# swacisko/ALGA

Measured on AMD Instinct MI355X. Metric: overlap_edges_per_sec, higher is better.
Workload: dtype u32; 1 GPU; cfg4_50M_150bp: 50000000 x 150 bp reads, genome 250000000, seed 11, err 0.00 -> 90621096 nodes (both strands, duplicates removed), min_overlap 82, rsoemo 116; generated on the device (alga_amd.workload.device_build) in 0.9 s; nodes=90621096, edges=92350115

## Files before the change

alga_amd/csrc/engine.hip:

```cpp
#include <hip/hip_runtime.h>

#include <algorithm>
#include <chrono>
#include <cstdio>
#include <cstdlib>
#include <cstring>
#include <new>
#include <string>
#include <thread>
#include <vector>

#include "engine_internal.h"

using namespace alga;

namespace {

using Prepared = AlgaPrepared;

int prepare(alga_engine *e, const alga_nodes *nodes, const alga_prefsuf_params *p, hipStream_t s, Prepared &out) {
    if (!nodes || !p) return alga_fail(e, ALGA_ERR_INVALID_ARGUMENT, "nodes/params must not be NULL");
    if (nodes->n < 0) return alga_fail(e, ALGA_ERR_INVALID_ARGUMENT, "negative node count");
    if (nodes->n > 0 && (!nodes->words || !nodes->len)) return alga_fail(e, ALGA_ERR_INVALID_ARGUMENT, "words/len must not be NULL");
    if (nodes->stride_words <= 0 && nodes->n > 0) return alga_fail(e, ALGA_ERR_INVALID_ARGUMENT, "stride_words must be positive");
// ... 2 lines not shown
    if (p->max_len_cap < 1 || p->max_len_cap > 500) return alga_fail(e, ALGA_ERR_INVALID_ARGUMENT, "max_len_cap must be in [1, 500]");
    if (p->rsoe_min_overlap < 0) return alga_fail(e, ALGA_ERR_INVALID_ARGUMENT, "rsoe_min_overlap must be >= 0");
    if (p->keys_shared < 0 || p->keys_shared > 2) return alga_fail(e, ALGA_ERR_INVALID_ARGUMENT, "keys_shared must be 0, 1 or 2");
    int rc;
    if ((rc = alga_ensure(e, e->counters, (CNT_TOTAL + 2) * sizeof(unsigned long long)))) return rc;
    HIP_TRY(e, hipMemsetAsync(e->counters.p, 0, (CNT_TOTAL + 2) * sizeof(unsigned long long), s));
    NodesDev nd;
    nd.words = nodes->words; nd.len = nodes->len; nd.from = nodes->align_from; nd.to = nodes->align_to;
    nd.n = nodes->n; nd.stride = nodes->stride_words;
    unsigned long long *cnt = (unsigned long long *) e->counters.p;
    int *d_maxlen = (int *) (cnt + CNT_TOTAL);
    unsigned long long mask_asym = 0;
    int min_len = 0;
    if (p->keys_shared == 2 && e->store_n == nodes->n && e->store_words == (const void *) nodes->words && e->stat_len == (const void *) nodes->len &&
        e->stat_from == (const void *) nodes->align_from && e->stat_to == (const void *) nodes->align_to) {
        out.max_len = e->stat_max_len; out.live = e->stat_live; mask_asym = e->stat_mask_asym; min_len = e->stat_min_len;
    } else {
        launch_node_stats(nd, cnt, d_maxlen, s);
        if ((rc = alga_check_launch(e, "k_node_stats"))) return rc;
        HIP_TRY(e, hipMemcpyAsync(e->h_counters, e->counters.p, (CNT_TOTAL + 2) * sizeof(unsigned long long), hipMemcpyDeviceToHost, s));
        HIP_TRY(e, hipStreamSynchronize(s));
        out.max_len = (int) (e->h_counters[CNT_TOTAL] & 0xFFFFFFFFull);
        min_len = out.max_len > 0 ? 0x7FFFFFFF - (int) (e->h_counters[CNT_TOTAL] >> 32) : 0;
        out.live = e->h_counters[CNT_LIVE_NODES];
        mask_asym = e->h_counters[CNT_MASK_ASYM];
        e->stat_max_len = out.max_len; e->stat_min_len = min_len; e->stat_live = out.live; e->stat_mask_asym = mask_asym;
        e->stat_len = (const void *) nodes->len; e->stat_from = (const void *) nodes->align_from; e->stat_to = (const void *) nodes->align_to;
    }
    out.nd = nd;
    out.uniform_len = (out.max_len > 0 && min_len == out.max_len && !nodes->align_from) ? out.max_len : 0;
    if ((int64_t) blocks_of(out.max_len) > (int64_t) nodes->stride_words)
        return alga_fail(e, ALGA_ERR_INVALID_ARGUMENT, "stride_words is smaller than the longest read needs");
    if (out.max_len > OL_MAX_NODE_LEN) return alga_fail(e, ALGA_ERR_CAPACITY, "a node is longer than 4 194 303 nt (overlap records keep the offset in 22 bits)");
    PrefSufCfg c;
    c.Lmin = p->min_overlap;
    c.rsoemo = p->rsoe_min_overlap;
    c.Lcap = std::min(out.max_len, p->max_len_cap) + 1;
    c.soes = p->soes;
    const int seed_nt = std::min(c.Lmin, SEED_MAX_NT);
    c.seed_words = (2 * seed_nt + 31) >> 5;
    c.seed_last_mask = (2 * seed_nt & 31) ? ((1u << (2 * seed_nt & 31)) - 1u) : 0xFFFFFFFFu;
    c.reversed = (c.rsoemo > c.Lcap) ? 1 : 0;
    c.stats = p->collect_stats ? 1 : 0;
    out.cfg = c;
    if (p->reduction < ALGA_REDUCTION_AUTO || p->reduction > ALGA_REDUCTION_SOURCE_SIDE)
        return alga_fail(e, ALGA_ERR_INVALID_ARGUMENT, "reduction must be an alga_reduction value");
    out.local_ok = out.max_len <= p->max_len_cap && out.max_len - c.Lmin <= LOCAL_MAX_SPAN && c.Lmin <= c.rsoemo && c.rsoemo <= c.Lcap &&
                   mask_asym == 0;
    out.local_sw = out.max_len - c.Lmin <= 63 ? 1 : 2;
    out.cluster_eq = 0;
    const bool wide = out.local_sw == 2 || blocks_of(out.max_len) > 13;
    if (out.local_ok && e->opt_probe != ALGA_PROBE_TABLE && !(wide && e->opt_probe == ALGA_PROBE_AUTO && out.live < (4ull << 20))) {
        int eq = 0;
        if (cluster_plan(c, out.max_len, out.live, e->opt_cluster_bucket_bias, &out.cluster, &eq)) out.cluster_eq = eq;
    }
    out.keys_shared = p->keys_shared;
    out.reduction = p->reduction;
    if (out.reduction == ALGA_REDUCTION_AUTO && e->opt_force_per_target) out.reduction = ALGA_REDUCTION_PER_TARGET;
    return ALGA_OK;
}

int cluster_alloc(alga_engine *e, const Prepared &pp) {
    int rc;
    const uint64_t n = (uint64_t) pp.nd.n;
    for (int k = 0; k < 2; k++) {
        if ((rc = alga_ensure(e, e->cl_keys[k], (n + ALGA_KEY_ARRAY_SLACK + 1) * sizeof(uint32_t)))) return rc;
        if ((rc = alga_ensure(e, e->cl_vals[k], (n + 1) * sizeof(uint32_t)))) return rc;
    }
    if ((rc = alga_ensure(e, e->cl_meta, (n + ALGA_KEY_ARRAY_SLACK + 1) * sizeof(uint32_t)))) return rc;
    if ((rc = alga_ensure(e, e->cl_runs, (n + 1) * CL_RMAX * 8))) return rc;
    if ((rc = alga_ensure(e, e->cl_nruns, n + 16))) return rc;
    if ((rc = alga_ensure(e, e->cl_store, (n + 2) * 16 * (size_t) pp.cluster_eq))) return rc;
    if ((rc = alga_ensure(e, e->cl_dir, ((size_t) pp.cluster.n_buckets + 2) * 16))) return rc;
    return alga_ensure(e, e->sort_temp, cluster_sort_temp_bytes(n));
}

int pile_alloc(alga_engine *e, uint64_t n, uint32_t n_buckets, hipStream_t s) {
    int rc;
    if ((rc = alga_ensure(e, e->cl_pile_rec, pile_record_bytes(n)))) return rc;
    if ((rc = alga_ensure(e, e->cl_pile_rec2, pile_record_bytes(n)))) return rc;
    if ((rc = alga_ensure(e, e->cl_pile_succ, ((size_t) n + 64) * 16))) return rc;
    if ((rc = alga_ensure(e, e->cl_pile_cnt, PILE_CNT_WORDS * sizeof(unsigned long long)))) return rc;
    if ((rc = alga_ensure(e, e->cl_pile_own, pile_own_mask_bytes(n)))) return rc;
    if ((rc = alga_ensure(e, e->cl_defer, (size_t) (n + 64) * sizeof(int32_t)))) return rc;
    const void *before = e->cl_pile_tab.p;
    const size_t cap_before = e->cl_pile_tab.cap;
    if ((rc = alga_ensure(e, e->cl_pile_tab, pile_table_bytes(n_buckets)))) return rc;
    if (e->cl_pile_tab.p != before || e->cl_pile_tab.cap != cap_before) {
        HIP_TRY(e, hipMemsetAsync(e->cl_pile_tab.p, 0, e->cl_pile_tab.cap, s));
        HIP_TRY(e, hipStreamSynchronize(s));
        e->pile_epoch = 0;
    }
    return ALGA_OK;
}

int discover_impl(alga_engine *e, const Prepared &pp, int32_t src_begin, int32_t src_end, hipStream_t s, uint64_t *n_rec, bool local = false,
                  bool *overflow = nullptr) {
    int rc;
    const NodesDev &nd = pp.nd;
    const PrefSufCfg &cfg = pp.cfg;
    unsigned long long *cnt = (unsigned long long *) e->counters.p;
    *n_rec = 0;
    HIP_TRY(e, hipEventRecord(e->ev[EV_START], s));
    if (pp.live >= (1ull << 31)) return alga_fail(e, ALGA_ERR_CAPACITY, "too many nodes for one seed table; shard the input");
    const bool clustered = local && pp.cluster_eq != 0;
    e->pairs_timed = false;
    e->store_timed = false;
    e->pile_timed = false;
    const bool all_sources = src_begin == 0 && src_end == pp.nd.n;
    const bool pile_index_left = e->opt_pile_range != 0 && e->pile_n == pp.nd.n && e->pile_words == (const void *) pp.nd.words;
    bool pile = clustered && e->opt_pile != 0 && e->opt_cluster_pairs != 0 && e->opt_cluster_order != 0 && pp.local_sw == 1 &&
                      (pp.keys_shared == 0 || (pp.keys_shared == 2 && pile_index_left)) &&
                      (all_sources || (e->opt_pile_range != 0 && src_begin >= 0 && src_end <= pp.nd.n && src_begin < src_end)) && pile_plan(cfg, pp.cluster, pp.cluster_eq, pp.uniform_len, pp.nd.from != nullptr || pp.nd.to != nullptr);
    e->loc_second_used = false;
    bool keys_only = false;
    const bool need_vals = !e->opt_own_sort || e->opt_test_unsorted_index;
    uint32_t n_buckets = 0, filter_bits = 0;
    bool have_table = false;
    auto build_table = [&]() -> int {
        n_buckets = seed_buckets_for(pp.live, e->seed_fill_x10);
        const size_t table_bytes = (size_t) n_buckets * SEED_BUCKET * sizeof(unsigned long long);
        int r;
        if ((r = alga_ensure(e, e->table, table_bytes))) return r;
        HIP_TRY(e, hipMemsetAsync(e->table.p, 0xFF, table_bytes, s));
        filter_bits = seed_filter_bits_for(pp.live);
        if (filter_bits) {
            if ((r = alga_ensure(e, e->filter, filter_bits / 8))) return r;
            HIP_TRY(e, hipMemsetAsync(e->filter.p, 0, filter_bits / 8, s));
        }
        launch_seed_build(nd, cfg, (unsigned long long *) e->table.p, n_buckets, (uint32_t *) e->filter.p, filter_bits, s);
        if ((r = alga_check_launch(e, "k_seed_build"))) return r;
        e->stats.table_slots = (uint64_t) n_buckets * SEED_BUCKET;
        have_table = true;
        return ALGA_OK;
    };
    ClusterCfg cc{};
    if (clustered) {
        cc = pp.cluster;
        if ((rc = cluster_alloc(e, pp))) return rc;
        if (pp.keys_shared == 2) {
            const bool store_left = e->store_n == nd.n && e->store_words == (const void *) nd.words && e->store_eq == pp.cluster_eq && e->store_buckets == cc.n_buckets;
            const bool piles_serve = pile && e->pile_kept_pure && e->store_buckets == cc.n_buckets && e->store_eq == pp.cluster_eq;
            if (!(store_left || piles_serve) || src_begin < e->store_run_begin || src_end > e->store_run_end)
                return alga_fail(e, ALGA_ERR_INVALID_ARGUMENT, "keys_shared = 2: no entry array of this node set that covers the sources is left from the previous build");
            keys_only = pile && e->pile_keys_only;
        } else {
            int32_t run_begin = 0, run_end = nd.n;
            if (pp.keys_shared == 1) {
                if (e->keyed_n != nd.n || e->keyed_words != (const void *) nd.words || src_begin < e->keyed_begin || src_end > e->keyed_end)
                    return alga_fail(e, ALGA_ERR_INVALID_ARGUMENT, "keys_shared: alga_prefsuf_keys_device has not been called on this node set for a range that covers the sources");
                run_begin = e->keyed_begin; run_end = e->keyed_end;
            } else {
                keys_only = pile && e->opt_pile_runs != 0 && !e->expect_pairwise && !e->opt_pile_check;
                launch_cluster_keys(nd, cfg, cc, 0, nd.n, (uint32_t *) e->cl_keys[0].p, need_vals ? (uint32_t *) e->cl_vals[0].p : nullptr, (uint32_t *) e->cl_meta.p, e->cl_runs.p,
                                    (uint8_t *) e->cl_nruns.p, s, !keys_only);
                if ((rc = alga_check_launch(e, "k_node_runs"))) return rc;
            }
            HIP_TRY(e, hipEventRecord(e->ev[EV_KEYS], s));
            e->keyed_n = -1;
            e->store_n = -1;
            HIP_TRY(e, launch_cluster_store(nd, cc, (uint32_t *) e->cl_keys[0].p, (uint32_t *) e->cl_vals[0].p, (uint32_t *) e->cl_keys[1].p,
                                            (uint32_t *) e->cl_vals[1].p, e->sort_temp.p, cluster_sort_temp_bytes((uint64_t) nd.n), e->cl_dir.p, pp.keys_shared == 1 || !need_vals,
                                            e->ev[EV_SORT], cnt + CNT_TOTAL + 1, e->opt_test_unsorted_index != 0, s, e->opt_own_sort != 0));
            HIP_TRY(e, hipEventRecord(e->ev[EV_DIR], s));
            e->pile_n = -1;
            if (pile) {
                rc = e->opt_test_pile_oom ? alga_fail(e, ALGA_ERR_OUT_OF_MEMORY, "pile_alloc (option test_pile_oom)") : pile_alloc(e, (uint64_t) nd.n, cc.n_buckets, s);
                if (rc == ALGA_ERR_OUT_OF_MEMORY) {
                    (void) hipGetLastError();
                    alga_release(e->cl_pile_tab); alga_release(e->cl_pile_rec); alga_release(e->cl_pile_rec2); alga_release(e->cl_pile_succ); alga_release(e->cl_pile_own);
                    e->pile_epoch = 0; e->pile_n = -1;
                    e->err.clear();
                    pile = false;
                    rc = ALGA_OK;
                    if (keys_only) {
                        launch_cluster_keys(nd, cfg, cc, 0, nd.n, (uint32_t *) e->cl_keys[0].p, (uint32_t *) e->cl_vals[0].p, (uint32_t *) e->cl_meta.p, e->cl_runs.p,
                                            (uint8_t *) e->cl_nruns.p, s, true);
                        if ((rc = alga_check_launch(e, "k_node_runs"))) return rc;
                        keys_only = false;
                    }
                } else if (rc) return rc;
            }
            if (pile) {
                launch_pile_sample(nd, cc, pp.uniform_len, (const uint32_t *) e->cl_keys[1].p, (const uint32_t *) e->cl_vals[1].p, e->cl_dir.p,
                                   (unsigned long long *) e->cl_pile_cnt.p, e->opt_pile >= 2 ? e->opt_pile - 1 : 0, s);
                if ((rc = alga_check_launch(e, "k_pile_build<sample>"))) return rc;
            }
            HIP_TRY(e, launch_cluster_gather(nd, cc, pp.cluster_eq, (const uint32_t *) e->cl_keys[1].p, (const uint32_t *) e->cl_vals[1].p, (const uint32_t *) e->cl_meta.p,
                                             pp.uniform_len, e->cl_store.p, (pile && e->opt_pile_skip_gather) ? (const unsigned long long *) e->cl_pile_cnt.p : nullptr, s));
            HIP_TRY(e, hipEventRecord(e->ev[EV_GATHER], s));
            if (pile) {
                if (e->pile_epoch >= 511u) {
                    HIP_TRY(e, hipMemsetAsync(e->cl_pile_tab.p, 0, e->cl_pile_tab.cap, s));
                    e->pile_epoch = 0;
                }
                e->pile_epoch++;
                const bool from_consensus = e->opt_pile_runs != 0;
                launch_pile_build(nd, cfg, cc, pp.uniform_len, (const uint32_t *) e->cl_keys[1].p, (const uint32_t *) e->cl_vals[1].p, e->cl_dir.p, e->cl_pile_rec.p, e->cl_pile_rec2.p, e->cl_pile_tab.p,
                                  e->pile_epoch, e->cl_pile_succ.p, e->cl_runs.p, pp.uniform_len - cfg.Lmin + 1, (const unsigned long long *) e->cl_pile_cnt.p,
                                  from_consensus ? (uint32_t *) e->cl_pile_own.p : nullptr, s);
                if ((rc = alga_check_launch(e, "k_pile_build"))) return rc;
                if (keys_only) {
                    launch_pile_own_ids((const uint32_t *) e->cl_pile_own.p, (const uint32_t *) e->cl_vals[1].p, (uint64_t) nd.n, (int32_t *) e->cl_defer.p, (uint32_t) nd.n,
                                        (unsigned long long *) e->cl_pile_cnt.p, s);
                    launch_cluster_runs_list(nd, cfg, cc, (const int32_t *) e->cl_defer.p, (const unsigned long long *) e->cl_pile_cnt.p + 3, (uint32_t) nd.n, (uint32_t) e->n_cu * 16u,
                                             e->cl_runs.p, (uint8_t *) e->cl_nruns.p, s);
                    launch_cluster_keys(nd, cfg, cc, 0, nd.n, (uint32_t *) e->cl_keys[0].p, (uint32_t *) e->cl_vals[0].p, (uint32_t *) e->cl_meta.p, e->cl_runs.p,
                                        (uint8_t *) e->cl_nruns.p, s, true, (const unsigned long long *) e->cl_pile_cnt.p);
                    if ((rc = alga_check_launch(e, "k_node_runs (own lists)"))) return rc;
                }
                if (e->opt_pile_check && from_consensus)
                    launch_pile_check(e->cl_pile_succ.p, (uint64_t) nd.n, cc.n_buckets, e->cl_pile_tab.p, e->cl_pile_rec2.p, e->pile_epoch, e->cl_runs.p, nd.n, pp.uniform_len - cfg.Lmin + 1,
                                      (unsigned long long *) e->cl_pile_cnt.p, s);
                e->pile_n = nd.n; e->pile_words = (const void *) nd.words;
                e->pile_keys_only = keys_only; e->pile_kept_pure = false;
                e->pile_timed = nd.n > 0;
            }
            e->store_timed = nd.n > 0;
            e->store_n = pile ? -1 : nd.n;
            e->store_words = (const void *) nd.words; e->store_eq = pp.cluster_eq; e->store_buckets = cc.n_buckets;
            e->store_run_begin = run_begin; e->store_run_end = run_end;
        }
        e->stats.table_slots = cc.n_buckets;
    } else if ((rc = build_table())) return rc;
    HIP_TRY(e, hipEventRecord(e->ev[EV_SEED], s));

    const uint64_t n_src = (uint64_t) std::max<int64_t>(0, (int64_t) src_end - src_begin);
    const uint64_t slack = std::max(probe_record_slack(e->n_cu, n_src, local), clustered ? cluster_record_slack(e->n_cu, n_src) : 0);
    uint64_t &hint = local ? e->rec_cap_hint_local : e->rec_cap_hint;
    uint64_t cap = std::max<uint64_t>(hint, (local ? 2 : 16) * n_src + 4096) + slack;
    if (local) {
        if ((rc = alga_ensure(e, e->outdeg, (size_t) (n_src + 1) * sizeof(uint32_t)))) return rc;
        if ((rc = alga_ensure(e, e->loc_first, (size_t) (n_src + 1) * sizeof(unsigned long long)))) return rc;
    }
    const uint32_t big_list_cap = 1u << 20;
    if (local && (rc = alga_ensure(e, e->loc_big_list, big_list_cap * sizeof(int32_t)))) return rc;
    for (int attempt = 0; attempt < 4; attempt++) {
        if (cap >= (1ull << 32) - 16) return alga_fail(e, ALGA_ERR_CAPACITY, "more than 2^32 overlap records; shard the input");
        if (local) HIP_TRY(e, hipMemsetAsync(e->outdeg.p, 0, (size_t) (n_src + 1) * sizeof(uint32_t), s));
        if ((rc = alga_ensure(e, e->rec_dst, cap * sizeof(uint32_t)))) return rc;
        if ((rc = alga_ensure(e, e->rec_val, cap * sizeof(unsigned long long)))) return rc;
        HIP_TRY(e, hipMemsetAsync(cnt, 0, CNT_TOTAL * sizeof(unsigned long long), s));
        ProbeBig big{(int32_t *) e->loc_big_list.p, big_list_cap, 0u, nullptr, 0u};
        e->defer_list_valid = clustered && e->opt_cluster_pairs && pp.local_sw == 1 && pp.cluster_eq <= 4;
        if (clustered) {
            if (e->opt_cluster_pairs && pp.local_sw == 1 && pp.cluster_eq <= 4) {
                if ((rc = alga_ensure(e, e->cl_defer, (size_t) (n_src + 64) * sizeof(int32_t)))) return rc;
                const uint32_t slot_stride = e->opt_stream_slots >= 4 ? (uint32_t) (n_src + 1) : 0u;
                if ((rc = alga_ensure(e, e->loc_second, (size_t) (slot_stride ? LOCAL_SLOTS_MAX - 1 : 1) * (n_src + 1) * sizeof(unsigned long long)))) return rc;
                e->loc_second_used = true;
                e->loc_slot_stride = slot_stride;
                const bool by_key = e->opt_cluster_order != 0 && src_begin == 0 && src_end == nd.n;
                const bool piled = pile && e->pile_n == nd.n && e->pile_words == (const void *) nd.words;
                if (piled) {
                    if (!all_sources) {
                        if ((rc = alga_ensure(e, e->cl_pile_side_r, (size_t) (n_src + 64) * 16))) return rc;
                        if ((rc = alga_ensure(e, e->cl_pile_cursor, 64))) return rc;
                    }
                    launch_pile_probe(nd, cfg, cc, pp.uniform_len, e->cl_pile_tab.p, e->pile_epoch, e->cl_pile_rec.p, e->cl_pile_rec2.p, e->cl_pile_succ.p,
                                      e->cl_runs.p, cnt, (uint32_t *) e->outdeg.p, (unsigned long long *) e->loc_first.p, (unsigned long long *) e->loc_second.p,
                                      (int32_t *) e->cl_defer.p, (uint32_t) n_src, (const unsigned long long *) e->cl_pile_cnt.p, e->n_cu, s, src_begin, src_end,
                                      e->cl_pile_side_r.p, (unsigned long long *) e->cl_pile_cursor.p);
                    if ((rc = alga_check_launch(e, "k_pile_probe"))) return rc;
                    if (keys_only)
                        launch_cluster_runs_list(nd, cfg, cc, (const int32_t *) e->cl_defer.p, cnt + CNT_DEFERRED, (uint32_t) std::min<uint64_t>(n_src + 64, 0xFFFFFFFFull),
                                                 (uint32_t) e->n_cu * 16u, e->cl_runs.p, (uint8_t *) e->cl_nruns.p, s);
                }
                launch_probe_stream(nd, cfg, cc, pp.cluster_eq, e->cl_store.p, e->cl_dir.p, e->cl_runs.p, (const uint8_t *) e->cl_nruns.p,
                                    src_begin, src_end, by_key, cnt, e->n_cu, (uint32_t *) e->outdeg.p, (unsigned long long *) e->loc_first.p,
                                    (unsigned long long *) e->loc_second.p, (int32_t *) e->cl_defer.p, (uint32_t) n_src,
                                    piled ? (const unsigned long long *) e->cl_pile_cnt.p : nullptr, s, slot_stride);
                if ((rc = alga_check_launch(e, "k_probe_stream"))) return rc;
                if (piled) {
                    if ((rc = alga_ensure(e, e->cl_defer2, (size_t) (n_src + 64) * sizeof(int32_t)))) return rc;
                    launch_probe_stream_list(nd, cfg, cc, pp.cluster_eq, e->cl_store.p, e->cl_dir.p, e->cl_runs.p, (const uint8_t *) e->cl_nruns.p, (int32_t *) e->cl_defer.p,
                                             (uint32_t) n_src, cnt, e->n_cu, (uint32_t *) e->outdeg.p, (unsigned long long *) e->loc_first.p,
                                             (unsigned long long *) e->loc_second.p, (int32_t *) e->cl_defer2.p, (const unsigned long long *) e->cl_pile_cnt.p, s, slot_stride, src_begin);
                    if ((rc = alga_check_launch(e, "k_probe_stream (list)"))) return rc;
                }
                HIP_TRY(e, hipEventRecord(e->ev[EV_PAIRS], s));
                e->pairs_timed = true;
                launch_probe_clustered(nd, cfg, cc, pp.cluster_eq, e->cl_store.p, e->cl_dir.p, e->cl_runs.p, (const uint8_t *) e->cl_nruns.p, 0,
                                       (int32_t) n_src, (const int32_t *) e->cl_defer.p, src_begin, (uint32_t *) e->rec_dst.p, (unsigned long long *) e->rec_val.p,
                                       cap, cnt, e->n_cu, (uint32_t *) e->outdeg.p, (unsigned long long *) e->loc_first.p, &big, cnt + CNT_DEFERRED, 1, s,
                                       (const uint32_t *) e->cl_keys[1].p, (const uint32_t *) e->cl_vals[1].p, pp.uniform_len,
                                       (piled && e->opt_pile_skip_gather) ? (const unsigned long long *) e->cl_pile_cnt.p : nullptr);
                if (piled) launch_pile_deg((int32_t) n_src, (unsigned long long *) e->loc_first.p, (uint32_t *) e->outdeg.p, (const unsigned long long *) e->cl_pile_cnt.p, s);
            } else {
                launch_probe_clustered(nd, cfg, cc, pp.cluster_eq, e->cl_store.p, e->cl_dir.p, e->cl_runs.p, (const uint8_t *) e->cl_nruns.p, src_begin,
                                       src_end, nullptr, src_begin, (uint32_t *) e->rec_dst.p, (unsigned long long *) e->rec_val.p, cap, cnt, e->n_cu,
                                       (uint32_t *) e->outdeg.p, (unsigned long long *) e->loc_first.p, &big, nullptr, pp.local_sw, s);
            }
        }
        else
            launch_probe(nd, cfg, (const unsigned long long *) e->table.p, n_buckets, (const uint32_t *) e->filter.p, filter_bits, src_begin, src_end,
                         (uint32_t *) e->rec_dst.p, (unsigned long long *) e->rec_val.p, cap, cnt, e->n_cu, local ? pp.local_sw : 0, (uint32_t *) e->outdeg.p,
                         (unsigned long long *) e->loc_first.p, local ? &big : nullptr, s);
        if ((rc = alga_check_launch(e, "k_probe_sources"))) return rc;
        HIP_TRY(e, hipEventRecord(e->ev[EV_PROBE], s));
        HIP_TRY(e, hipMemcpyAsync(e->h_counters, cnt, (CNT_TOTAL + 2) * sizeof(unsigned long long), hipMemcpyDeviceToHost, s));
        HIP_TRY(e, hipStreamSynchronize(s));
        if (clustered && e->h_counters[CNT_TOTAL + 1] != 0) {
            e->store_n = -1; e->keyed_n = -1;
            return alga_fail(e, ALGA_ERR_HIP, "clustered index: the sorted key array is not in order (entry directory invalid)");
        }
        if (local && e->h_counters[CNT_LOCAL_OVERFLOW] != 0) {
            const uint64_t n_big = e->h_counters[CNT_LOCAL_OVERFLOW], max_items = e->h_counters[CNT_LOCAL_MAXITEMS];
            const uint64_t limit = e->big_limit >= 0 ? (uint64_t) e->big_limit : (uint64_t) local_big_limit();
            if (n_big > big_list_cap || max_items > limit) { if (overflow) *overflow = true; *n_rec = 0; return ALGA_OK; }
            big.count = (uint32_t) n_big;
            big.item_cap = (uint32_t) ((max_items + 63) & ~63ull);
            if ((rc = alga_ensure(e, e->loc_big_items, probe_big_bytes(e->n_cu, big.count, pp.local_sw, big.item_cap)))) return rc;
            big.items = e->loc_big_items.p;
            if (!have_table && (rc = build_table())) return rc;
            HIP_TRY(e, hipMemsetAsync(cnt + CNT_LOCAL_OVERFLOW, 0, sizeof(unsigned long long), s));
            launch_probe(nd, cfg, (const unsigned long long *) e->table.p, n_buckets, (const uint32_t *) e->filter.p, filter_bits, src_begin, src_end,
                         (uint32_t *) e->rec_dst.p, (unsigned long long *) e->rec_val.p, cap, cnt, e->n_cu, pp.local_sw, (uint32_t *) e->outdeg.p,
                         (unsigned long long *) e->loc_first.p, &big, s);
            if ((rc = alga_check_launch(e, "k_probe_sources (second pass)"))) return rc;
            HIP_TRY(e, hipEventRecord(e->ev[EV_PROBE], s));
            HIP_TRY(e, hipMemcpyAsync(e->h_counters, cnt, CNT_TOTAL * sizeof(unsigned long long), hipMemcpyDeviceToHost, s));
            HIP_TRY(e, hipStreamSynchronize(s));
            if (e->h_counters[CNT_LOCAL_OVERFLOW] != 0) { if (overflow) *overflow = true; *n_rec = 0; return ALGA_OK; }
            e->stats.big_sources = n_big;
        }
        const uint64_t need = e->h_counters[CNT_RECORDS];
        if (need <= cap) {
            *n_rec = need;
            hint = std::max<uint64_t>(hint, need + need / 16 + 4096);
            if (overflow) *overflow = false;
            if (local) { e->stats.transitive_compares = e->h_counters[CNT_TR_COMPARES]; e->stats.generic_sources = e->h_counters[CNT_LOCAL_GENERIC]; }
            e->stats.records = e->h_counters[CNT_VALID_RECORDS];
            e->stats.raw_overlaps = e->h_counters[CNT_RAW];
            e->stats.windows_probed = e->h_counters[CNT_WINDOWS];
            e->stats.slots_scanned = e->h_counters[CNT_SLOTS];
            e->stats.probe_rounds = e->h_counters[CNT_ROUNDS];
            e->stats.pile_buckets = e->h_counters[CNT_PILE_BUCKETS]; e->stats.pile_irregular = e->h_counters[CNT_PILE_IRREGULAR];
            e->stats.pile_own_lists = e->h_counters[CNT_PILE_OWN];
            if (pile && pp.keys_shared != 2 && e->pile_n == nd.n) {
                const bool kept = e->opt_pile == 2 || e->stats.pile_irregular * (uint64_t) ALGA_PILE_DECLINE_ONE_IN <= e->stats.pile_buckets;
                e->stats.pile_mixed = kept && e->stats.pile_irregular * (uint64_t) ALGA_PILE_IRREGULAR_ONE_IN > e->stats.pile_buckets;
                e->stats.pile_deferred = e->stats.pile_mixed ? e->h_counters[CNT_DEFERRED_PILE] : (kept ? e->h_counters[CNT_DEFERRED] : 0);
                if (!kept || e->stats.pile_mixed || !e->opt_pile_skip_gather) e->store_n = nd.n;
                e->expect_pairwise = !kept;
                e->pile_kept_pure = kept && !e->stats.pile_mixed && e->opt_pile_skip_gather != 0;
                e->stats.pile_list_checked = 0; e->stats.pile_list_mismatch = 0;
                if (e->opt_pile_check) {
                    unsigned long long chk[2] = {0ull, 0ull};
                    HIP_TRY(e, hipMemcpyAsync(chk, (const unsigned long long *) e->cl_pile_cnt.p + 4, sizeof(chk), hipMemcpyDeviceToHost, s));
                    HIP_TRY(e, hipStreamSynchronize(s));
                    e->stats.pile_list_checked = chk[0]; e->stats.pile_list_mismatch = chk[1];
                }
            }
            if (!pile) e->expect_pairwise = false;
            e->stats.probe_used = clustered ? ALGA_PROBE_CLUSTER : ALGA_PROBE_TABLE;
            if (clustered) e->stats.deferred_sources = e->defer_list_valid ? e->h_counters[CNT_DEFERRED] : n_src;
            return ALGA_OK;
        }
        cap = need + need / 16 + 4096 + slack;
    }
    return alga_fail(e, ALGA_ERR_HIP, "record buffer kept overflowing");
}

int key_bits_for(int64_t n_owned) {
    int b = 1;
    while (b < 31 && (1ll << b) < n_owned) b++;
    return std::min(32, b + 1);
}

int reduce_impl(alga_engine *e, const Prepared &pp, const uint32_t *rec_dst, const unsigned long long *rec_val, uint64_t n_rec,
                uint64_t n_valid_hint, int32_t dst_begin, int32_t dst_end, hipStream_t s, uint64_t *n_edges) {
    int rc;
    const NodesDev &nd = pp.nd;
    const PrefSufCfg &cfg = pp.cfg;
    unsigned long long *cnt = (unsigned long long *) e->counters.p;
    const int32_t n_owned = dst_end - dst_begin;
    *n_edges = 0;
    if (n_rec >= (1ull << 32) - 16) return alga_fail(e, ALGA_ERR_CAPACITY, "more than 2^32 overlap records; shard the input");
    const int bits = key_bits_for(n_owned);
    const size_t temp_bytes = sort_records_temp_bytes(n_rec, bits);
    if ((rc = alga_ensure(e, e->keys, (size_t) (n_rec + 1) * sizeof(uint32_t)))) return rc;
    if ((rc = alga_ensure(e, e->seg_key, (size_t) (n_rec + 1) * sizeof(uint32_t)))) return rc;
    if ((rc = alga_ensure(e, e->seg_val, (size_t) (n_rec + 1) * sizeof(unsigned long long)))) return rc;
    if ((rc = alga_ensure(e, e->sort_temp, temp_bytes))) return rc;
    if ((rc = alga_ensure(e, e->heads, (size_t) (n_rec + 1) * 16))) return rc;
    if ((rc = alga_ensure(e, e->rowptr, (size_t) (n_owned + 2) * sizeof(uint32_t)))) return rc;
    HIP_TRY(e, hipMemsetAsync(cnt + CNT_SORT_VALID, 0, sizeof(unsigned long long), s));
    launch_make_keys(rec_dst, n_rec, dst_begin, dst_end, (uint32_t *) e->keys.p, cnt + CNT_SORT_VALID, s);
    if ((rc = alga_check_launch(e, "k_make_keys"))) return rc;
    HIP_TRY(e, sort_records(e->sort_temp.p, temp_bytes, (const uint32_t *) e->keys.p, (uint32_t *) e->seg_key.p, rec_val,
                            (unsigned long long *) e->seg_val.p, n_rec, bits, s));
    launch_rowptr_from_sorted((const uint32_t *) e->seg_key.p, cnt + CNT_SORT_VALID, n_rec, n_owned, (uint32_t *) e->rowptr.p, s);
    if ((rc = alga_check_launch(e, "k_rowptr_from_sorted"))) return rc;
    launch_gather_heads(nd, (const unsigned long long *) e->seg_val.p, cnt + CNT_SORT_VALID, n_rec, e->heads.p, s);
    if ((rc = alga_check_launch(e, "k_gather_heads"))) return rc;
    HIP_TRY(e, hipEventRecord(e->ev[EV_GROUP], s));

    if ((rc = alga_ensure(e, e->out_cnt, (size_t) (n_owned + 1) * sizeof(uint32_t)))) return rc;
    if ((rc = alga_ensure(e, e->outdeg, (size_t) (nd.n + 1) * sizeof(uint32_t)))) return rc;
    HIP_TRY(e, hipMemsetAsync(e->outdeg.p, 0, (size_t) (nd.n + 1) * sizeof(uint32_t), s));
    const int tpb = reduce_targets_per_block(n_valid_hint, (uint64_t) std::max(1, n_owned));
    launch_reduce_targets(nd, cfg, dst_begin, n_owned, tpb, (const uint32_t *) e->rowptr.p, (unsigned long long *) e->seg_val.p,
                          e->heads.p, (uint32_t *) e->out_cnt.p, (uint32_t *) e->outdeg.p, cnt, s);
    if ((rc = alga_check_launch(e, "k_reduce_targets"))) return rc;
    HIP_TRY(e, hipEventRecord(e->ev[EV_REDUCE], s));

    if ((rc = alga_ensure(e, e->scan_scratch, scan_scratch_bytes((uint64_t) nd.n)))) return rc;
    if ((rc = alga_ensure(e, e->out_rowptr, (size_t) (nd.n + 1) * sizeof(uint32_t)))) return rc;
    launch_exclusive_scan((const uint32_t *) e->outdeg.p, (uint64_t) nd.n, (uint32_t *) e->out_rowptr.p, (uint64_t *) e->scan_scratch.p, s);
    if ((rc = alga_check_launch(e, "scan(outdeg)"))) return rc;
    uint64_t *d_total = (uint64_t *) e->scan_scratch.p + scan_total_index((uint64_t) nd.n);
    HIP_TRY(e, hipMemcpyAsync(&e->h_counters[CNT_TOTAL], d_total, sizeof(uint64_t), hipMemcpyDeviceToHost, s));
    HIP_TRY(e, hipMemcpyAsync(e->h_counters, cnt, CNT_TOTAL * sizeof(unsigned long long), hipMemcpyDeviceToHost, s));
    HIP_TRY(e, hipStreamSynchronize(s));
    const uint64_t E = e->h_counters[CNT_TOTAL];
    if (E >= (1ull << 32) - 16) return alga_fail(e, ALGA_ERR_CAPACITY, "more than 2^32 edges; shard the input");
    if ((rc = alga_ensure(e, e->edges, (size_t) (E + 1) * sizeof(alga_edge_dev)))) return rc;
    launch_scatter_by_source(cfg, dst_begin, n_owned, (const uint32_t *) e->rowptr.p, (const unsigned long long *) e->seg_val.p,
                             (const uint32_t *) e->out_cnt.p, (const uint32_t *) e->out_rowptr.p, (uint32_t *) e->outdeg.p,
                             (alga_edge_dev *) e->edges.p, s);
    if ((rc = alga_check_launch(e, "k_scatter_by_source"))) return rc;
    launch_sort_rows(nd.n, (const uint32_t *) e->out_rowptr.p, (alga_edge_dev *) e->edges.p, s);
    if ((rc = alga_check_launch(e, "k_sort_rows"))) return rc;
    HIP_TRY(e, hipEventRecord(e->ev[EV_EMIT], s));
    HIP_TRY(e, hipStreamSynchronize(s));
    *n_edges = E;
    e->stats.edges = E;
    e->stats.transitive_listed = e->h_counters[CNT_TR_LISTED];
    e->stats.transitive_compares = e->h_counters[CNT_TR_COMPARES];
    e->stats.transitive_removed = e->h_counters[CNT_TR_REMOVED];
    e->stats.max_in_records = e->h_counters[CNT_MAX_IN];
    return ALGA_OK;
}

int finalize_local(alga_engine *e, const Prepared &pp, int32_t src_begin, int32_t src_end, uint64_t n_rec, hipStream_t s, uint64_t *n_edges) {
    int rc;
    *n_edges = 0;
    const uint64_t n_src = (uint64_t) std::max<int64_t>(0, (int64_t) src_end - src_begin);
    if ((rc = alga_ensure(e, e->scan_scratch, scan_scratch_bytes(n_src)))) return rc;
    if ((rc = alga_ensure(e, e->out_rowptr, (size_t) (n_src + 1) * sizeof(uint32_t)))) return rc;
    if ((rc = alga_ensure(e, e->out_cnt, (size_t) (n_src + 1) * sizeof(uint32_t)))) return rc;
    HIP_TRY(e, hipEventRecord(e->ev[EV_GROUP], s));
    HIP_TRY(e, hipEventRecord(e->ev[EV_REDUCE], s));
    launch_exclusive_scan((const uint32_t *) e->outdeg.p, n_src, (uint32_t *) e->out_rowptr.p, (uint64_t *) e->scan_scratch.p, s);
    if ((rc = alga_check_launch(e, "scan(outdeg)"))) return rc;
    const uint64_t E = e->stats.records;
    if (E >= (1ull << 32) - 16) return alga_fail(e, ALGA_ERR_CAPACITY, "more than 2^32 edges; shard the input");
    if ((rc = alga_ensure(e, e->edges, (size_t) (E + 1) * sizeof(alga_edge_dev)))) return rc;
    launch_local_emit(src_begin, (int32_t) n_src, (const uint32_t *) e->outdeg.p, (const unsigned long long *) e->loc_first.p,
                      e->loc_second_used ? (const unsigned long long *) e->loc_second.p : nullptr, (const uint32_t *) e->rec_dst.p, (const unsigned long long *) e->rec_val.p, n_rec, (const uint32_t *) e->out_rowptr.p,
                      (uint32_t *) e->out_cnt.p, (alga_edge_dev *) e->edges.p,
                      e->defer_list_valid ? (const int32_t *) e->cl_defer.p : nullptr, (const unsigned long long *) e->counters.p + CNT_DEFERRED, (uint32_t) n_src, s,
                      e->loc_second_used ? e->loc_slot_stride : 0u);
    if ((rc = alga_check_launch(e, "k_local_emit"))) return rc;
    HIP_TRY(e, hipEventRecord(e->ev[EV_EMIT], s));
    uint64_t *d_total = (uint64_t *) e->scan_scratch.p + scan_total_index(n_src);
    HIP_TRY(e, hipMemcpyAsync(&e->h_counters[CNT_TOTAL], d_total, sizeof(uint64_t), hipMemcpyDeviceToHost, s));
    HIP_TRY(e, hipStreamSynchronize(s));
    if (e->h_counters[CNT_TOTAL] != E) return alga_fail(e, ALGA_ERR_HIP, "source-side emit: out-degrees and edge count disagree");
    *n_edges = E;
    e->stats.edges = E;
    return ALGA_OK;
}

int build_local(alga_engine *e, const Prepared &pp, int32_t src_begin, int32_t src_end, hipStream_t s, uint64_t *n_edges) {
    if (!pp.local_ok) return alga_fail(e, ALGA_ERR_UNSUPPORTED, "source-side reduction is not exact for this input (read lengths / masks / rsoemo)");
    uint64_t n_rec = 0;
    bool overflow = false;
    int rc = discover_impl(e, pp, src_begin, src_end, s, &n_rec, true, &overflow);
    if (rc) return rc;
    if (overflow) return alga_fail(e, ALGA_ERR_UNSUPPORTED, "a source node has more raw overlaps than the source-side reduction holds");
    if ((rc = finalize_local(e, pp, src_begin, src_end, n_rec, s, n_edges))) return rc;
    e->stats.reduction_used = ALGA_REDUCTION_SOURCE_SIDE;
    return ALGA_OK;
}

double now_ms_host() { return std::chrono::duration<double, std::milli>(std::chrono::steady_clock::now().time_since_epoch()).count(); }

float ev_ms(alga_engine *e, int a, int b) {
    float ms = 0.f;
    if (hipEventElapsedTime(&ms, e->ev[a], e->ev[b]) != hipSuccess) return 0.f;
    return ms;
}

void store_phase_stats(alga_engine *e) {
    if (!e->store_timed) return;
    e->stats.ms_keys = ev_ms(e, EV_START, EV_KEYS);
    e->stats.ms_sort = ev_ms(e, EV_KEYS, EV_SORT);
    e->stats.ms_dir = ev_ms(e, EV_SORT, EV_DIR);
    e->stats.ms_gather = ev_ms(e, EV_DIR, EV_GATHER);
    e->stats.ms_pile = e->pile_timed ? ev_ms(e, EV_GATHER, EV_SEED) : 0.0;
}

}

int alga_prepare(alga_engine *e, const alga_nodes *nodes, const alga_prefsuf_params *p, hipStream_t s, AlgaPrepared &out) { return prepare(e, nodes, p, s, out); }
int alga_cluster_alloc(alga_engine *e, const AlgaPrepared &pp) { return cluster_alloc(e, pp); }

extern "C" {

int alga_abi_version(void) { return ALGA_AMD_ABI_VERSION; }

struct DeviceGuard {
    int prev = -1;
    DeviceGuard() { if (hipGetDevice(&prev) != hipSuccess) prev = -1; }
    ~DeviceGuard() { if (prev >= 0) (void) hipSetDevice(prev); }
};

static void engine_free_handles(alga_engine *e) {
    if (e->h_counters) (void) hipHostFree(e->h_counters);
    for (int i = 0; i < EV_COUNT; i++) if (e->ev[i]) (void) hipEventDestroy(e->ev[i]);
    if (e->own_stream) (void) hipStreamDestroy(e->own_stream);
    if (e->side_stream) (void) hipStreamDestroy(e->side_stream);
    if (e->ev_side) (void) hipEventDestroy(e->ev_side);
    e->h_counters = nullptr; e->own_stream = nullptr; e->side_stream = nullptr; e->ev_side = nullptr;
    for (int i = 0; i < EV_COUNT; i++) e->ev[i] = nullptr;
}

int alga_engine_create(int hip_device, alga_engine **out) {
    if (!out) return ALGA_ERR_INVALID_ARGUMENT;
    *out = nullptr;
    int ndev = 0;
    hipError_t err = hipGetDeviceCount(&ndev);
    if (err != hipSuccess || ndev <= 0) return ALGA_ERR_NO_DEVICE;
    if (hip_device < 0 || hip_device >= ndev) return ALGA_ERR_INVALID_ARGUMENT;
    DeviceGuard guard;
    if (hipSetDevice(hip_device) != hipSuccess) return ALGA_ERR_NO_DEVICE;
    alga_engine *e = new (std::nothrow) alga_engine();
    if (!e) return ALGA_ERR_OUT_OF_MEMORY;
    e->device = hip_device;
    memset(&e->stats, 0, sizeof(e->stats));
    hipDeviceProp_t prop;
    if (hipGetDeviceProperties(&prop, hip_device) == hipSuccess) {
        snprintf(e->dev_name, sizeof(e->dev_name), "%s (%s, %d CUs)", prop.name, prop.gcnArchName, prop.multiProcessorCount);
        if (prop.multiProcessorCount > 0) e->n_cu = prop.multiProcessorCount;
    }
    int rc = ALGA_OK;
    if (hipStreamCreateWithFlags(&e->own_stream, hipStreamNonBlocking) != hipSuccess) { e->own_stream = nullptr; rc = ALGA_ERR_HIP; }
    if (rc == ALGA_OK && hipStreamCreateWithFlags(&e->side_stream, hipStreamNonBlocking) != hipSuccess) { e->side_stream = nullptr; rc = ALGA_ERR_HIP; }
    if (rc == ALGA_OK && hipEventCreateWithFlags(&e->ev_side, hipEventDisableTiming) != hipSuccess) { e->ev_side = nullptr; rc = ALGA_ERR_HIP; }
    for (int i = 0; i < EV_COUNT && rc == ALGA_OK; i++)
        if (hipEventCreate(&e->ev[i]) != hipSuccess) { e->ev[i] = nullptr; rc = ALGA_ERR_HIP; }
    if (rc == ALGA_OK && hipHostMalloc((void **) &e->h_counters, (CNT_TOTAL + 2 + alga_engine::H_EXTRA) * sizeof(unsigned long long)) != hipSuccess) { e->h_counters = nullptr; rc = ALGA_ERR_OUT_OF_MEMORY; }
    if (rc == ALGA_OK && hipHostGetDevicePointer((void **) &e->h_counters_dev, e->h_counters, 0) != hipSuccess) rc = ALGA_ERR_HIP;
    if (rc != ALGA_OK) { engine_free_handles(e); delete e; return rc; }
    *out = e;
    return ALGA_OK;
}

void alga_engine_destroy(alga_engine *e) {
    if (!e) return;
    DeviceGuard guard;
    (void) hipSetDevice(e->device);
    if (e->own_stream) (void) hipStreamSynchronize(e->own_stream);
    if (e->side_stream) (void) hipStreamSynchronize(e->side_stream);
    for (DevBuf *b : e->owned) alga_release(*b);
    alga_release(e->up_raw);
    for (DevBuf *b : {&e->in_bytes[0], &e->in_bytes[1], &e->in_nl[0], &e->in_nl[1], &e->in_tiles, &e->in_tile_off}) alga_release(*b);
    for (DevBuf *b : {&e->sp_rowptr, &e->sp_sorted, &e->sp_list, &e->sp_cnt, &e->sp_orow, &e->sp_out, &e->sp_in}) alga_release(*b);
    alga_staging_release(e);
    for (void *&p : e->gfa_pin) { if (p) (void) hipHostFree(p); p = nullptr; }
    for (auto &kv : e->host_lists) free(kv.first);
    e->host_lists.clear();
    engine_free_handles(e);
    delete e;
}

const char *alga_last_error(const alga_engine *e) { return e ? e->err.c_str() : "no engine"; }

int alga_engine_device_name(const alga_engine *e, char *buf, size_t buflen) {
    if (!e || !buf || buflen == 0) return ALGA_ERR_INVALID_ARGUMENT;
    snprintf(buf, buflen, "%s", e->dev_name);
    return ALGA_OK;
}

int alga_engine_set_option(alga_engine *e, const char *name, int64_t value) {
    if (!e || !name) return ALGA_ERR_INVALID_ARGUMENT;
    e->err.clear();
    if (!strcmp(name, "probe")) {
        if (value < ALGA_PROBE_AUTO || value > ALGA_PROBE_CLUSTER) return alga_fail(e, ALGA_ERR_INVALID_ARGUMENT, "option probe: 0 auto, 1 table, 2 cluster");
        e->opt_probe = (int) value;
    } else if (!strcmp(name, "cluster_bucket_bias")) {
        if (value < -8 || value > 8) return alga_fail(e, ALGA_ERR_INVALID_ARGUMENT, "option cluster_bucket_bias: -8 .. 8");
        e->opt_cluster_bucket_bias = (int) value;
    } else if (!strcmp(name, "cluster_pairs")) {
        e->opt_cluster_pairs = value != 0;
    } else if (!strcmp(name, "pile")) {
        e->opt_pile = (value == 2 || value == 3) ? (int) value : (value != 0);
    } else if (!strcmp(name, "pile_runs")) {
        e->opt_pile_runs = value != 0;
    } else if (!strcmp(name, "pile_check")) {
        e->opt_pile_check = value != 0;
    } else if (!strcmp(name, "pile_skip_gather")) {
        e->opt_pile_skip_gather = value != 0;
    } else if (!strcmp(name, "cluster_order")) {
        e->opt_cluster_order = value != 0;
    } else if (!strcmp(name, "local_big_max")) {
        e->big_limit = value < 0 ? -1 : (int) std::min<int64_t>(value, 1 << 20);
    } else if (!strcmp(name, "shard_bucket_max")) {
        e->opt_shard_dmax = (int) std::max<int64_t>(1, std::min<int64_t>(value, 4096));
    } else if (!strcmp(name, "rsort_variant")) {
        rsort_set_variant((int) value);
    } else if (!strcmp(name, "stream_slots")) {
        e->opt_stream_slots = value >= 4 ? 4 : 2;
    } else if (!strcmp(name, "pile_range")) {
        e->opt_pile_range = value != 0;
    } else if (!strcmp(name, "pkb_legacy")) {
        e->opt_pkb_legacy = (int) value;
    } else if (!strcmp(name, "own_sort")) {
        e->opt_own_sort = value != 0;
    } else if (!strcmp(name, "test_presort_oom")) {
        e->opt_test_presort_oom = value != 0;
    } else if (!strcmp(name, "test_pile_oom")) {
        e->opt_test_pile_oom = value != 0;
    } else if (!strcmp(name, "test_unsorted_index")) {
        e->opt_test_unsorted_index = value != 0;
    } else if (!strcmp(name, "gfa_chunk_mb")) {
        if (value < 1 || value > 4096) return alga_fail(e, ALGA_ERR_INVALID_ARGUMENT, "option gfa_chunk_mb: 1 .. 4096");
        e->opt_gfa_chunk_mb = (int) value;
    } else if (!strcmp(name, "auto_reduction_per_target")) {
        e->opt_force_per_target = value != 0;
    } else return alga_fail(e, ALGA_ERR_INVALID_ARGUMENT, "unknown option");
    return ALGA_OK;
}

int alga_engine_reserve(alga_engine *e, int32_t n_nodes, int32_t max_len, int32_t min_overlap, uint64_t n_edges_hint) {
    if (!e) return ALGA_ERR_INVALID_ARGUMENT;
    e->err.clear();
    if (n_nodes < 0 || max_len < 1 || min_overlap < 1) return alga_fail(e, ALGA_ERR_INVALID_ARGUMENT, "alga_engine_reserve: n_nodes >= 0, max_len >= 1, min_overlap >= 1");
    DeviceGuard guard;
    HIP_TRY(e, hipSetDevice(e->device));
    int rc;
    const uint64_t n = (uint64_t) n_nodes;
    const uint64_t E = n_edges_hint ? n_edges_hint : n + n / 16 + 4096;
    if ((rc = alga_ensure(e, e->counters, (CNT_TOTAL + 2) * sizeof(unsigned long long)))) return rc;
    Prepared pp;
    pp.nd.n = n_nodes; pp.max_len = max_len; pp.live = n;
    pp.cfg.Lmin = min_overlap; pp.cfg.Lcap = std::min(max_len, 500) + 1; pp.cfg.rsoemo = min_overlap; pp.cfg.soes = 3;
    int eq = 0;
    const bool local = max_len <= 500 && max_len - min_overlap <= LOCAL_MAX_SPAN;
    const bool clustered = local && e->opt_probe != ALGA_PROBE_TABLE &&
                           cluster_plan(pp.cfg, max_len, n, e->opt_cluster_bucket_bias, &pp.cluster, &eq);
    if (clustered) {
        pp.cluster_eq = eq;
        if ((rc = cluster_alloc(e, pp))) return rc;
        if (max_len - min_overlap <= 63 && eq <= 4) {
            if ((rc = alga_ensure(e, e->cl_defer, (size_t) (n + 64) * sizeof(int32_t)))) return rc;
            if ((rc = alga_ensure(e, e->loc_second, (size_t) (e->opt_stream_slots >= 4 ? LOCAL_SLOTS_MAX - 1 : 1) * (n + 1) * sizeof(unsigned long long)))) return rc;
        }
        if (e->opt_pile != 0 && e->opt_cluster_pairs != 0 && e->opt_cluster_order != 0 && max_len - min_overlap <= 63 && pile_plan(pp.cfg, pp.cluster, eq, max_len, false)) {
            if ((rc = pile_alloc(e, n, pp.cluster.n_buckets, e->own_stream))) return rc;
        }
    } else {
        const uint32_t nb = seed_buckets_for(n, e->seed_fill_x10);
        if ((rc = alga_ensure(e, e->table, (size_t) nb * SEED_BUCKET * sizeof(unsigned long long)))) return rc;
        const uint32_t fb = seed_filter_bits_for(n);
        if (fb && (rc = alga_ensure(e, e->filter, fb / 8))) return rc;
    }
    if (local) {
        const uint64_t slack = std::max(probe_record_slack(e->n_cu, n, true), clustered ? cluster_record_slack(e->n_cu, n) : 0);
        const uint64_t cap = std::max<uint64_t>(e->rec_cap_hint_local, 2 * n + 4096) + slack;
        if ((rc = alga_ensure(e, e->outdeg, (size_t) (n + 1) * sizeof(uint32_t)))) return rc;
        if ((rc = alga_ensure(e, e->loc_first, (size_t) (n + 1) * sizeof(unsigned long long)))) return rc;
        if ((rc = alga_ensure(e, e->loc_big_list, (1u << 20) * sizeof(int32_t)))) return rc;
        if ((rc = alga_ensure(e, e->rec_dst, cap * sizeof(uint32_t)))) return rc;
        if ((rc = alga_ensure(e, e->rec_val, cap * sizeof(unsigned long long)))) return rc;
        if ((rc = alga_ensure(e, e->scan_scratch, scan_scratch_bytes(n)))) return rc;
        if ((rc = alga_ensure(e, e->out_rowptr, (size_t) (n + 1) * sizeof(uint32_t)))) return rc;
        if ((rc = alga_ensure(e, e->out_cnt, (size_t) (n + 1) * sizeof(uint32_t)))) return rc;
    }
    if ((rc = alga_ensure(e, e->edges, (size_t) (E + 1) * sizeof(alga_edge_dev)))) return rc;
    if (!e->warmed && n_nodes > 0) {
        const int W = blocks_of(max_len), stride = hbm_row_stride(W), wn = 4096;
// ... 616 lines not shown
```

alga_amd/csrc/engine_internal.h:

```cpp
#pragma once
#include <hip/hip_runtime.h>

#include <cstdio>
#include <algorithm>
#include <string>
#include <vector>
#include <unordered_map>

#include "../../include/alga_amd.h"
#include "prefsuf_common.h"
#include "prefsuf_kernels.h"
#include "pkb_kernels.h"

struct DevBuf {
    void  *p = nullptr;
    size_t cap = 0;
};

enum { EV_START = 0, EV_SEED, EV_PROBE, EV_GROUP, EV_REDUCE, EV_EMIT, EV_PAIRS, EV_KEYS, EV_SORT, EV_GATHER, EV_DIR, EV_COUNT };
constexpr int ALGA_STAGE_THREADS = 8;

struct alga_engine {
    std::vector<DevBuf *> owned;
    int         device = -1;
    hipStream_t own_stream = nullptr;
    hipStream_t side_stream = nullptr;
    hipEvent_t  ev_side = nullptr;
    std::string err;
    char        dev_name[256] = {0};
    int         n_cu = 256;
    int         seed_fill_x10 = 20;
    int         opt_probe = 0;
    int         opt_cluster_bucket_bias = 0;
    int         opt_force_per_target = 0;
    int         opt_shard_dmax = 4096;
    int         opt_test_unsorted_index = 0;
    hipEvent_t  ev[EV_COUNT] = {};
    DevBuf table, filter, counters, rowptr, rec_dst, rec_val, keys, seg_key, seg_val, heads, sort_temp, out_cnt, outdeg, out_rowptr, edges, scan_scratch;
    DevBuf cl_defer;
    uint32_t h_first_hkey = 255;
    int32_t keyed_n = -1, keyed_begin = 0, keyed_end = 0;
    bool defer_list_valid = false;
    const void *keyed_words = nullptr;
    int32_t store_n = -1, store_run_begin = 0, store_run_end = 0, store_eq = 0;
    uint32_t store_buckets = 0;
    const void *store_words = nullptr;
    int stat_max_len = 0, stat_min_len = 0; uint64_t stat_live = 0; unsigned long long stat_mask_asym = 0;
    const void *stat_len = nullptr, *stat_from = nullptr, *stat_to = nullptr;
    bool   warmed = false;
    bool   pairs_timed = false;
    bool   store_timed = false;
    bool   pile_keys_only = false, pile_kept_pure = false;
    int    opt_pile_range = 1;
    int    opt_pile_skip_gather = 1;
    int    opt_pile = 1;
    int    opt_pile_runs = 1;
    int    opt_pile_check = 0;
    bool   expect_pairwise = false;
    DevBuf cl_pile_side_r, cl_pile_cursor;
    DevBuf cl_pile_own;
    int    opt_pkb_legacy = 0;
    int    opt_own_sort = 1;
    int    opt_test_presort_oom = 0;
    int    opt_test_pile_oom = 0;
    bool   pile_timed = false;
    DevBuf cl_pile_succ;
    DevBuf cl_pile_rec2;
    DevBuf cl_pile_rec, cl_pile_cnt, cl_pile_tab;
    uint32_t pile_epoch = 0;
    int32_t pile_n = -1; const void *pile_words = nullptr;
    int    opt_cluster_order = 1;
    int    opt_cluster_pairs = 1;
    DevBuf cl_keys[2], cl_vals[2], cl_meta, cl_runs, cl_nruns, cl_store, cl_dir;
    DevBuf loc_second;
    bool   loc_second_used = false;
    uint32_t loc_slot_stride = 0;
    int    opt_stream_slots = 4;
    DevBuf loc_first, loc_big_list, loc_big_items;
    int    big_limit = -1;
    DevBuf edge_keys, edge_keys2, edge_vals, edge_vals2, edges_sorted, xs_dst, xs_val;
    DevBuf up_words, up_len, up_from, up_to;
    DevBuf up_len_narrow;
    DevBuf cp_deg, cp_dst, cp_off;
    DevBuf cl_defer2;
    DevBuf pk_keys, pk_keys2, pk_vals, pk_vals2, pk_marks, pk_big, pk_add, pk_ekeys, pk_ekeys2, pk_flag, pk_pos, pk_edges[2], pk_rowptr, pk_deg,
           pk_mask, pk_cnt, pk_io, pk_io2, pk_tips, pk_heads, pk_g[2], pk_addk, pk_addk2, pk_merged, pk_hsz, pk_hsz2, pk_heads2, pk_nadd, pk_koff,
           pk_gsz, pk_fixlist, pk_bounds, pk_tiprec, pk_tipidx, pk_keys_all, pk_vals_all;
    DevBuf pk_keys2b, pk_vals2b, pk_headsb, pk_hszb, sort_temp2, pk_fixlist2, pk_cnt2;
    DevBuf pp_rows, pp_len, pp_perm[2], pp_keys[2], pp_mark, pp_keep, pp_pos, pp_out_rows, pp_out_len, pp_out_pair, pp_tally;
    bool        stage_ready = false;
    void       *stage_pin[ALGA_STAGE_THREADS][2] = {};
    hipEvent_t  stage_ev[ALGA_STAGE_THREADS][2] = {};
    hipStream_t stage_stream[ALGA_STAGE_THREADS] = {};
    DevBuf      up_raw;
    std::unordered_map<void *, size_t> host_lists;
    void       *host_spare = nullptr;
    size_t      host_spare_cap = 0;
    DevBuf      in_bytes[2], in_nl[2], in_tiles, in_tile_off;
    DevBuf      sp_rowptr, sp_sorted, sp_list, sp_cnt, sp_orow, sp_out, sp_in;
    DevBuf      gfa_sizes, gfa_off, gfa_rowptr, gfa_tiles, gfa_bounds, gfa_buf;
    void       *gfa_pin[2] = {nullptr, nullptr};
    size_t      gfa_pin_cap = 0;
    int         opt_gfa_chunk_mb = 256;
    DevBuf      sh_keys[2], sh_vals[2], sh_store, sh_dir, sh_desc_out, sh_dkey[2], sh_dval[2], sh_small_top, sh_pending, sh_bitmap, sh_small_out,
                sh_ssrc[2], sh_skey[2], sh_edges_out, sh_deg, sh_rowptr, sh_cursor, sh_edges, sh_flagged, sh_cnt, sh_gflag, sh_gpos, sh_gstart;
    struct {
        int      phase = 0;
        int      rank = 0, n_ranks = 1, eq = 0, uniform_len = 0;
        int32_t  n = 0;
        const void *words = nullptr;
        alga::PrefSufCfg cfg{};
        alga::ClusterCfg cc{};
        uint32_t bucket_base = 0, bpr = 0;
        uint64_t n_targets = 0, n_desc = 0, n_rec = 0;
        uint32_t *d_keys_sorted = nullptr;
        unsigned long long *d_vals_sorted = nullptr;
    } sh;
    alga_shard_stats shard_stats{};
    struct {
        int      phase = 0;
        int      rounds = 0, round = 0, rank = 0, n_ranks = 1, cur = 0, key_bits = 0;
        int32_t  prio[4] = {0, 1, 2, 3};
        uint64_t E = 0, nk = 0;
        uint32_t n_tips = 0;
        int      pre_set = 0, cur_set = 0;
        bool     no_look_ahead = false;
        int      pre_round = -1;
        bool     kmers_all = false;
        size_t   kmers_stride = 0;
        int      kmers_sort_bits = 0;
        alga_nodes dn{};
        alga::PkbCfg cfg{};
    } pkb;
    unsigned long long *h_counters = nullptr;
    static constexpr int H_EXTRA = 132 + 16, H_PRE = alga::CNT_TOTAL + 2 + 132;
    uint32_t *h_counters_dev = nullptr;
    uint64_t    rec_cap_hint = 0, rec_cap_hint_local = 0;
    alga_prefsuf_stats stats;
    double      stats_host[2] = {0.0, 0.0};
// ... 71 lines not shown
```

alga_amd/csrc/prefsuf_cluster_device.h:

```cpp
#pragma once
#include <hip/hip_runtime.h>
#include "prefsuf_common.h"
#include "../../include/alga_amd.h"
#include "prefsuf_device.h"

namespace alga {

__device__ __forceinline__ uint32_t kmer_hash(uint32_t lo, uint32_t hi) {
    return (lo ^ __funnelshift_l(hi, hi, 13) ^ (hi >> 7)) * 0x9E3779B1u;
}

__device__ __forceinline__ bool kmer_class0(uint32_t lo) { return (lo & 3u) == 0u && ((((lo >> 2) ^ (lo >> 3)) & 1u) != 0u); }
__device__ __forceinline__ uint32_t order_key0(uint32_t h, int pos) { return ((h >> 1) & 0x7FFFFF00u) | (uint32_t) pos; }
__device__ __forceinline__ uint32_t order_key(uint32_t h, uint32_t lo, int pos) { return order_key0(h, pos) | (kmer_class0(lo) ? 0u : 0x80000000u); }
__device__ __forceinline__ uint32_t class0_mask16(uint32_t cur, uint32_t nxt) {
    const uint32_t nx = __funnelshift_r(cur, nxt, 2);
    return ~(cur | (cur >> 1)) & (nx ^ (nx >> 1)) & 0x55555555u;
}
__device__ __forceinline__ uint32_t compress_even(uint32_t x) {
    x = (x | (x >> 1)) & 0x33333333u;
    x = (x | (x >> 2)) & 0x0F0F0F0Fu;
    x = (x | (x >> 4)) & 0x00FF00FFu;
    return (x | (x >> 8)) & 0x0000FFFFu;
}

__device__ __forceinline__ uint32_t cluster_key(uint32_t h, int fs) {
    uint32_t k = h * 0x9E3779B1u;
    k ^= k >> 15;
    k *= 0x85EBCA77u;
    k ^= k >> 13;
    k *= 0xC2B2AE3Du;
    return (k >> (fs + CL_MBITS)) == (0xFFFFFFFFu >> (fs + CL_MBITS)) ? k ^ 0x80000000u : k;
}

__device__ __forceinline__ uint32_t tgt_sort_key(uint32_t ckey, uint32_t m_c, int fs) {
    const uint32_t fm = ((1u << CL_MBITS) - 1u) << fs;
    return (ckey & ~fm) | ((m_c << fs) & fm);
}
__device__ __forceinline__ bool same_cluster(uint32_t entry_key, uint32_t ckey, int fs) {
    return ((entry_key ^ ckey) & ~(((1u << CL_MBITS) - 1u) << fs)) == 0u;
}

constexpr unsigned long long PILE_IRREGULAR_ONE_IN = ALGA_PILE_IRREGULAR_ONE_IN;
constexpr unsigned long long PILE_DECLINE_ONE_IN = ALGA_PILE_DECLINE_ONE_IN;
__device__ __forceinline__ bool pile_cnt_declines(const unsigned long long *c) { return c[1] * PILE_DECLINE_ONE_IN > c[0]; }
__device__ __forceinline__ bool pile_cnt_mixed(const unsigned long long *c) { return !pile_cnt_declines(c) && c[1] * PILE_IRREGULAR_ONE_IN > c[0]; }
__device__ __forceinline__ void run_slice(const uint4 &rec, uint32_t run_y, uint32_t &e0, uint32_t &cnt) {
    const int q = (int) (run_y & 255u), p0 = (int) ((run_y >> 8) & 255u), p1 = (int) ((run_y >> 16) & 255u);
    int mlo = q - p1 + 1, mhi = q - p0;
    mlo = mlo < 0 ? 0 : mlo; mhi = mhi > 63 ? 63 : mhi;
    e0 = rec.x; cnt = rec.y;
    if (mhi < mlo) { cnt = 0u; return; }
    if (rec.y > 255u) return;
    const int s0 = mlo >> 3, s1 = (mhi >> 3) + 1;
    const uint32_t b0 = ((s0 < 4 ? rec.z : rec.w) >> (8 * (s0 & 3))) & 255u;
    const uint32_t b1 = s1 >= 8 ? rec.y : (((s1 < 4 ? rec.z : rec.w) >> (8 * (s1 & 3))) & 255u);
    e0 = rec.x + b0; cnt = b1 - b0;
}

__device__ __forceinline__ void kmer_key(const uint32_t *row, int i, bool valid, const ClusterCfg &cc, uint32_t &h, uint32_t &pk) {
    const int bit = 2 * i, q = bit >> 5, r = bit & 31;
    const uint32_t x0 = row[q], x1 = row[q + 1], x2 = row[q + 2];
    const uint32_t lo = funnel(x0, x1, r) & cc.lo_mask;
    h = kmer_hash(lo, funnel(x1, x2, r) & cc.hi_mask);
    pk = valid ? order_key(h, lo, i) : 0xFFFFFFFFu;
}

constexpr int TK_ROWS = 128;
constexpr int NR_STACK = 8;

template <bool WIDE, int RCAP = CL_RMAX>
__device__ __forceinline__ void node_runs_core(const uint32_t *row, int nwin, bool act, const ClusterCfg &cc, uint32_t (*stk)[TK_ROWS], uint16_t (*rbuf)[TK_ROWS], int t,
                                               int &nr, bool &uncovered, bool &stack_ovf, uint32_t &cur0, int step = 64) {
    constexpr int S0 = NR_STACK + 1;
    const int w = cc.w;
    nr = 0; uncovered = false; stack_ovf = false; cur0 = 0xFFFFFFFFu;
    for (int hb = (WIDE && nwin > step) ? ((nwin - 1) / step) * step : 0; hb >= 0; hb -= step) {
        const uint32_t *rowh = row + (hb >> 4);
        const int nwh = !WIDE ? nwin : (nwin - hb < step ? nwin - hb : step);
        const int nk = act ? nwh - 1 + w : 0;
        uint64_t m_lo, m_hi;
        {
            uint32_t dm[4];
#pragma unroll
            for (int d = 0; d < 4; d++) {
                const uint32_t x0 = rowh[2 * d], x1 = rowh[2 * d + 1], x2 = rowh[2 * d + 2];
                dm[d] = compress_even(class0_mask16(x0, x1)) | (compress_even(class0_mask16(x1, x2)) << 16);
            }
            m_lo = (uint64_t) dm[0] | ((uint64_t) dm[1] << 32);
            m_hi = (uint64_t) dm[2] | ((uint64_t) dm[3] << 32);
            m_lo &= nk >= 64 ? ~0ull : (nk <= 0 ? 0ull : ((1ull << nk) - 1ull));
            m_hi &= nk <= 64 ? 0ull : ((1ull << (nk - 64)) - 1ull);
        }
        uint64_t b0 = w >= 64 ? m_lo : (m_lo & ((1ull << w) - 1ull));
        uint64_t b1 = w >= 64 ? m_hi : ((m_lo >> w) | (m_hi << (64 - w)));
        auto key_at = [&](int pos) -> uint32_t {
            const int bit = 2 * pos, q = bit >> 5, r = bit & 31;
            const uint32_t x0 = rowh[q], x1 = rowh[q + 1], x2 = rowh[q + 2];
            return order_key0(kmer_hash(funnel(x0, x1, r) & cc.lo_mask, funnel(x1, x2, r) & cc.hi_mask), pos);
        };
        uint32_t cur1 = 0xFFFFFFFFu;
        int sp1 = 0;
        while (b1 != 0ull) {
            const int e = __builtin_ctzll(b1);
            b1 &= b1 - 1ull;
            const uint32_t pk = key_at(w + e);
            const bool push = pk < cur1;
            stk[(push && sp1 < NR_STACK) ? sp1 : NR_STACK][t] = pk;
            cur1 = push ? pk : cur1;
            sp1 += push ? 1 : 0;
        }
        uint32_t cur0h = 0xFFFFFFFFu;
        int sp0 = 0;
        while (b0 != 0ull) {
            const int e = 63 - __builtin_clzll(b0);
            b0 ^= 1ull << e;
            const uint32_t pk = key_at(e);
            const bool push = pk < cur0h;
            stk[S0 + ((push && sp0 < NR_STACK) ? sp0 : NR_STACK)][t] = pk;
            cur0h = push ? pk : cur0h;
            sp0 += push ? 1 : 0;
        }
        if (hb == 0) cur0 = cur0h;
        stack_ovf = stack_ovf || sp1 > NR_STACK || sp0 > NR_STACK;
        sp1 = sp1 > NR_STACK ? NR_STACK : sp1;
        sp0 = sp0 > NR_STACK ? NR_STACK : sp0;
        {
            const uint32_t hq = (uint32_t) hb | ((uint32_t) hb << 8);
            uint32_t top = sp1 > 0 ? stk[sp1 - 1][t] : 0xFFFFFFFFu;
            uint32_t nxt0 = stk[S0][t];
            uint32_t c0 = 0xFFFFFFFFu, win = top;
            int i0 = 0, p_hi = nwh - 1;
            int e0 = sp0 > 0 ? (int) (nxt0 & 255u) : -1;
            int e1 = sp1 > 0 ? (int) (top & 255u) - w : -1;
            while ((e0 > e1 ? e0 : e1) >= 0) {
                const int pe = e0 > e1 ? e0 : e1;
                const bool take0 = e0 >= e1;
                const int row_i = take0 ? S0 + i0 + 1 : (sp1 >= 2 ? sp1 - 2 : NR_STACK);
                const uint32_t v = stk[row_i][t];
                i0 += take0 ? 1 : 0;
                sp1 -= take0 ? 0 : 1;
                c0 = take0 ? nxt0 : c0;
                nxt0 = take0 ? v : nxt0;
                top = take0 ? top : (sp1 >= 1 ? v : 0xFFFFFFFFu);
                e0 = take0 ? (i0 < sp0 ? (int) (v & 255u) : -1) : e0;
                e1 = take0 ? e1 : (sp1 >= 1 ? (int) (v & 255u) - w : -1);
                const uint32_t wn = c0 < top ? c0 : top;
                const int pc = pe < p_hi ? pe : p_hi;
                const bool em = wn != win && pc < p_hi;
                rbuf[(em && nr < RCAP) ? nr : RCAP][t] = (uint16_t) (((win & 255u) | ((uint32_t) (pc + 1) << 8)) + hq);
                uncovered = uncovered || (em && win == 0xFFFFFFFFu);
                nr += em ? 1 : 0;
                p_hi = em ? pc : p_hi;
                win = wn;
            }
            if (act) {
                if (nr < RCAP) rbuf[nr][t] = (uint16_t) ((win & 255u) + hq);
                uncovered = uncovered || win == 0xFFFFFFFFu;
                nr++;
            }
        }
    }
}

__device__ __forceinline__ uint32_t bperm(uint32_t v, int src_lane) { return (uint32_t) __builtin_amdgcn_ds_bpermute(src_lane << 2, (int) v); }

}
```

alga_amd/csrc/prefsuf_kernels.h:

```cpp
#pragma once
#include <hip/hip_runtime.h>
#include <stddef.h>
#include <stdint.h>
#include "prefsuf_common.h"

namespace alga {

struct alga_edge_dev { int32_t src, dst, offset; };

void launch_restride(const uint32_t *in, int stride_in, uint32_t *out, int stride_out, uint64_t n, hipStream_t s);
void launch_widen_len(const void *in, int elem_bytes , int32_t *out, uint64_t n, hipStream_t s);
void launch_compact_edges(const alga_edge_dev *edges, int32_t n, uint64_t n_edges, uint8_t *deg, uint32_t *dst, uint8_t *off, unsigned long long *bad, hipStream_t s);
void launch_expand_twins(const uint32_t *in, int stride_in, const int32_t *len , uint32_t *out, int stride_out, uint64_t n_pairs, hipStream_t s);
void launch_node_stats(const NodesDev &nd, unsigned long long *counters, int *max_len , hipStream_t s);

uint32_t seed_buckets_for(uint64_t live_nodes, int fill_x10);
uint32_t seed_filter_bits_for(uint64_t live_nodes);
void launch_seed_build(const NodesDev &nd, const PrefSufCfg &cfg, unsigned long long *table, uint32_t n_buckets, uint32_t *filter,
                       uint32_t filter_bits, hipStream_t s);

struct ProbeBig { int32_t *list; uint32_t list_cap; uint32_t count; void *items; uint32_t item_cap; };
int    local_item_capacity();
int    local_big_limit();
size_t probe_big_bytes(int n_cu, uint32_t count, int local, uint32_t item_cap);

void launch_probe(const NodesDev &nd, const PrefSufCfg &cfg, const unsigned long long *table, uint32_t n_buckets,
                  const uint32_t *filter, uint32_t filter_bits, int32_t src_begin, int32_t src_end, uint32_t *rec_dst, unsigned long long *rec_val, uint64_t rec_cap,
                  unsigned long long *counters, int n_cu, int local , uint32_t *deg , unsigned long long *first ,
                  const ProbeBig *big , hipStream_t s);
uint64_t probe_record_slack(int n_cu, uint64_t n_src, bool local);
void launch_local_emit(int32_t src_base, int32_t n_src, const uint32_t *deg, const unsigned long long *first, const unsigned long long *second,
                       const uint32_t *rec_dst, const unsigned long long *rec_val, uint64_t n_rec, const uint32_t *rowptr, uint32_t *cursor,
                       alga_edge_dev *edges, const int32_t *record_sources, const unsigned long long *record_sources_count, uint32_t record_sources_cap, hipStream_t s, uint32_t slot_stride = 0);

bool       cluster_plan(const PrefSufCfg &cfg, int max_len, uint64_t live, int bucket_log2_bias, ClusterCfg *c, int *eq);
size_t     cluster_sort_temp_bytes(uint64_t n);
void       launch_cluster_keys(const NodesDev &nd, const PrefSufCfg &cfg, const ClusterCfg &cc, int32_t node_begin, int32_t node_end, uint32_t *keys,
                               uint32_t *vals, uint32_t *meta, void *runs, uint8_t *nruns, hipStream_t s, bool with_runs = true ,
                               const unsigned long long *only_if_declined = nullptr );
void       launch_cluster_runs_list(const NodesDev &nd, const PrefSufCfg &cfg, const ClusterCfg &cc, const int32_t *ids, const unsigned long long *count, uint32_t cap,
                                    uint32_t grid_blocks, void *runs, uint8_t *nruns, hipStream_t s);
hipError_t launch_cluster_store(const NodesDev &nd, const ClusterCfg &cc, uint32_t *keys, uint32_t *vals, uint32_t *keys2 , uint32_t *vals2, void *sort_temp,
                                size_t sort_temp_bytes, void *dir, bool fill_vals, hipEvent_t ev_sorted ,
                                unsigned long long *bad_flag ,
                                bool test_skip_sort , hipStream_t s, bool own_sort = true);
hipError_t launch_cluster_gather(const NodesDev &nd, const ClusterCfg &cc, int eq, const uint32_t *keys2, const uint32_t *vals2, const uint32_t *meta,
                                 int uniform_len , void *store,
                                 const unsigned long long *pile_cnt , hipStream_t s);
uint64_t   cluster_record_slack(int n_cu, uint64_t n_src);
void       launch_probe_clustered(const NodesDev &nd, const PrefSufCfg &cfg, const ClusterCfg &cc, int eq, const void *store, const void *dir,
                                  const void *runs, const uint8_t *nruns, int32_t src_begin, int32_t src_end, const int32_t *src_list, int32_t src_base, uint32_t *rec_dst, unsigned long long *rec_val, uint64_t rec_cap,
                                  unsigned long long *counters, int n_cu, uint32_t *deg, unsigned long long *first, const ProbeBig *big,
                                  const unsigned long long *list_count ,
                                  int sw , hipStream_t s,
                                  const uint32_t *skeys = nullptr, const uint32_t *sids = nullptr, int uniform_len = 0,
                                  const unsigned long long *pile_cnt = nullptr );
void       launch_probe_stream(const NodesDev &nd, const PrefSufCfg &cfg, const ClusterCfg &cc, int eq, const void *store, const void *dir,
                               const void *runs, const uint8_t *nruns, int32_t src_begin, int32_t src_end, bool by_key ,
                               unsigned long long *counters, int n_cu, uint32_t *deg, unsigned long long *first, unsigned long long *second, int32_t *defer_list,
                               uint32_t defer_cap, const unsigned long long *pile_cnt ,
                               hipStream_t s, uint32_t slot_stride = 0 );
void       launch_pile_deg(int32_t n, unsigned long long *first, uint32_t *deg, const unsigned long long *pile_cnt, hipStream_t s);
bool       pile_plan(const PrefSufCfg &cfg, const ClusterCfg &cc, int eq, int uniform_len, bool masks);
size_t     pile_record_bytes(uint64_t n);
size_t     pile_table_bytes(uint32_t n_buckets);
void       launch_pile_sample(const NodesDev &nd, const ClusterCfg &cc, int uniform_len, const uint32_t *skeys , const uint32_t *sids , const void *dir,
                              unsigned long long *pile_cnt , int no_sample, hipStream_t s);
constexpr int PILE_CNT_WORDS = 6;
size_t     pile_own_mask_bytes(uint64_t n);
void       launch_pile_build(const NodesDev &nd, const PrefSufCfg &cfg, const ClusterCfg &cc, int uniform_len, const uint32_t *skeys, const uint32_t *sids, const void *dir, void *rec,
                             void *rec2 , void *tab, uint32_t epoch, void *side, const void *runs, int nwin, const unsigned long long *pile_cnt,
                             uint32_t *own_mask , hipStream_t s);
void       launch_pile_own_ids(const uint32_t *own_mask, const uint32_t *sids, uint64_t n_entries, int32_t *list, uint32_t cap, unsigned long long *pile_cnt, hipStream_t s);
void       launch_pile_check(const void *side, uint64_t n_entries, uint32_t n_buckets, const void *tab, const void *rec2, uint32_t epoch, const void *runs, int n_nodes, int nwin,
                             unsigned long long *pile_cnt, hipStream_t s);
void       launch_probe_stream_list(const NodesDev &nd, const PrefSufCfg &cfg, const ClusterCfg &cc, int eq, const void *store, const void *dir, const void *runs, const uint8_t *nruns,
                                    int32_t *src_list, uint32_t list_cap, unsigned long long *counters, int n_cu, uint32_t *deg, unsigned long long *first,
                                    unsigned long long *second, int32_t *defer2, const unsigned long long *pile_cnt, hipStream_t s, uint32_t slot_stride = 0,
                                    int32_t src_base = 0 );
void       launch_pile_probe(const NodesDev &nd, const PrefSufCfg &cfg, const ClusterCfg &cc, int uniform_len, const void *tab, uint32_t epoch, const void *rec, const void *rec2, const void *side,
                             const void *runs, unsigned long long *counters, uint32_t *deg, unsigned long long *first, unsigned long long *second, int32_t *defer_list,
                             uint32_t defer_cap, const unsigned long long *pile_cnt, int n_cu, hipStream_t s, int32_t src_begin, int32_t src_end,
                             void *side_range , unsigned long long *cursor );

size_t     rsort_u32_pairs_temp_bytes(uint64_t n);
void       rsort_set_variant(int v);
hipError_t rsort_u32_pairs(void *temp, size_t temp_bytes, const uint32_t *keys_in, uint32_t *keys_out, const uint32_t *vals_in, uint32_t *vals_out, uint64_t n,
                           int begin_bit, hipStream_t s);
size_t     sort_u32_pairs_temp_bytes(uint64_t n);
hipError_t sort_u32_pairs(void *temp, size_t temp_bytes, const uint32_t *keys_in, uint32_t *keys_out, const uint32_t *vals_in, uint32_t *vals_out,
                          uint64_t n, int begin_bit , hipStream_t s, bool own_sort = true );
size_t     rsort_u64_pairs_temp_bytes(uint64_t n);
hipError_t rsort_u64_pairs(void *temp, size_t temp_bytes, const unsigned long long *keys_in, unsigned long long *keys_out, const unsigned long long *vals_in,
                           unsigned long long *vals_out, uint64_t n, int bits, hipStream_t s);
hipError_t rsort_u32_u64(void *temp, size_t temp_bytes, const uint32_t *keys_in, uint32_t *keys_out, const unsigned long long *vals_in, unsigned long long *vals_out,
                         uint64_t n, int begin_bit, int end_bit, hipStream_t s);
size_t     sort_u64_pairs_temp_bytes(uint64_t n, int bits);
hipError_t sort_u64_pairs(void *temp, size_t temp_bytes, const unsigned long long *keys_in, unsigned long long *keys_out,
                          const unsigned long long *vals_in, unsigned long long *vals_out, uint64_t n, int bits, hipStream_t s);

void launch_make_keys(const uint32_t *rec_dst, uint64_t n_rec, int32_t dst_begin, int32_t dst_end, uint32_t *keys,
                      unsigned long long *n_valid, hipStream_t s);
size_t     sort_records_temp_bytes(uint64_t n, int bits);
hipError_t sort_records(void *temp, size_t temp_bytes, const uint32_t *keys_in, uint32_t *keys_out, const unsigned long long *vals_in,
                        unsigned long long *vals_out, uint64_t n, int bits, hipStream_t s);
void launch_rowptr_from_sorted(const uint32_t *keys, const unsigned long long *n_valid_ptr, uint64_t n_rec_max, int32_t n_owned,
                               uint32_t *rowptr, hipStream_t s);

size_t   scan_scratch_bytes(uint64_t n);
uint64_t scan_total_index(uint64_t n);
void launch_exclusive_scan(const uint32_t *in, uint64_t n, uint32_t *out, uint64_t *scratch, hipStream_t s);
constexpr int MAIL_SEGS = 6;
struct MailSeg { const uint32_t *src; uint32_t words, dst; };
struct MailArgs {
    MailSeg seg[MAIL_SEGS];
    int n = 0;
    void add(const void *src, uint32_t words, uint32_t dst_word) { seg[n].src = (const uint32_t *) src; seg[n].words = words; seg[n].dst = dst_word; n++; }
};
void launch_mail(const MailArgs &a, uint32_t *host_block_dev, hipStream_t s);

int  reduce_targets_per_block(uint64_t n_records, uint64_t n_targets);
void launch_gather_heads(const NodesDev &nd, const unsigned long long *seg_val, const unsigned long long *n_valid_ptr, uint64_t n_rec_max,
                         void *heads , hipStream_t s);
void launch_reduce_targets(const NodesDev &nd, const PrefSufCfg &cfg, int32_t dst_begin, int32_t n_owned, int32_t targets_per_block,
                           const uint32_t *rowptr, unsigned long long *seg_val, const void *heads, uint32_t *out_cnt, uint32_t *outdeg,
                           unsigned long long *counters, hipStream_t s);
void launch_scatter_by_source(const PrefSufCfg &cfg, int32_t dst_begin, int32_t n_owned, const uint32_t *rowptr,
                              const unsigned long long *seg_val, const uint32_t *out_cnt, const uint32_t *out_rowptr, uint32_t *out_cursor,
                              alga_edge_dev *edges, hipStream_t s);
void launch_sort_rows(int32_t n, const uint32_t *out_rowptr, alga_edge_dev *edges, hipStream_t s);

void launch_edges_to_keys(const alga_edge_dev *e, uint64_t n, unsigned long long *keys, uint32_t *vals, hipStream_t s);
void launch_keys_to_edges(const unsigned long long *keys, const uint32_t *vals, uint64_t n, alga_edge_dev *e, hipStream_t s);
size_t     sort_edges_temp_bytes(uint64_t n);
hipError_t sort_edges(void *temp, size_t temp_bytes, const unsigned long long *keys_in, unsigned long long *keys_out, const uint32_t *vals_in,
                      uint32_t *vals_out, uint64_t n, int src_bits, hipStream_t s);

}
```

alga_amd/csrc/prefsuf_kernels.hip:

```cpp
#include <hip/hip_runtime.h>
#include <algorithm>
#include "prefsuf_common.h"
#include "prefsuf_kernels.h"
#include "prefsuf_device.h"

namespace alga {

__global__ void __launch_bounds__(256) k_node_stats(NodesDev nd, unsigned long long *counters, int *max_len) {
    __shared__ int s_max[4], s_min[4];
    __shared__ unsigned long long s_live[4];
    int m = 0, mn = 0x7FFFFFFF;
    unsigned long long live = 0, asym = 0;
    auto one = [&](int l, int64_t i) {
        m = l > m ? l : m;
        mn = (l > 0 && l < mn) ? l : mn;
        live += l > 0;
        if (nd.to && l > 0 && !nd.to[i] && (nd.from == nullptr || nd.from[i])) asym++;
    };
    const int64_t gid = (int64_t) blockIdx.x * blockDim.x + threadIdx.x, gsz = (int64_t) gridDim.x * blockDim.x;
    int64_t done = 0;
    if ((reinterpret_cast<uintptr_t>(nd.len) & 15u) == 0) {
        const int64_t nq = (int64_t) nd.n >> 2;
        const int4 *len4 = reinterpret_cast<const int4 *>(nd.len);
        for (int64_t q = gid; q < nq; q += gsz) { const int4 l = len4[q]; one(l.x, 4 * q); one(l.y, 4 * q + 1); one(l.z, 4 * q + 2); one(l.w, 4 * q + 3); }
        done = 4 * nq;
    }
    for (int64_t i = done + gid; i < nd.n; i += gsz) one(nd.len[i], i);
#pragma unroll
    for (int o = 32; o > 0; o >>= 1) { int t = __shfl_xor(m, o); m = t > m ? t : m; t = __shfl_xor(mn, o); mn = t < mn ? t : mn; }
    live = wave_sum_u64(live);
    asym = wave_sum_u64(asym);
    const int wave = (int) (threadIdx.x >> 6);
    if (lane_id() == 0) { s_max[wave] = m; s_min[wave] = mn; s_live[wave] = live; if (asym) atomicAdd(&counters[CNT_MASK_ASYM], asym); }
    __syncthreads();
    if (threadIdx.x == 0) {
        for (int w = 1; w < 4; w++) { m = s_max[w] > m ? s_max[w] : m; mn = s_min[w] < mn ? s_min[w] : mn; live += s_live[w]; }
        if (m > 0) { atomicMax(max_len, m); atomicMax(max_len + 1, 0x7FFFFFFF - mn); }
        if (live) atomicAdd(&counters[CNT_LIVE_NODES], live);
    }
}

__device__ __forceinline__ uint32_t seed_bucket(uint64_t h, uint32_t n_buckets) { return __umulhi((uint32_t) h, n_buckets); }
__device__ __forceinline__ uint32_t seed_taglen(uint64_t h, int len) {
    return ((uint32_t) (h >> 41) << 9) | (uint32_t) (len > 511 ? 511 : len);
}

__device__ __forceinline__ uint32_t seed_filter_index(uint64_t h, uint32_t filter_mask) { return (uint32_t) (h >> 32) & filter_mask; }

__global__ void __launch_bounds__(256) k_seed_build(NodesDev nd, PrefSufCfg cfg, unsigned long long *table, uint32_t n_buckets,
                                                     uint32_t *filter, uint32_t filter_mask) {
    int i = blockIdx.x * blockDim.x + threadIdx.x;
    if (i >= nd.n) return;
    int len = nd.len[i];
    if (len <= 0 || len < cfg.Lmin) return;
    if (nd.to && !nd.to[i]) return;
    const uint32_t *row = nd.words + (size_t) i * nd.stride;
    uint64_t h = fp_init();
    for (int k = 0; k < cfg.seed_words; k++) {
        uint32_t w = row[k];
        if (k == cfg.seed_words - 1) w &= cfg.seed_last_mask;
        h = fp_step(h, w);
    }
    h = fp_final(h);
    uint32_t b = seed_bucket(h, n_buckets);
    if (filter) { const uint32_t fi = seed_filter_index(h, filter_mask); atomicOr(&filter[fi >> 5], 1u << (fi & 31)); }
    const unsigned long long entry = ((unsigned long long) seed_taglen(h, len) << 32) | (uint32_t) i;
    for (;;) {
        unsigned long long *bp = table + (size_t) b * SEED_BUCKET;
        for (int j = 0; j < SEED_BUCKET; j++) {
            if (bp[j] != SEED_EMPTY) continue;
            if (atomicCAS(&bp[j], (unsigned long long) SEED_EMPTY, entry) == SEED_EMPTY) return;
        }
        b = (b + 1 == n_buckets) ? 0u : b + 1;
    }
}

#ifndef PROBE_OCC
#define PROBE_OCC 4
#endif
template <bool STATS, int NQ, int LOCAL, bool BIG = false>
__global__ void __launch_bounds__(PROBE_WAVES * 64, PROBE_OCC)
k_probe_sources(NodesDev nd, PrefSufCfg cfg, const unsigned long long *__restrict__ table, uint32_t n_buckets,
                const uint32_t *__restrict__ filter, uint32_t filter_mask, int32_t src_begin, int32_t src_end, ProbeOut o) {
    __shared__ uint32_t sB[PROBE_WAVES][STAGE_WORDS];
    __shared__ uint32_t sCandC[PROBE_WAVES][CANDMAX];
    __shared__ uint32_t sCandW[PROBE_WAVES][CANDMAX];
    constexpr int WB = LOCAL ? WBUF_LOCAL : WBUF;
// ... 397 lines not shown
    flush_records<CHUNK, WB>(o, w, chunk_base, chunk_fill);
    close_chunk<CHUNK>(o, chunk_base, chunk_fill);
    st_rec = wave_sum_u64(st_rec);
    if (lane == 0 && st_rec) atomicAdd(&o.counters[CNT_VALID_RECORDS], (unsigned long long) st_rec);
    if (STATS) {
        st_raw = wave_sum_u64(st_raw); st_slots = wave_sum_u64(st_slots); st_win = wave_sum_u64(st_win);
        st_cmp = wave_sum_u64(st_cmp); st_generic = wave_sum_u64(st_generic);
        if (lane == 0) {
            atomicAdd(&o.counters[CNT_RAW], (unsigned long long) st_raw);
            atomicAdd(&o.counters[CNT_SLOTS], (unsigned long long) st_slots);
            atomicAdd(&o.counters[CNT_WINDOWS], (unsigned long long) st_win);
            if (LOCAL) {
                atomicAdd(&o.counters[CNT_TR_COMPARES], (unsigned long long) st_cmp);
                atomicAdd(&o.counters[CNT_LOCAL_GENERIC], (unsigned long long) st_generic);
            }
        }
    }
}

__global__ void __launch_bounds__(256) k_make_keys(const uint32_t *__restrict__ rec_dst, uint64_t n_rec, int32_t dst_begin, int32_t dst_end,
                                                    uint32_t *__restrict__ keys, unsigned long long *__restrict__ n_valid) {
    __shared__ unsigned long long s_cnt[4];
    unsigned long long cnt = 0;
    for (uint64_t i = (uint64_t) blockIdx.x * blockDim.x + threadIdx.x; i < n_rec; i += (uint64_t) gridDim.x * blockDim.x) {
        const uint32_t c = rec_dst[i];
        const bool ok = c != REC_INVALID && (int) c >= dst_begin && (int) c < dst_end;
        keys[i] = ok ? c - (uint32_t) dst_begin : 0xFFFFFFFFu;
        cnt += ok;
    }
    cnt = wave_sum_u64(cnt);
    if (lane_id() == 0) s_cnt[threadIdx.x >> 6] = cnt;
    __syncthreads();
    if (threadIdx.x == 0) { cnt = s_cnt[0] + s_cnt[1] + s_cnt[2] + s_cnt[3]; if (cnt) atomicAdd(n_valid, cnt); }
}

__global__ void __launch_bounds__(256) k_rowptr_from_sorted(const uint32_t *__restrict__ keys, const unsigned long long *__restrict__ n_valid_ptr,
                                                             int32_t n_owned, uint32_t *__restrict__ rowptr) {
    const uint64_t nv = (uint64_t) *n_valid_ptr;
    for (uint64_t i = (uint64_t) blockIdx.x * blockDim.x + threadIdx.x; i <= nv; i += (uint64_t) gridDim.x * blockDim.x) {
        const int64_t lo = i == 0 ? 0 : (int64_t) keys[i - 1] + 1;
        const int64_t hi = i == nv ? (int64_t) n_owned : (int64_t) keys[i];
        for (int64_t t = lo; t <= hi; t++) rowptr[t] = (uint32_t) i;
    }
}

constexpr int SCAN_BLOCK = 256;
constexpr int SCAN_ITEMS = 16;
constexpr int SCAN_TILE = SCAN_BLOCK * SCAN_ITEMS;

__device__ __forceinline__ uint32_t block_exclusive_scan(uint32_t v, uint32_t *total, uint32_t *lds ) {
    const int lane = lane_id(), wave = (int) (threadIdx.x >> 6);
    uint32_t inc = v;
#pragma unroll
    for (int o = 1; o < 64; o <<= 1) { uint32_t t = (uint32_t) __shfl_up((int) inc, o); if (lane >= o) inc += t; }
    if (lane == 63) lds[wave] = inc;
    __syncthreads();
    uint32_t wave_off = 0, tot = 0;
    const int nw = (int) (blockDim.x >> 6);
    for (int w = 0; w < nw; w++) { uint32_t s = lds[w]; if (w < wave) wave_off += s; tot += s; }
    __syncthreads();
    *total = tot;
    return wave_off + inc - v;
}

__global__ void __launch_bounds__(SCAN_BLOCK) k_scan_tile_sums(const uint32_t *__restrict__ in, uint64_t n, uint64_t *__restrict__ tile_sums) {
    __shared__ uint32_t lds[8];
    const uint64_t base = (uint64_t) blockIdx.x * SCAN_TILE;
    uint32_t s = 0;
    if (base + SCAN_TILE <= n && (reinterpret_cast<uintptr_t>(in) & 15u) == 0) {
        const uint4 *in4 = reinterpret_cast<const uint4 *>(in + base);
#pragma unroll
        for (int k = 0; k < SCAN_ITEMS / 4; k++) { const uint4 v = in4[k * SCAN_BLOCK + threadIdx.x]; s += v.x + v.y + v.z + v.w; }
    } else {
        for (int k = 0; k < SCAN_ITEMS; k++) {
            uint64_t i = base + (uint64_t) k * SCAN_BLOCK + threadIdx.x;
            if (i < n) s += in[i];
        }
    }
    uint32_t tot;
    block_exclusive_scan(s, &tot, lds);
    if (threadIdx.x == 0) tile_sums[blockIdx.x] = tot;
}

__global__ void __launch_bounds__(1024) k_scan_spine(uint64_t *tile_sums, uint32_t n_tiles) {
    __shared__ uint64_t lds[1024];
    __shared__ uint64_t carry;
    if (threadIdx.x == 0) carry = 0;
    __syncthreads();
    for (uint32_t base = 0; base < n_tiles; base += 1024) {
        uint32_t i = base + threadIdx.x;
        uint64_t v = i < n_tiles ? tile_sums[i] : 0;
        lds[threadIdx.x] = v;
        __syncthreads();
        for (int o = 1; o < 1024; o <<= 1) {
            uint64_t t = threadIdx.x >= (unsigned) o ? lds[threadIdx.x - o] : 0;
            __syncthreads();
            lds[threadIdx.x] += t;
            __syncthreads();
        }
        uint64_t inc = lds[threadIdx.x];
        uint64_t c = carry;
        if (i < n_tiles) tile_sums[i] = c + inc - v;
        __syncthreads();
        if (threadIdx.x == 1023) carry = c + inc;
        __syncthreads();
    }
    if (threadIdx.x == 0) tile_sums[n_tiles] = carry;
}

__global__ void __launch_bounds__(SCAN_BLOCK) k_scan_tiles(const uint32_t *__restrict__ in, uint64_t n,
                                                            const uint64_t *__restrict__ tile_sums, uint32_t *__restrict__ out) {
    __shared__ uint32_t lds[8];
    const bool full = (uint64_t) (blockIdx.x + 1) * SCAN_TILE <= n && (reinterpret_cast<uintptr_t>(in) & 15u) == 0 && (reinterpret_cast<uintptr_t>(out) & 15u) == 0;
    if (full) {
        constexpr int G = SCAN_ITEMS / 4;
        const int lane = lane_id(), wave = (int) (threadIdx.x >> 6);
        const uint64_t wbase = (uint64_t) blockIdx.x * SCAN_TILE + (uint64_t) wave * (64 * SCAN_ITEMS);
        const uint4 *in4 = reinterpret_cast<const uint4 *>(in + wbase);
        uint4 q[G];
        uint32_t ex[G];
#pragma unroll
        for (int k = 0; k < G; k++) q[k] = in4[k * 64 + lane];
        uint32_t run = 0;
#pragma unroll
        for (int k = 0; k < G; k++) {
            const uint32_t sk = q[k].x + q[k].y + q[k].z + q[k].w;
            uint32_t inc = sk;
#pragma unroll
            for (int o = 1; o < 64; o <<= 1) { const uint32_t t = (uint32_t) __shfl_up((int) inc, o); if (lane >= o) inc += t; }
            ex[k] = run + inc - sk;
            run += (uint32_t) __shfl((int) inc, 63);
        }
        if (lane == 0) lds[wave] = run;
        __syncthreads();
        uint32_t woff = (uint32_t) tile_sums[blockIdx.x];
        for (int w = 0; w < wave; w++) woff += lds[w];
        uint4 *out4 = reinterpret_cast<uint4 *>(out + wbase);
#pragma unroll
        for (int k = 0; k < G; k++) {
            uint32_t e = woff + ex[k];
            uint4 r;
            r.x = e; e += q[k].x; r.y = e; e += q[k].y; r.z = e; e += q[k].z; r.w = e;
            out4[k * 64 + lane] = r;
        }
    } else {
        const uint64_t base = (uint64_t) blockIdx.x * SCAN_TILE + (uint64_t) threadIdx.x * SCAN_ITEMS;
        uint32_t v[SCAN_ITEMS];
        uint32_t s = 0;
#pragma unroll
        for (int k = 0; k < SCAN_ITEMS; k++) { uint64_t i = base + k; v[k] = i < n ? in[i] : 0u; s += v[k]; }
        uint32_t tot;
        uint32_t ex = block_exclusive_scan(s, &tot, lds) + (uint32_t) tile_sums[blockIdx.x];
#pragma unroll
        for (int k = 0; k < SCAN_ITEMS; k++) { uint64_t i = base + k; if (i < n) out[i] = ex; ex += v[k]; }
    }
    if (blockIdx.x == gridDim.x - 1 && threadIdx.x == 0) out[n] = (uint32_t) tile_sums[gridDim.x];
}

__device__ __forceinline__ uint64_t seg_key(unsigned long long val) {
    const uint32_t ol = (uint32_t) (val >> 32);
    return ((uint64_t) (ol_small(ol) ? 0u : 1u) << 63) | ((uint64_t) (uint32_t) ol_len(ol) << 32) | (uint32_t) val;
}

__device__ __forceinline__ bool eq_shifted(const uint32_t *rowA, const uint32_t *rowB, int d, int nnt, int wordsA) {
    const int bit = 2 * d, q = bit >> 5, r = bit & 31;
    const int nbits = 2 * nnt;
// ... 438 lines not shown
template <int NQ>
static void launch_probe_nq(const NodesDev &nd, const PrefSufCfg &cfg, const ProbeTable &t, int local,
                            int32_t src_begin, int32_t src_end, const ProbeOut &o, dim3 grid, dim3 block, hipStream_t s) {
    if (local == 1)      launch_probe_nql<NQ, 1>(nd, cfg, t, src_begin, src_end, o, grid, block, s);
    else if (local == 2) launch_probe_nql<NQ, 2>(nd, cfg, t, src_begin, src_end, o, grid, block, s);
    else                 launch_probe_nql<NQ, 0>(nd, cfg, t, src_begin, src_end, o, grid, block, s);
}

void launch_probe(const NodesDev &nd, const PrefSufCfg &cfg, const unsigned long long *table, uint32_t n_buckets,
                  const uint32_t *filter, uint32_t filter_bits,
                  int32_t src_begin, int32_t src_end, uint32_t *rec_dst, unsigned long long *rec_val, uint64_t rec_cap,
                  unsigned long long *counters, int n_cu, int local, uint32_t *deg, unsigned long long *first, const ProbeBig *big, hipStream_t s) {
    const int64_t ns = (int64_t) src_end - src_begin;
    if (ns <= 0) return;
    const bool second = local && big && big->count > 0;
    dim3 grid((unsigned) probe_blocks(n_cu, second ? (uint64_t) big->count : (uint64_t) ns)), block(PROBE_WAVES * 64);
    ProbeOut o{rec_dst, rec_val, rec_cap, counters, deg, first, src_begin};
    if (local && big) {
        o.big_list = big->list; o.big_list_cap = big->list_cap;
        if (second) {
            const size_t items = (size_t) grid.x * PROBE_WAVES * (size_t) big->item_cap;
            o.big_count = big->count;
            o.bigO = (uint4 *) big->items;
            o.bigC = (uint32_t *) (o.bigO + items * (size_t) local);
            o.bigM = o.bigC + items;
            o.big_cap = big->item_cap;
        }
    }
    ProbeTable t{table, n_buckets, filter_bits ? filter : nullptr, filter_bits ? filter_bits - 1 : 0u};
    const int need_q = (((2 * cfg.Lcap + 31) >> 5) + 3) >> 2;
    const bool aligned = (nd.stride & 3) == 0 && ((uintptr_t) nd.words & 15u) == 0;
    const int row_q = nd.stride >> 2;
    if (aligned && need_q <= 2 && row_q >= 2)      launch_probe_nq<2>(nd, cfg, t, local, src_begin, src_end, o, grid, block, s);
    else if (aligned && need_q <= 3 && row_q >= 3) launch_probe_nq<3>(nd, cfg, t, local, src_begin, src_end, o, grid, block, s);
    else if (aligned && need_q <= 4 && row_q >= 4) launch_probe_nq<4>(nd, cfg, t, local, src_begin, src_end, o, grid, block, s);
    else                                           launch_probe_nq<0>(nd, cfg, t, local, src_begin, src_end, o, grid, block, s);
}

void launch_local_emit(int32_t src_base, int32_t n_src, const uint32_t *deg, const unsigned long long *first, const unsigned long long *second,
                       const uint32_t *rec_dst, const unsigned long long *rec_val, uint64_t n_rec, const uint32_t *rowptr, uint32_t *cursor,
                       alga_edge_dev *edges, const int32_t *record_sources, const unsigned long long *record_sources_count, uint32_t record_sources_cap, hipStream_t s,
                       uint32_t slot_stride) {
    if (n_src <= 0) return;
    if (record_sources) hipLaunchKernelGGL(k_zero_cursors_list, dim3(std::min<unsigned>(grid_for((uint64_t) record_sources_cap, 256), 2048u)), dim3(256), 0, s, record_sources, record_sources_count,
                                           record_sources_cap, src_base, cursor);
    else (void) hipMemsetAsync(cursor, 0, (size_t) (n_src + 1) * sizeof(uint32_t), s);
    hipLaunchKernelGGL(k_local_emit_first, dim3(grid_for((uint64_t) n_src, 256)), dim3(256), 0, s, src_base, n_src, deg, first, second, rowptr, edges, slot_stride);
    if (n_rec) {
        unsigned g = std::min<unsigned>(grid_for(n_rec, 256), 4096u);
        hipLaunchKernelGGL(k_local_emit_records, dim3(std::max(1u, g)), dim3(256), 0, s, src_base, rec_dst, rec_val, n_rec, rowptr, cursor, edges);
    }
    if (record_sources) {
        if (n_rec) hipLaunchKernelGGL(k_sort_rows_list, dim3(std::min<unsigned>(grid_for((uint64_t) record_sources_cap, 256), 2048u)), dim3(256), 0, s, record_sources, record_sources_count,
                                      record_sources_cap, src_base, rowptr, edges);
    } else hipLaunchKernelGGL(k_sort_rows, dim3(grid_for((uint64_t) n_src, 256)), dim3(256), 0, s, n_src, rowptr, edges);
}

void launch_make_keys(const uint32_t *rec_dst, uint64_t n_rec, int32_t dst_begin, int32_t dst_end, uint32_t *keys,
                      unsigned long long *n_valid, hipStream_t s) {
    if (n_rec == 0) return;
    unsigned g = std::min<unsigned>(grid_for(n_rec, 256 * 4), 4096u);
    hipLaunchKernelGGL(k_make_keys, dim3(std::max(1u, g)), dim3(256), 0, s, rec_dst, n_rec, dst_begin, dst_end, keys, n_valid);
}

void launch_rowptr_from_sorted(const uint32_t *keys, const unsigned long long *n_valid_ptr, uint64_t n_rec_max, int32_t n_owned,
                               uint32_t *rowptr, hipStream_t s) {
    unsigned g = std::min<unsigned>(grid_for(n_rec_max + 1, 256), 8192u);
    hipLaunchKernelGGL(k_rowptr_from_sorted, dim3(std::max(1u, g)), dim3(256), 0, s, keys, n_valid_ptr, n_owned, rowptr);
}

size_t scan_scratch_bytes(uint64_t n) {
    uint64_t tiles = (n + SCAN_TILE - 1) / SCAN_TILE;
    return (size_t) (tiles + 2) * sizeof(uint64_t);
}

void launch_exclusive_scan(const uint32_t *in, uint64_t n, uint32_t *out, uint64_t *scratch, hipStream_t s) {
    if (n == 0) { (void) hipMemsetAsync(out, 0, sizeof(uint32_t), s); (void) hipMemsetAsync(scratch, 0, 2 * sizeof(uint64_t), s); return; }
    const uint32_t tiles = (uint32_t) ((n + SCAN_TILE - 1) / SCAN_TILE);
    hipLaunchKernelGGL(k_scan_tile_sums, dim3(tiles), dim3(SCAN_BLOCK), 0, s, in, n, scratch);
    hipLaunchKernelGGL(k_scan_spine, dim3(1), dim3(1024), 0, s, scratch, tiles);
    hipLaunchKernelGGL(k_scan_tiles, dim3(tiles), dim3(SCAN_BLOCK), 0, s, in, n, scratch, out);
}

uint64_t scan_total_index(uint64_t n) { return (n + SCAN_TILE - 1) / SCAN_TILE; }

__global__ void __launch_bounds__(256) k_mail(MailArgs a, uint32_t *__restrict__ dst) {
    for (int i = 0; i < a.n; i++)
        for (uint32_t w = threadIdx.x; w < a.seg[i].words; w += 256) dst[a.seg[i].dst + w] = a.seg[i].src[w];
}

void launch_mail(const MailArgs &a, uint32_t *host_block_dev, hipStream_t s) {
    if (a.n > 0) hipLaunchKernelGGL(k_mail, dim3(1), dim3(256), 0, s, a, host_block_dev);
}

int reduce_targets_per_block(uint64_t n_records, uint64_t n_targets) {
    const double avg = n_targets ? (double) n_records / (double) n_targets : 0.0;
    int tpb = avg > 0 ? (int) (0.6 * RED_CAP / avg) : RED_BLOCK;
    return std::max(16, std::min(RED_BLOCK, tpb));
}

void launch_gather_heads(const NodesDev &nd, const unsigned long long *seg_val, const unsigned long long *n_valid_ptr, uint64_t n_rec_max,
                         void *heads, hipStream_t s) {
    if (n_rec_max == 0) return;
    unsigned g = std::min<unsigned>(grid_for(n_rec_max, 256), 16384u);
    hipLaunchKernelGGL(k_gather_heads, dim3(std::max(1u, g)), dim3(256), 0, s, nd, seg_val, n_valid_ptr, (uint4 *) heads);
}

void launch_reduce_targets(const NodesDev &nd, const PrefSufCfg &cfg, int32_t dst_begin, int32_t n_owned, int32_t targets_per_block,
                           const uint32_t *rowptr, unsigned long long *seg_val, const void *heads, uint32_t *out_cnt, uint32_t *outdeg,
                           unsigned long long *counters, hipStream_t s) {
    if (n_owned <= 0) return;
    dim3 grid(grid_for((uint64_t) n_owned, targets_per_block)), block(RED_BLOCK);
    if (cfg.stats)
        hipLaunchKernelGGL(k_reduce_targets<true>, grid, block, 0, s, nd, cfg, dst_begin, n_owned, targets_per_block, rowptr, seg_val,
                           (const uint4 *) heads, out_cnt, outdeg, counters);
    else
        hipLaunchKernelGGL(k_reduce_targets<false>, grid, block, 0, s, nd, cfg, dst_begin, n_owned, targets_per_block, rowptr, seg_val,
                           (const uint4 *) heads, out_cnt, outdeg, counters);
}

void launch_scatter_by_source(const PrefSufCfg &cfg, int32_t dst_begin, int32_t n_owned, const uint32_t *rowptr,
                              const unsigned long long *seg_val, const uint32_t *out_cnt, const uint32_t *out_rowptr, uint32_t *out_cursor,
                              alga_edge_dev *edges, hipStream_t s) {
    if (n_owned <= 0) return;
    hipLaunchKernelGGL(k_scatter_by_source, dim3(grid_for((uint64_t) n_owned, 256)), dim3(256), 0, s, cfg, dst_begin, n_owned, rowptr, seg_val,
                       out_cnt, out_rowptr, out_cursor, edges);
}

void launch_edges_to_keys(const alga_edge_dev *e, uint64_t n, unsigned long long *keys, uint32_t *vals, hipStream_t s) {
    if (n == 0) return;
    hipLaunchKernelGGL(k_edges_to_keys, dim3(std::min<unsigned>(grid_for(n, 256), 8192u)), dim3(256), 0, s, e, n, keys, vals);
}

void launch_keys_to_edges(const unsigned long long *keys, const uint32_t *vals, uint64_t n, alga_edge_dev *e, hipStream_t s) {
    if (n == 0) return;
    hipLaunchKernelGGL(k_keys_to_edges, dim3(std::min<unsigned>(grid_for(n, 256), 8192u)), dim3(256), 0, s, keys, vals, n, e);
}

void launch_sort_rows(int32_t n, const uint32_t *out_rowptr, alga_edge_dev *edges, hipStream_t s) {
    if (n <= 0) return;
    hipLaunchKernelGGL(k_sort_rows, dim3(grid_for((uint64_t) n, 256)), dim3(256), 0, s, n, out_rowptr, edges);
}

}
```

alga_amd/csrc/prefsuf_pile.hip:

```cpp
#include <hip/hip_runtime.h>
#include <algorithm>
#include "prefsuf_common.h"
#include "prefsuf_kernels.h"
#include "prefsuf_device.h"
#include "prefsuf_cluster_device.h"

namespace alga {

constexpr int PB_TILE = 192, PB_HALO = 64, PB_THREADS = PB_TILE + PB_HALO;
constexpr int PILE_SW = 13;
constexpr int PILE_MAXSUB = 4;
constexpr int PILE_EQ = 3;

__device__ __forceinline__ bool pile_declines(const unsigned long long *pile_cnt) { return pile_cnt_declines(pile_cnt); }

__device__ __forceinline__ void load_row9(const NodesDev &nd, uint32_t id, uint32_t (&row)[9]) {
    const uint32_t *rp = nd.words + (size_t) id * nd.stride;
    if ((nd.stride & 3) == 0 && nd.stride >= 12 && ((uintptr_t) nd.words & 15u) == 0) {
        const uint4 v0 = reinterpret_cast<const uint4 *>(rp)[0], v1 = reinterpret_cast<const uint4 *>(rp)[1];
        row[0] = v0.x; row[1] = v0.y; row[2] = v0.z; row[3] = v0.w; row[4] = v1.x; row[5] = v1.y; row[6] = v1.z; row[7] = v1.w;
        row[8] = rp[8];
    } else {
#pragma unroll
        for (int k = 0; k < 9; k++) row[k] = k < nd.stride ? rp[k] : 0u;
    }
}

template <bool SAMPLE>
__global__ void __launch_bounds__(PB_THREADS, 6) k_pile_build(NodesDev nd, const uint32_t *__restrict__ skeys, const uint32_t *__restrict__ sids, uint64_t n_entries, const uint4 *__restrict__ dir, ClusterCfg cc, int U,
                                                           uint4 *__restrict__ rec, uint4 *__restrict__ tab, uint32_t epoch,
                                                           uint4 *__restrict__ side, unsigned long long *__restrict__ pile_cnt, uint32_t *__restrict__ own_mask) {
    if (!SAMPLE && pile_declines(pile_cnt)) return;
    const int idx_shift = cc.idx_shift, kk = cc.kk;
    __shared__ uint32_t sRow[PB_THREADS][PILE_SW];
    __shared__ unsigned long long sKm[PB_THREADS];
    __shared__ unsigned long long sLead[PB_THREADS];
    __shared__ unsigned long long sRm[PB_THREADS];
    __shared__ uint32_t sMin[PB_THREADS], sMax[PB_THREADS];
    __shared__ uint32_t sBad[PB_THREADS];
    __shared__ uint8_t sTag[PB_THREADS];
    __shared__ uint32_t sCount[3];
    const int t = (int) threadIdx.x;
    const uint64_t base = (uint64_t) blockIdx.x * PB_TILE;
    const uint64_t j = base + (uint64_t) t;
    const bool have = j < n_entries;
    const uint64_t jc = have ? j : (n_entries ? n_entries - 1 : 0);
    const uint32_t key = skeys[jc], node_id = min(sids[jc], (uint32_t) nd.n - 1u);
    const uint32_t meta = key >> (cc.idx_shift - CL_MBITS);
    const bool tgt = have && key != 0xFFFFFFFFu;
    uint4 drec = make_uint4(0u, 0u, 0u, 0u);
    if (tgt) drec = dir[key >> idx_shift];
    const uint64_t e0 = drec.x;
    const uint32_t cnt = drec.y;
    const bool owned = tgt && e0 >= base && e0 < base + PB_TILE && e0 <= j && j - e0 < (uint64_t) cnt;
    const int s = owned ? (int) (e0 - base) : 0;
    const int i = owned ? (int) (j - e0) : 0;
    const bool part = owned && cnt <= 64u;
    uint32_t row[9] = {0u, 0u, 0u, 0u, 0u, 0u, 0u, 0u, 0u};
    if (part) load_row9(nd, node_id, row);
    sLead[t] = 0ull; sRm[t] = 0ull; sMin[t] = 0xFFFFFFFFu; sMax[t] = 0u; sBad[t] = 0u;
    if (t < 3) sCount[t] = 0u;
    __syncthreads();
    const int m = (int) (meta & 63u);
    uint32_t A[PILE_SW];
    {
        const int w0 = (2 * m) >> 5, sh = (2 * m) & 31;
        const int lo = 2 * (64 - m), hi = lo + 2 * U;
        uint32_t Rp[18];
#pragma unroll
        for (int k = 0; k < 18; k++) Rp[k] = 0u;
#pragma unroll
        for (int k = 0; k < 9; k++) Rp[4 + k] = row[k];
        uint32_t m1 = 0u - (uint32_t) (w0 & 1), m2 = 0u - (uint32_t) ((w0 >> 1) & 1);
        asm volatile("" : "+v"(m1), "+v"(m2));
        uint32_t y1[PILE_SW + 3], y[PILE_SW + 1];
#pragma unroll
        for (int k = 0; k < PILE_SW + 3; k++) y1[k] = (Rp[k + 1] & m1) | (Rp[k] & ~m1);
#pragma unroll
        for (int k = 0; k <= PILE_SW; k++) y[k] = (y1[k + 2] & m2) | (y1[k] & ~m2);
#pragma unroll
        for (int k = 0; k < PILE_SW; k++) A[k] = funnel(y[k], y[k + 1], sh) & low_bits32(hi - 32 * k) & ~low_bits32(lo - 32 * k);
    }
    const unsigned long long kmask = kk >= 32 ? ~0ull : ((1ull << (2 * kk)) - 1ull);
    const unsigned long long kmer = (((unsigned long long) A[5] << 32) | A[4]) & kmask;
    sKm[t] = kmer;
#pragma unroll
    for (int k = 0; k < PILE_SW; k++) sRow[t][k] = A[k];
    __syncthreads();
    int L = t;
    if (part) {
        for (int u = 0; u < i; u++) if (sKm[s + u] == kmer) { L = s + u; break; }
        if (L == t) {
            atomicOr(&sLead[s], 1ull << i);
            sTag[t] = (uint8_t) (cluster_key(kmer_hash((uint32_t) kmer & cc.lo_mask, (uint32_t) (kmer >> 32) & cc.hi_mask), idx_shift - CL_MBITS) & 31u);
        }
        atomicMin(&sMin[L], ((uint32_t) m << 16) | (uint32_t) t);
        atomicMax(&sMax[L], ((uint32_t) m << 16) | (uint32_t) t);
        const unsigned long long bit = 1ull << (63 - m);
        if (atomicOr(&sRm[L], bit) & bit) atomicOr(&sBad[s], 1u);
    }
    __syncthreads();
    uint32_t *sSlot = reinterpret_cast<uint32_t *>(sKm);
    int my_slot = -1, my_rank = 0;
    if (part) {
        const unsigned long long lm = sLead[s];
        const int kgrp = __popcll(lm & ((1ull << (L - s)) - 1ull));
        if (kgrp < PILE_MAXSUB) {
            int before = 0;
            unsigned long long rest = lm;
#pragma unroll
            for (int g = 0; g < PILE_MAXSUB - 1; g++) {
                if (g < kgrp) { before += __popcll(sRm[s + __builtin_ctzll(rest)]); rest &= rest - 1ull; }
            }
            my_rank = m == 0 ? 0 : __popcll(sRm[L] >> (64 - m));
            my_slot = s + before + my_rank;
            if (my_slot < s + (int) cnt) sSlot[my_slot] = node_id; else my_slot = -1;
        }
    }
    uint32_t S[PILE_SW];
#pragma unroll
    for (int k = 0; k < PILE_SW; k++) S[k] = 0u;
    if (part) {
        const int t0 = (int) (sMax[L] & 0xFFFFu), t1 = (int) (sMin[L] & 0xFFFFu);
        const int lo = 2 * (64 - m), hi = lo + 2 * U;
        uint32_t diff = 0u;
#pragma unroll
        for (int k = 0; k < PILE_SW; k++) {
            S[k] = sRow[t0][k] | sRow[t1][k];
            diff |= (A[k] ^ S[k]) & low_bits32(hi - 32 * k) & ~low_bits32(lo - 32 * k);
        }
        if (diff != 0u) atomicOr(&sBad[s], 1u);
    }
    __syncthreads();
    if (owned) {
        uint4 *line = tab + (size_t) (key >> idx_shift) * 8;
        if (!part) {
            if (i == 0) {
                if (!SAMPLE) { line[3] = make_uint4(0u, 0u, 0u, (1u << 22) | (epoch << 23)); line[4] = make_uint4(127u, drec.x, drec.z, drec.w); }
                atomicAdd(&sCount[0], 1u); atomicAdd(&sCount[1], 1u);
            }
        } else {
            const unsigned long long lm = sLead[s];
            const int nsub = __popcll(lm);
            const int iL = L - s;
            const int k = __popcll(lm & ((1ull << iL) - 1ull));
            if (!SAMPLE) {
                const unsigned long long right = m == 0 ? 0ull : (sRm[L] >> (64 - m));
                uint32_t succ_id = 0xFFFFFFFFu, delta = 0u;
                if (right != 0ull && my_slot > s && my_rank >= 1) { succ_id = sSlot[my_slot - 1]; delta = 1u + (uint32_t) __builtin_ctzll(right); }
                const bool first_group = (k == 0 || own_mask != nullptr) && k < PILE_MAXSUB && sBad[s] == 0u && nsub <= PILE_MAXSUB;
                const bool leftmost = first_group && t == (int) (sMax[L] & 0xFFFFu);
                side[j] = make_uint4(node_id, succ_id, delta | ((uint32_t) m << 8) | ((uint32_t) k << 16) | (leftmost ? 0x40000000u : 0u) | (first_group ? 0x80000000u : 0u),
                                     k == 0 ? key >> idx_shift : (uint32_t) (e0 + (uint64_t) k));
                if (!first_group && own_mask) atomicOr(&own_mask[j >> 5], 1u << (j & 31u));
            }
            if (!SAMPLE && L == t && k >= 1 && k < PILE_MAXSUB) {
                const unsigned long long rm = sRm[t];
                const uint64_t slot = e0 + (uint64_t) k;
                rec[slot * 4 + 0] = make_uint4(S[0], S[1], S[2], S[3]);
                rec[slot * 4 + 1] = make_uint4(S[4], S[5], S[6], S[7]);
                rec[slot * 4 + 2] = make_uint4(S[8], S[9], S[10], S[11]);
                rec[slot * 4 + 3] = make_uint4(S[12], 0u, (uint32_t) rm, (uint32_t) (rm >> 32));
            }
            if (i == 0) {
                uint32_t tg[PILE_MAXSUB] = {0u, 0u, 0u, 0u};
                unsigned long long rest = lm;
#pragma unroll
                for (int g = 0; g < PILE_MAXSUB; g++) {
                    if (rest) { tg[g] = sTag[s + __builtin_ctzll(rest)]; rest &= rest - 1ull; }
                }
                const bool irregular = sBad[s] != 0u || nsub > PILE_MAXSUB;
                const uint32_t ns1 = (uint32_t) (nsub < PILE_MAXSUB ? nsub : PILE_MAXSUB) - 1u;
                if (!SAMPLE) {
                    const unsigned long long rm = sRm[t];
                    line[0] = make_uint4(S[0], S[1], S[2], S[3]);
                    line[1] = make_uint4(S[4], S[5], S[6], S[7]);
                    line[2] = make_uint4(S[8], S[9], S[10], S[11]);
                    line[3] = make_uint4(S[12], (uint32_t) rm, (uint32_t) (rm >> 32), tg[0] | (tg[1] << 5) | (tg[2] << 10) | (tg[3] << 15) | (ns1 << 20) | (irregular ? 1u << 22 : 0u) | (epoch << 23));
                }
                atomicAdd(&sCount[0], 1u);
                if (irregular) atomicAdd(&sCount[1], 1u);
            }
            if (!SAMPLE && L == s && t == (int) (sMax[s] & 0xFFFFu)) {
                line[4] = make_uint4(cnt, drec.x, drec.z, drec.w);
                line[5] = make_uint4(sSlot[s], sMin[s] >> 16, 0u, 0u);
            }
        }
    }
    if (!SAMPLE && have && t < PB_TILE && !(tgt && cnt <= 64u)) {
        side[j] = make_uint4(node_id, 0xFFFFFFFFu, 0u, 0u);
        if (own_mask) atomicOr(&own_mask[j >> 5], 1u << (j & 31u));
    }
    if (SAMPLE && owned) atomicAdd(&sCount[2], 1u);
    __syncthreads();
    if (SAMPLE && t < 3 && sCount[t]) atomicAdd(&pile_cnt[t], (unsigned long long) sCount[t]);
}

constexpr int PILE_RUNS = 8;
__device__ __forceinline__ void pile_list_store(uint4 *line, uint32_t entries, bool ok, int n, const uint32_t (&key)[PILE_RUNS], const uint32_t (&kc)[PILE_RUNS], uint32_t c1_last) {
    uint32_t *lw = reinterpret_cast<uint32_t *>(line);
    if (ok) {
        line[5] = make_uint4(key[0], key[1], key[2], key[3]);
        line[6] = make_uint4(key[4], key[5], key[6], key[7]);
        line[7] = make_uint4(kc[0] | (kc[1] << 16), kc[2] | (kc[3] << 16), kc[4] | (kc[5] << 16), kc[6] | (kc[7] << 16));
        bool dup = false;
#pragma unroll
        for (int a = 0; a < PILE_RUNS; a++)
#pragma unroll
            for (int b = a + 1; b < PILE_RUNS; b++) dup = dup || (b < n && key[a] == key[b]);
        lw[16] = (entries & 255u) | ((uint32_t) n << 8) | ((c1_last & 255u) << 16) | (dup ? 0x80000000u : 0u);
    } else lw[16] = entries & 255u;
}

__global__ void __launch_bounds__(256) k_pile_runs(const uint4 *__restrict__ side, uint64_t n_entries, uint32_t n_buckets, uint4 *__restrict__ tab, const uint2 *__restrict__ runs,
                                                   int n_nodes, int nwin, const unsigned long long *__restrict__ pile_cnt) {
    if (pile_declines(pile_cnt)) return;
    const uint64_t j = (uint64_t) blockIdx.x * 256 + threadIdx.x;
    if (j >= n_entries) return;
    const uint4 sd = side[j];
    if (((sd.z >> 30) & 1u) == 0u) return;
    uint4 *line = tab + (size_t) min(sd.w, n_buckets) * 8;
    const uint4 l4 = line[4], l5 = line[5];
    const uint4 *r0 = reinterpret_cast<const uint4 *>(runs + (size_t) min(sd.x, (uint32_t) n_nodes - 1u) * CL_RMAX);
    const uint4 *r1 = reinterpret_cast<const uint4 *>(runs + (size_t) min(l5.x, (uint32_t) n_nodes - 1u) * CL_RMAX);
    const uint4 a0 = r0[0], a1 = r0[1], a2 = r0[2], a3 = r0[3], b0 = r1[0], b1 = r1[1], b2 = r1[2];
    const int s0 = -(int) ((sd.z >> 8) & 63u), s1 = -(int) (l5.y & 63u), seam = s0 + nwin;
    const uint32_t k0[CL_RMAX] = {a0.x, a0.z, a1.x, a1.z, a2.x, a2.z, a3.x, a3.z}, y0[CL_RMAX] = {a0.y, a0.w, a1.y, a1.w, a2.y, a2.w, a3.y, a3.w};
    const uint32_t k1[6] = {b0.x, b0.z, b1.x, b1.z, b2.x, b2.z}, y1[6] = {b0.y, b0.w, b1.y, b1.w, b2.y, b2.w};
    const int nr0 = (int) (y0[0] >> 24), nr1 = (int) (y1[0] >> 24);
    bool ok = nr0 >= 1 && nr0 <= CL_RMAX && nr1 >= 1 && nr1 <= 6 && s1 <= seam;
    uint32_t ok_[PILE_RUNS], kc_[PILE_RUNS];
#pragma unroll
    for (int k = 0; k < PILE_RUNS; k++) { ok_[k] = 0u; kc_[k] = 0u; }
    int n = 0;
    uint32_t last_key = 0u, last_pos = 0xFFFFFFFFu, c1_last = 0u;
#pragma unroll
    for (int r = CL_RMAX - 1; r >= 0; r--) {
        if (ok && r < nr0) {
            const uint32_t kpos = (uint32_t) (s0 + (int) (y0[r] & 255u) + 64), c0 = (uint32_t) (s0 + (int) ((y0[r] >> 8) & 255u) + 64), c1 = (uint32_t) (s0 + (int) ((y0[r] >> 16) & 255u) + 64);
#pragma unroll
            for (int k = 0; k < PILE_RUNS; k++) if (k == n) { ok_[k] = k0[r]; kc_[k] = kpos | (c0 << 8); }
            last_key = k0[r]; last_pos = kpos; c1_last = c1;
            n++;
        }
    }
#pragma unroll
    for (int r = 5; r >= 0; r--) {
        if (ok && r < nr1) {
            const int c1i = s1 + (int) ((y1[r] >> 16) & 255u);
            if (c1i > seam) {
                const int c0i = max(s1 + (int) ((y1[r] >> 8) & 255u), seam);
                const uint32_t kpos = (uint32_t) (s1 + (int) (y1[r] & 255u) + 64), c1 = (uint32_t) (c1i + 64);
                if (n >= 1 && k1[r] == last_key && kpos == last_pos) c1_last = c1;
                else {
#pragma unroll
                    for (int k = 0; k < PILE_RUNS; k++) if (k == n) { ok_[k] = k1[r]; kc_[k] = kpos | ((uint32_t) (c0i + 64) << 8); }
                    last_key = k1[r]; last_pos = kpos; c1_last = c1;
                    n++;
                }
            }
        }
    }
    ok = ok && n >= 1 && n <= PILE_RUNS;
    pile_list_store(line, l4.x, ok, n, ok_, kc_, c1_last);
}

constexpr int PR_TILE = 3072;
constexpr int PR_TKW = 21;
constexpr int PR_RCAP = 14;
__global__ void __launch_bounds__(TK_ROWS) k_pile_runs_consensus(const uint4 *__restrict__ side, uint64_t n_entries, uint32_t n_buckets, uint4 *__restrict__ tab, const uint4 *__restrict__ rec,
                                                                 uint4 *__restrict__ rec2, ClusterCfg cc, int U, int Lmin,
                                                                 const unsigned long long *__restrict__ pile_cnt, uint32_t *__restrict__ own_mask) {
    if (pile_declines(pile_cnt)) return;
    __shared__ uint32_t s[TK_ROWS][PR_TKW];
    __shared__ uint32_t stk[2 * (NR_STACK + 1)][TK_ROWS];
    __shared__ uint16_t rbuf[PR_RCAP + 1][TK_ROWS];
    __shared__ uint32_t sList[PR_TILE];
    __shared__ uint32_t sN;
    const int t = (int) threadIdx.x;
    if (t == 0) sN = 0u;
    __syncthreads();
    const uint64_t base = (uint64_t) blockIdx.x * PR_TILE;
#pragma unroll
    for (int q = 0; q < PR_TILE / TK_ROWS; q++) {
        const uint64_t j = base + (uint64_t) q * TK_ROWS + (uint64_t) t;
        if (j < n_entries) {
            const uint4 sd = side[j];
            if ((sd.z >> 30) & 1u) sList[atomicAdd(&sN, 1u)] = ((sd.z >> 16) & 3u) == 0u ? min(sd.w, n_buckets) : (uint32_t) min((uint64_t) sd.w, n_entries) | 0x80000000u;
        }
    }
    __syncthreads();
    const int np = (int) sN;
    const int fs = cc.idx_shift - CL_MBITS;
    const int step = max(16, min(64, cc.w) & ~15);
    for (int c0 = 0; c0 < np; c0 += TK_ROWS) {
        const bool in = c0 + t < np;
        const uint32_t who = sList[in ? c0 + t : 0];
        const bool further = (who >> 31) != 0u;
        const uint32_t slot = who & 0x7FFFFFFFu;
        uint4 *line = tab + (size_t) (further ? 0u : who) * 8;
        const uint4 *src = further ? rec + (size_t) slot * 4 : (const uint4 *) line;
        uint32_t S[PILE_SW + 1];
        unsigned long long rm = 0ull;
        {
            const uint4 l0 = src[0], l1 = src[1], l2 = src[2], l3 = src[3];
            S[0] = l0.x; S[1] = l0.y; S[2] = l0.z; S[3] = l0.w; S[4] = l1.x; S[5] = l1.y; S[6] = l1.z; S[7] = l1.w;
            S[8] = l2.x; S[9] = l2.y; S[10] = l2.z; S[11] = l2.w; S[12] = l3.x; S[13] = 0u;
            rm = !in ? 0ull : (further ? (((unsigned long long) l3.w << 32) | l3.z) : (((unsigned long long) l3.z << 32) | l3.y));
        }
        const bool act = in && rm != 0ull;
        const int m_min = act ? __clzll((long long) rm) : 0, m_max = act ? 63 - __builtin_ctzll(rm) : 0;
        const int len_v = U + m_max - m_min;
        const int nwin = len_v - Lmin + 1;
        {
            const int ob = 2 * (64 - m_max), w0 = ob >> 5, sh = ob & 31;
            uint32_t m1 = 0u - (uint32_t) (w0 & 1), m2 = 0u - (uint32_t) ((w0 >> 1) & 1), m4 = 0u - (uint32_t) ((w0 >> 2) & 1);
            asm volatile("" : "+v"(m1), "+v"(m2), "+v"(m4));
            uint32_t y1[PILE_SW + 1], y2[PILE_SW + 1], y[PILE_SW + 1];
#pragma unroll
            for (int k = 0; k <= PILE_SW; k++) y1[k] = ((k + 1 <= PILE_SW ? S[k + 1] : 0u) & m1) | (S[k] & ~m1);
#pragma unroll
            for (int k = 0; k <= PILE_SW; k++) y2[k] = ((k + 2 <= PILE_SW ? y1[k + 2] : 0u) & m2) | (y1[k] & ~m2);
#pragma unroll
            for (int k = 0; k <= PILE_SW; k++) y[k] = ((k + 4 <= PILE_SW ? y2[k + 4] : 0u) & m4) | (y2[k] & ~m4);
#pragma unroll
            for (int k = 0; k < PR_TKW; k++) s[t][k] = k < PILE_SW ? funnel(y[k], y[k + 1], sh) : 0u;
        }
        int nr = 0;
        bool uncovered = false, stack_ovf = false;
        uint32_t cur0 = 0u;
        node_runs_core<true, PR_RCAP>(s[t], nwin, act, cc, stk, rbuf, t, nr, uncovered, stack_ovf, cur0, step);
        bool ok = act && nr >= 1 && nr <= PR_RCAP && !uncovered && !stack_ovf;
        uint32_t key_[PILE_RUNS], kc_[PILE_RUNS];
#pragma unroll
        for (int k = 0; k < PILE_RUNS; k++) { key_[k] = 0u; kc_[k] = 0u; }
        int n = 0;
        uint32_t last_q = 0xFFFFFFFFu;
        const int nrs = nr < PR_RCAP ? nr : PR_RCAP;
        for (int r = PR_RCAP - 1; r >= 0; r--) {
            if (ok && r < nrs) {
                const uint32_t d = rbuf[r][t];
                const int q = (int) (d & 255u), p0 = (int) (d >> 8);
                if ((uint32_t) q != last_q) {
                    uint32_t h, pk;
                    kmer_key(s[t], q < 192 ? q : 0, true, cc, h, pk);
                    const uint32_t kv = cluster_key(h, fs), cv = (uint32_t) (q - m_max + 64) | ((uint32_t) (p0 - m_max + 64) << 8);
#pragma unroll
                    for (int k = 0; k < PILE_RUNS; k++) if (k == n) { key_[k] = kv; kc_[k] = cv; }
                    n++;
                    last_q = (uint32_t) q;
                }
            }
        }
        ok = ok && n >= 1 && n <= PILE_RUNS;
        if (in && further) {
            uint4 *l2 = rec2 + (size_t) slot * 4 - 4;
            pile_list_store(l2, 0u, ok, n, key_, kc_, (uint32_t) (nwin - m_max + 64));
            if (!ok) {
                const uint64_t jb = slot >= 3u ? (uint64_t) slot - 3u : 0ull;
                for (uint64_t j2 = jb; j2 < jb + 64u + 3u && j2 < n_entries; j2++) {
                    const uint4 s2 = side[j2];
                    if ((s2.z >> 31) && ((s2.z >> 16) & 3u) != 0u && s2.w == slot) atomicOr(&own_mask[j2 >> 5], 1u << (j2 & 31u));
                }
            }
        } else if (in) {
            uint32_t *lw = reinterpret_cast<uint32_t *>(line);
            pile_list_store(line, lw[16], ok, n, key_, kc_, (uint32_t) (nwin - m_max + 64));
            if (!ok) {
                lw[16] = lw[16] & 255u;
                const uint32_t cntb = min(lw[16] & 255u, 64u), e0b = lw[17];
                for (uint32_t i2 = 0; i2 < cntb; i2++) {
                    const uint64_t j2 = (uint64_t) e0b + i2;
                    if (j2 < n_entries) { const uint4 s2 = side[j2]; if ((s2.z >> 31) && ((s2.z >> 16) & 3u) == 0u) atomicOr(&own_mask[j2 >> 5], 1u << (j2 & 31u)); }
                }
            }
        }
    }
}

__global__ void __launch_bounds__(256) k_pile_own_ids(const uint32_t *__restrict__ own_mask, const uint32_t *__restrict__ sids, uint64_t n_entries, int32_t *__restrict__ out, uint32_t cap,
                                                      unsigned long long *__restrict__ count, const unsigned long long *__restrict__ pile_cnt) {
    if (pile_declines(pile_cnt)) return;
    __shared__ uint32_t sTot, sBase;
    const uint64_t words = (n_entries + 31) / 32;
    const uint64_t w0 = (uint64_t) blockIdx.x * 1024 + threadIdx.x;
    uint32_t mw[4];
    uint32_t mine = 0u;
#pragma unroll
    for (int q = 0; q < 4; q++) { const uint64_t w = w0 + (uint64_t) q * 256; mw[q] = w < words ? own_mask[w] : 0u; mine += (uint32_t) __popc(mw[q]); }
    if (threadIdx.x == 0) sTot = 0u;
    __syncthreads();
    const uint32_t at = atomicAdd(&sTot, mine);
    __syncthreads();
    if (threadIdx.x == 0) sBase = (uint32_t) atomicAdd(count, (unsigned long long) sTot);
    __syncthreads();
    uint32_t o = sBase + at;
#pragma unroll
    for (int q = 0; q < 4; q++) {
        const uint64_t w = w0 + (uint64_t) q * 256;
        uint32_t m = mw[q];
        while (m) {
            const int b = __builtin_ctz(m);
            m &= m - 1u;
            const uint64_t j = w * 32 + (uint64_t) b;
            if (j < n_entries && o < cap) out[o] = (int32_t) sids[j];
            o++;
        }
    }
}

__global__ void __launch_bounds__(256) k_pile_list_check(const uint4 *__restrict__ side, uint64_t n_entries, uint32_t n_buckets, const uint4 *__restrict__ tab, const uint4 *__restrict__ rec2,
                                                         uint32_t epoch, const uint2 *__restrict__ runs, int n_nodes, int nwin, unsigned long long *__restrict__ out ,
                                                         const unsigned long long *__restrict__ pile_cnt) {
    if (pile_declines(pile_cnt)) return;
    const uint64_t j = (uint64_t) blockIdx.x * 256 + threadIdx.x;
    if (j >= n_entries) return;
    const uint4 sd = side[j];
    if ((sd.z >> 31) == 0u) return;
    const bool further = ((sd.z >> 16) & 3u) != 0u;
    const uint4 *line = further ? rec2 + (size_t) min((uint64_t) sd.w, n_entries - 1) * 4 - 4 : tab + (size_t) min(sd.w, n_buckets) * 8;
    const uint4 l4 = line[4];
    if (!further) { const uint4 l3 = line[3]; if ((l3.w >> 23) != epoch || ((l3.w >> 22) & 1u)) return; }
    const int npr = (int) ((l4.x >> 8) & 15u);
    if (npr == 0) return;
    const uint32_t *lw = reinterpret_cast<const uint32_t *>(line);
    const uint2 *own = runs + (size_t) min(sd.x, (uint32_t) n_nodes - 1u) * CL_RMAX;
    const int code = (int) (own[0].y >> 24);
    if (code == 0 || code == CL_RUNS_FLAGGED) return;
    const int nown = code < CL_RMAX ? code : CL_RMAX;
    const int sB = 64 - (int) ((sd.z >> 8) & 63u);
    bool bad = false;
    int r = nown - 1;
    for (int a = 0; a < npr && a < PILE_RUNS; a++) {
        const uint32_t vx = lw[20 + a], pq = (lw[28 + (a >> 1)] >> (16 * (a & 1))) & 0xFFFFu;
        const uint32_t pqn = a + 1 < npr ? (lw[28 + ((a + 1) >> 1)] >> (16 * ((a + 1) & 1))) & 0xFFFFu : 0u;
        const int kpos = (int) (pq & 255u), c0 = (int) (pq >> 8), c1 = a + 1 < npr ? (int) (pqn >> 8) : (int) ((l4.x >> 16) & 255u);
        const int p0 = max(c0, sB) - sB, p1 = min(c1, sB + nwin) - sB;
        if (p0 >= p1) continue;
        if (r < 0) { bad = true; break; }
        const uint2 o = own[r];
        const int oq = (int) (o.y & 255u), op0 = (int) ((o.y >> 8) & 255u), op1 = (int) ((o.y >> 16) & 255u);
        bad = bad || o.x != vx || oq != kpos - sB || op0 != p0 || op1 != p1;
        r--;
    }
    bad = bad || r >= 0;
    atomicAdd(&out[0], 1ull);
    if (bad) atomicAdd(&out[1], 1ull);
}

__device__ __forceinline__ unsigned long long smear_up(unsigned long long x, int g ) {
    unsigned long long acc = 0ull, pw = x;
    int done = 0;
#pragma unroll
    for (int b = 0; b < 6; b++) {
        if ((g >> b) & 1) { acc |= pw << (done + 1); done += 1 << b; }
        pw |= pw << (1 << b);
    }
    return acc;
}
// ... 308 lines not shown
        for (int k = 0; k < CL_RMAX; k++) p1_home = (((vmask >> k) & 1u) != 0u && ((ry[k] >> 8) & 255u) == 0u) ? (int) ((ry[k] >> 16) & 255u) : p1_home;
        const bool by_succ = d1 < p1_home && (int) (my.z & 255u) == d1 && my.y != 0xFFFFFFFFu;
#ifdef PP_LK
        const int d2 = nkept == 2 ? 63 - __clzll((long long) kept) : -1;
        const int dA = by_succ ? d2 : d1, dB = by_succ ? -1 : d2;
        uint32_t idA = 0xFFFFFFFFu, idB = 0xFFFFFFFFu;
        if (dA >= 0) idA = lookup(dA);
        if (dB >= 0) idB = lookup(dB);
        const uint32_t id1 = by_succ ? my.y : idA;
        const uint32_t id2 = by_succ ? idA : idB;
        bool two = false;
        if (nkept == 2) {
#else
        const uint32_t id1 = by_succ ? my.y : lookup(d1);
        uint32_t id2 = 0u;
        int d2 = 0;
        bool two = false;
        if (nkept == 2) {
            d2 = 63 - __clzll((long long) kept);
            id2 = lookup(d2);
#endif
            const int ds0 = U - cfg.rsoemo + 1;
            const unsigned long long lowm = ds0 <= 0 ? 0ull : (ds0 >= 64 ? ~0ull : ((1ull << ds0) - 1ull));
            two = d2 < ds0 || __popcll(occ & ((1ull << d2) - 1ull) & ~lowm) < 3;
        }
        if (id1 == 0xFFFFFFFFu || (nkept == 2 && id2 == 0xFFFFFFFFu)) dfr = true;
        else {
            slot_val = ((unsigned long long) id1 << 32) | (uint32_t) d1 | (two ? 0x100u : 0u);
            if (two) o.second[Bs - o.src_base] = ((unsigned long long) id2 << 32) | (uint32_t) d2;
            st_rec += two ? 2 : 1;
        }
    }
    if (have) o.first[Bs - o.src_base] = slot_val;
    dfr = dfr && nr_code != 0;
    const uint64_t dm = __ballot(dfr);
    if (dm != 0ull) {
        if (dfr) sDefer[wave][n_defer + (int) __builtin_amdgcn_mbcnt_hi((uint32_t) (dm >> 32), __builtin_amdgcn_mbcnt_lo((uint32_t) dm, 0u))] = Bs;
        n_defer += __popcll(dm);
        wave_lds_fence();
        if (n_defer >= 64) flush_defer();
    }
    }
    flush_defer();
    st_rec = wave_sum_u64(st_rec);
    if (lane == 0 && st_rec) atomicAdd(&o.counters[CNT_VALID_RECORDS], (unsigned long long) st_rec);
}

__global__ void __launch_bounds__(256) k_pile_deg(int32_t n, unsigned long long *__restrict__ first, uint32_t *__restrict__ deg, const unsigned long long *__restrict__ pile_cnt) {
    if (pile_declines(pile_cnt)) return;
    const int64_t i = (int64_t) blockIdx.x * 256 + threadIdx.x;
    if (i >= n) return;
    const unsigned long long f = first[i];
    if (f == LOCAL_FIRST_NONE || deg[i] != 0u) return;
    deg[i] = 1u + (uint32_t) ((f >> 8) & 1ull);
    if (f & 0x100ull) first[i] = f & ~0x100ull;
}

bool pile_plan(const PrefSufCfg &cfg, const ClusterCfg &cc, int eq, int uniform_len, bool masks) {
    if (eq != PILE_EQ || uniform_len <= 0 || masks || cfg.stats) return false;
    if (uniform_len > 144 || blocks_of(uniform_len) > 9) return false;
    if (uniform_len - cfg.Lmin + 1 > 64 || cc.w > 64 || cc.w < 16 || cc.kk > 32 || cc.kk < 1) return false;
    return true;
}
size_t pile_record_bytes(uint64_t n) { return (size_t) (n + 2) * 64; }

size_t pile_table_bytes(uint32_t n_buckets) { return ((size_t) n_buckets + 2) * 128; }

__global__ void k_pile_sample_close(unsigned long long *__restrict__ pile_cnt) {
    const unsigned long long by_entries = pile_cnt[2] / 8ull;
    if (by_entries > pile_cnt[0]) pile_cnt[0] = by_entries;
}

__global__ void k_pile_sample_force(unsigned long long *__restrict__ pile_cnt, unsigned long long buckets, unsigned long long irregular) { pile_cnt[0] = buckets; pile_cnt[1] = irregular; }

void launch_pile_sample(const NodesDev &nd, const ClusterCfg &cc, int uniform_len, const uint32_t *skeys, const uint32_t *sids, const void *dir, unsigned long long *pile_cnt,
                        int no_sample, hipStream_t s) {
    (void) hipMemsetAsync(pile_cnt, 0, PILE_CNT_WORDS * sizeof(unsigned long long), s);
    const uint64_t n_entries = nd.n > 0 ? (uint64_t) nd.n : 0;
    if (no_sample == 2) hipLaunchKernelGGL(k_pile_sample_force, dim3(1), dim3(1), 0, s, pile_cnt, 100ull, 1ull);
    if (n_entries == 0 || no_sample) return;
    const uint64_t tiles = (n_entries + PB_TILE - 1) / PB_TILE;
    const dim3 sample((unsigned) std::max<uint64_t>(1, std::min<uint64_t>(tiles, std::max<uint64_t>(64, tiles / 32)))), block(PB_THREADS);
    hipLaunchKernelGGL((k_pile_build<true>), sample, block, 0, s, nd, skeys, sids, n_entries, (const uint4 *) dir, cc, uniform_len, (uint4 *) nullptr, (uint4 *) nullptr, 0u, (uint4 *) nullptr, pile_cnt,
                       (uint32_t *) nullptr);
    hipLaunchKernelGGL(k_pile_sample_close, dim3(1), dim3(1), 0, s, pile_cnt);
}

void launch_pile_build(const NodesDev &nd, const PrefSufCfg &cfg, const ClusterCfg &cc, int uniform_len, const uint32_t *skeys, const uint32_t *sids, const void *dir, void *rec, void *rec2,
                       void *tab, uint32_t epoch, void *side, const void *runs, int nwin, const unsigned long long *pile_cnt, uint32_t *own_mask, hipStream_t s) {
    const uint64_t n_entries = nd.n > 0 ? (uint64_t) nd.n : 0;
    if (n_entries == 0) return;
    const uint64_t tiles = (n_entries + PB_TILE - 1) / PB_TILE;
    if (own_mask) (void) hipMemsetAsync(own_mask, 0, pile_own_mask_bytes(n_entries), s);
    hipLaunchKernelGGL((k_pile_build<false>), dim3((unsigned) tiles), dim3(PB_THREADS), 0, s, nd, skeys, sids, n_entries, (const uint4 *) dir, cc, uniform_len, (uint4 *) rec, (uint4 *) tab, epoch,
                       (uint4 *) side, const_cast<unsigned long long *>(pile_cnt), own_mask);
    if (own_mask)
        hipLaunchKernelGGL(k_pile_runs_consensus, dim3((unsigned) ((n_entries + PR_TILE - 1) / PR_TILE)), dim3(TK_ROWS), 0, s, (const uint4 *) side, n_entries, cc.n_buckets, (uint4 *) tab,
                           (const uint4 *) rec, (uint4 *) rec2, cc, uniform_len, cfg.Lmin, pile_cnt, own_mask);
    else
        hipLaunchKernelGGL(k_pile_runs, dim3((unsigned) ((n_entries + 255) / 256)), dim3(256), 0, s, (const uint4 *) side, n_entries, cc.n_buckets, (uint4 *) tab, (const uint2 *) runs, nd.n, nwin, pile_cnt);
}

size_t pile_own_mask_bytes(uint64_t n) { return (size_t) ((n + 31) / 32 + 1024) * 4; }

void launch_pile_own_ids(const uint32_t *own_mask, const uint32_t *sids, uint64_t n_entries, int32_t *list, uint32_t cap, unsigned long long *pile_cnt, hipStream_t s) {
    if (n_entries == 0) return;
    const uint64_t words = (n_entries + 31) / 32;
    hipLaunchKernelGGL(k_pile_own_ids, dim3((unsigned) ((words + 1023) / 1024)), dim3(256), 0, s, own_mask, sids, n_entries, list, cap, pile_cnt + 3, (const unsigned long long *) pile_cnt);
}

void launch_pile_check(const void *side, uint64_t n_entries, uint32_t n_buckets, const void *tab, const void *rec2, uint32_t epoch, const void *runs, int n_nodes, int nwin,
                       unsigned long long *pile_cnt, hipStream_t s) {
    if (n_entries == 0) return;
    hipLaunchKernelGGL(k_pile_list_check, dim3((unsigned) ((n_entries + 255) / 256)), dim3(256), 0, s, (const uint4 *) side, n_entries, n_buckets, (const uint4 *) tab, (const uint4 *) rec2, epoch,
                       (const uint2 *) runs,
                       n_nodes, nwin, pile_cnt + 4, (const unsigned long long *) pile_cnt);
}

constexpr int PSR_IPT = 4;
__global__ void __launch_bounds__(256) k_pile_side_range(const uint4 *__restrict__ side, uint64_t n_entries, uint32_t src_begin, uint32_t src_end, uint4 *__restrict__ out,
                                                         uint64_t out_cap, unsigned long long *__restrict__ cursor, const unsigned long long *__restrict__ pile_cnt) {
    if (pile_declines(pile_cnt)) return;
    __shared__ uint32_t cnt[PSR_IPT * 4];
    __shared__ unsigned long long base;
    const int wave = (int) (threadIdx.x >> 6);
    const uint64_t b0 = (uint64_t) blockIdx.x * (256 * PSR_IPT);
    uint4 v[PSR_IPT];
    uint32_t before[PSR_IPT];
    bool in[PSR_IPT];
#pragma unroll
    for (int k = 0; k < PSR_IPT; k++) {
        const uint64_t j = b0 + (uint64_t) k * 256 + threadIdx.x;
        v[k] = j < n_entries ? side[j] : make_uint4(0xFFFFFFFFu, 0u, 0u, 0u);
        in[k] = j < n_entries && v[k].x >= src_begin && v[k].x < src_end;
        const uint64_t m = __ballot(in[k]);
        before[k] = (uint32_t) __builtin_amdgcn_mbcnt_hi((uint32_t) (m >> 32), __builtin_amdgcn_mbcnt_lo((uint32_t) m, 0u));
        if ((threadIdx.x & 63u) == 0u) cnt[k * 4 + wave] = (uint32_t) __popcll(m);
    }
    __syncthreads();
    if (threadIdx.x == 0) {
        uint32_t tot = 0;
        for (int i = 0; i < PSR_IPT * 4; i++) tot += cnt[i];
        base = tot ? atomicAdd(cursor, (unsigned long long) tot) : 0ull;
    }
    __syncthreads();
    uint32_t run = 0;
#pragma unroll
    for (int k = 0; k < PSR_IPT; k++) {
        uint32_t mine = run;
        for (int w = 0; w < 4; w++) { if (w < wave) mine += cnt[k * 4 + w]; run += cnt[k * 4 + w]; }
        const unsigned long long at = base + mine + before[k];
        if (in[k] && at < out_cap) out[at] = v[k];
    }
}

void launch_pile_probe(const NodesDev &nd, const PrefSufCfg &cfg, const ClusterCfg &cc, int uniform_len, const void *tab, uint32_t epoch, const void *rec, const void *rec2,
                       const void *side, const void *runs, unsigned long long *counters, uint32_t *deg, unsigned long long *first, unsigned long long *second,
                       int32_t *defer_list, uint32_t defer_cap, const unsigned long long *pile_cnt, int n_cu, hipStream_t s, int32_t src_begin, int32_t src_end,
                       void *side_range, unsigned long long *cursor) {
    const uint64_t n_entries = nd.n > 0 ? (uint64_t) nd.n : 0;
    if (n_entries == 0 || src_end <= src_begin) return;
    ProbeOut o{};
    o.counters = counters; o.deg = deg; o.first = first; o.second = second; o.src_base = src_begin;
    uint64_t n_mine = n_entries;
    const void *side_src = side;
    if (src_begin != 0 || src_end != nd.n) {
        n_mine = (uint64_t) (src_end - src_begin);
        (void) hipMemsetAsync(cursor, 0, sizeof(unsigned long long), s);
        hipLaunchKernelGGL(k_pile_side_range, dim3((unsigned) ((n_entries + 256 * PSR_IPT - 1) / (256 * PSR_IPT))), dim3(256), 0, s, (const uint4 *) side, n_entries,
                           (uint32_t) src_begin, (uint32_t) src_end, (uint4 *) side_range, n_mine, cursor, pile_cnt);
        side_src = side_range;
    }
    const uint64_t tiles = (n_mine + PP_WAVES * 64 - 1) / (PP_WAVES * 64);
    const dim3 grid((unsigned) std::max<uint64_t>(1, std::min<uint64_t>(tiles, (uint64_t) std::max(1, n_cu) * (PP_OCC * 4 / PP_WAVES)))), block(PP_WAVES * 64);
    hipLaunchKernelGGL(k_pile_probe, grid, block, 0, s, cfg, cc, uniform_len, nd, n_entries, n_mine, nd.n, (const uint4 *) tab, epoch, (const uint4 *) rec, (const uint4 *) rec2,
                       (const uint4 *) side, (const uint4 *) side_src, (const uint2 *) runs, o, defer_list, defer_cap, pile_cnt);
}

void launch_pile_deg(int32_t n, unsigned long long *first, uint32_t *deg, const unsigned long long *pile_cnt, hipStream_t s) {
    if (n <= 0) return;
    hipLaunchKernelGGL(k_pile_deg, dim3((unsigned) (((int64_t) n + 255) / 256)), dim3(256), 0, s, n, first, deg, pile_cnt);
}

}
```

Before: 4.716 billion edges/s.

## Compact pile consensus work via per-tile lists and fold pile degree into scan

The pile build kernel now records which piles each tile owns into a compact per-tile list with counts. A new list-driven consensus kernel processes only those entries instead of scanning every side entry, using a strided shared-memory row layout that the templated row_word/kmer_key helpers support. Separately, the pile degree fix-up is deferred and folded into the first pass of the outdegree exclusive scan, which removes one kernel pass over outdeg and loc_first. This costs an extra list buffer and more complex indexing, and the deferred degree update has to run before any fallback probe that reads it.

```diff
diff --git a/alga_amd/csrc/engine.hip b/alga_amd/csrc/engine.hip
--- a/alga_amd/csrc/engine.hip
+++ b/alga_amd/csrc/engine.hip
@@ -108,6 +108,7 @@
     if ((rc = alga_ensure(e, e->cl_pile_succ, ((size_t) n + 64) * 16))) return rc;
     if ((rc = alga_ensure(e, e->cl_pile_cnt, PILE_CNT_WORDS * sizeof(unsigned long long)))) return rc;
     if ((rc = alga_ensure(e, e->cl_pile_own, pile_own_mask_bytes(n)))) return rc;
+    if (e->opt_pile_runs_list && (rc = alga_ensure(e, e->cl_pile_list, pile_list_bytes(n)))) return rc;
     if ((rc = alga_ensure(e, e->cl_defer, (size_t) (n + 64) * sizeof(int32_t)))) return rc;
     const void *before = e->cl_pile_tab.p;
     const size_t cap_before = e->cl_pile_tab.cap;
@@ -133,6 +134,7 @@
     e->pairs_timed = false;
     e->store_timed = false;
     e->pile_timed = false;
+    e->pile_deg_pending = false;
     const bool all_sources = src_begin == 0 && src_end == pp.nd.n;
     const bool pile_index_left = e->opt_pile_range != 0 && e->pile_n == pp.nd.n && e->pile_words == (const void *) pp.nd.words;
     bool pile = clustered && e->opt_pile != 0 && e->opt_cluster_pairs != 0 && e->opt_cluster_order != 0 && pp.local_sw == 1 &&
@@ -195,6 +197,7 @@
                 if (rc == ALGA_ERR_OUT_OF_MEMORY) {
                     (void) hipGetLastError();
                     alga_release(e->cl_pile_tab); alga_release(e->cl_pile_rec); alga_release(e->cl_pile_rec2); alga_release(e->cl_pile_succ); alga_release(e->cl_pile_own);
+                    alga_release(e->cl_pile_list);
                     e->pile_epoch = 0; e->pile_n = -1;
                     e->err.clear();
                     pile = false;
@@ -224,7 +227,7 @@
                 const bool from_consensus = e->opt_pile_runs != 0;
                 launch_pile_build(nd, cfg, cc, pp.uniform_len, (const uint32_t *) e->cl_keys[1].p, (const uint32_t *) e->cl_vals[1].p, e->cl_dir.p, e->cl_pile_rec.p, e->cl_pile_rec2.p, e->cl_pile_tab.p,
                                   e->pile_epoch, e->cl_pile_succ.p, e->cl_runs.p, pp.uniform_len - cfg.Lmin + 1, (const unsigned long long *) e->cl_pile_cnt.p,
-                                  from_consensus ? (uint32_t *) e->cl_pile_own.p : nullptr, s);
+                                  from_consensus ? (uint32_t *) e->cl_pile_own.p : nullptr, (from_consensus && e->opt_pile_runs_list) ? e->cl_pile_list.p : nullptr, s);
                 if ((rc = alga_check_launch(e, "k_pile_build"))) return rc;
                 if (keys_only) {
                     launch_pile_own_ids((const uint32_t *) e->cl_pile_own.p, (const uint32_t *) e->cl_vals[1].p, (uint64_t) nd.n, (int32_t *) e->cl_defer.p, (uint32_t) nd.n,
@@ -311,7 +314,8 @@
                                        cap, cnt, e->n_cu, (uint32_t *) e->outdeg.p, (unsigned long long *) e->loc_first.p, &big, cnt + CNT_DEFERRED, 1, s,
                                        (const uint32_t *) e->cl_keys[1].p, (const uint32_t *) e->cl_vals[1].p, pp.uniform_len,
                                        (piled && e->opt_pile_skip_gather) ? (const unsigned long long *) e->cl_pile_cnt.p : nullptr);
-                if (piled) launch_pile_deg((int32_t) n_src, (unsigned long long *) e->loc_first.p, (uint32_t *) e->outdeg.p, (const unsigned long long *) e->cl_pile_cnt.p, s);
+                e->pile_deg_pending = piled && e->opt_pile_deg_fold != 0;
+                if (piled && !e->pile_deg_pending) launch_pile_deg((int32_t) n_src, (unsigned long long *) e->loc_first.p, (uint32_t *) e->outdeg.p, (const unsigned long long *) e->cl_pile_cnt.p, s);
             } else {
                 launch_probe_clustered(nd, cfg, cc, pp.cluster_eq, e->cl_store.p, e->cl_dir.p, e->cl_runs.p, (const uint8_t *) e->cl_nruns.p, src_begin,
                                        src_end, nullptr, src_begin, (uint32_t *) e->rec_dst.p, (unsigned long long *) e->rec_val.p, cap, cnt, e->n_cu,
@@ -339,6 +343,10 @@
             if ((rc = alga_ensure(e, e->loc_big_items, probe_big_bytes(e->n_cu, big.count, pp.local_sw, big.item_cap)))) return rc;
             big.items = e->loc_big_items.p;
             if (!have_table && (rc = build_table())) return rc;
+            if (e->pile_deg_pending) {
+                launch_pile_deg((int32_t) n_src, (unsigned long long *) e->loc_first.p, (uint32_t *) e->outdeg.p, (const unsigned long long *) e->cl_pile_cnt.p, s);
+                e->pile_deg_pending = false;
+            }
             HIP_TRY(e, hipMemsetAsync(cnt + CNT_LOCAL_OVERFLOW, 0, sizeof(unsigned long long), s));
             launch_probe(nd, cfg, (const unsigned long long *) e->table.p, n_buckets, (const uint32_t *) e->filter.p, filter_bits, src_begin, src_end,
                          (uint32_t *) e->rec_dst.p, (unsigned long long *) e->rec_val.p, cap, cnt, e->n_cu, pp.local_sw, (uint32_t *) e->outdeg.p,
@@ -468,7 +476,12 @@
     if ((rc = alga_ensure(e, e->out_cnt, (size_t) (n_src + 1) * sizeof(uint32_t)))) return rc;
     HIP_TRY(e, hipEventRecord(e->ev[EV_GROUP], s));
     HIP_TRY(e, hipEventRecord(e->ev[EV_REDUCE], s));
-    launch_exclusive_scan((const uint32_t *) e->outdeg.p, n_src, (uint32_t *) e->out_rowptr.p, (uint64_t *) e->scan_scratch.p, s);
+    if (e->pile_deg_pending)
+        launch_exclusive_scan_pile_deg((uint32_t *) e->outdeg.p, n_src, (uint32_t *) e->out_rowptr.p, (uint64_t *) e->scan_scratch.p, (unsigned long long *) e->loc_first.p,
+                                       (const unsigned long long *) e->cl_pile_cnt.p, s);
+    else
+        launch_exclusive_scan((const uint32_t *) e->outdeg.p, n_src, (uint32_t *) e->out_rowptr.p, (uint64_t *) e->scan_scratch.p, s);
+    e->pile_deg_pending = false;
     if ((rc = alga_check_launch(e, "scan(outdeg)"))) return rc;
     const uint64_t E = e->stats.records;
     if (E >= (1ull << 32) - 16) return alga_fail(e, ALGA_ERR_CAPACITY, "more than 2^32 edges; shard the input");
@@ -615,6 +628,10 @@
         e->opt_pile = (value == 2 || value == 3) ? (int) value : (value != 0);
     } else if (!strcmp(name, "pile_runs")) {
         e->opt_pile_runs = value != 0;
+    } else if (!strcmp(name, "pile_runs_list")) {
+        e->opt_pile_runs_list = value != 0;
+    } else if (!strcmp(name, "pile_deg_fold")) {
+        e->opt_pile_deg_fold = value != 0;
     } else if (!strcmp(name, "pile_check")) {
         e->opt_pile_check = value != 0;
     } else if (!strcmp(name, "pile_skip_gather")) {
diff --git a/alga_amd/csrc/engine_internal.h b/alga_amd/csrc/engine_internal.h
--- a/alga_amd/csrc/engine_internal.h
+++ b/alga_amd/csrc/engine_internal.h
@@ -55,6 +55,10 @@
     int    opt_pile_skip_gather = 1;
     int    opt_pile = 1;
     int    opt_pile_runs = 1;
+    int    opt_pile_runs_list = 1;
+    DevBuf cl_pile_list;
+    int    opt_pile_deg_fold = 1;
+    bool   pile_deg_pending = false;
     int    opt_pile_check = 0;
     bool   expect_pairwise = false;
     DevBuf cl_pile_side_r, cl_pile_cursor;
diff --git a/alga_amd/csrc/prefsuf_cluster_device.h b/alga_amd/csrc/prefsuf_cluster_device.h
--- a/alga_amd/csrc/prefsuf_cluster_device.h
+++ b/alga_amd/csrc/prefsuf_cluster_device.h
@@ -58,9 +58,16 @@
     e0 = rec.x + b0; cnt = b1 - b0;
 }
 
+template <int RS = 1, int RW = 0>
+__device__ __forceinline__ uint32_t row_word(const uint32_t *row, int k) {
+    if (RW > 0) { const uint32_t v = row[(k < RW ? k : RW - 1) * RS]; return k < RW ? v : 0u; }
+    return row[k * RS];
+}
+
+template <int RS = 1, int RW = 0>
 __device__ __forceinline__ void kmer_key(const uint32_t *row, int i, bool valid, const ClusterCfg &cc, uint32_t &h, uint32_t &pk) {
     const int bit = 2 * i, q = bit >> 5, r = bit & 31;
-    const uint32_t x0 = row[q], x1 = row[q + 1], x2 = row[q + 2];
+    const uint32_t x0 = row_word<RS, RW>(row, q), x1 = row_word<RS, RW>(row, q + 1), x2 = row_word<RS, RW>(row, q + 2);
     const uint32_t lo = funnel(x0, x1, r) & cc.lo_mask;
     h = kmer_hash(lo, funnel(x1, x2, r) & cc.hi_mask);
     pk = valid ? order_key(h, lo, i) : 0xFFFFFFFFu;
@@ -69,14 +76,15 @@
 constexpr int TK_ROWS = 128;
 constexpr int NR_STACK = 8;
 
-template <bool WIDE, int RCAP = CL_RMAX>
+template <bool WIDE, int RCAP = CL_RMAX, int RS = 1, int RW = 0>
 __device__ __forceinline__ void node_runs_core(const uint32_t *row, int nwin, bool act, const ClusterCfg &cc, uint32_t (*stk)[TK_ROWS], uint16_t (*rbuf)[TK_ROWS], int t,
                                                int &nr, bool &uncovered, bool &stack_ovf, uint32_t &cur0, int step = 64) {
     constexpr int S0 = NR_STACK + 1;
     const int w = cc.w;
     nr = 0; uncovered = false; stack_ovf = false; cur0 = 0xFFFFFFFFu;
     for (int hb = (WIDE && nwin > step) ? ((nwin - 1) / step) * step : 0; hb >= 0; hb -= step) {
-        const uint32_t *rowh = row + (hb >> 4);
+        const int h0 = hb >> 4;
+        auto rowh = [&](int k) -> uint32_t { return row_word<RS, RW>(row, h0 + k); };
         const int nwh = !WIDE ? nwin : (nwin - hb < step ? nwin - hb : step);
         const int nk = act ? nwh - 1 + w : 0;
         uint64_t m_lo, m_hi;
@@ -84,7 +92,7 @@
             uint32_t dm[4];
 #pragma unroll
             for (int d = 0; d < 4; d++) {
-                const uint32_t x0 = rowh[2 * d], x1 = rowh[2 * d + 1], x2 = rowh[2 * d + 2];
+                const uint32_t x0 = rowh(2 * d), x1 = rowh(2 * d + 1), x2 = rowh(2 * d + 2);
                 dm[d] = compress_even(class0_mask16(x0, x1)) | (compress_even(class0_mask16(x1, x2)) << 16);
             }
             m_lo = (uint64_t) dm[0] | ((uint64_t) dm[1] << 32);
@@ -96,7 +104,7 @@
         uint64_t b1 = w >= 64 ? m_hi : ((m_lo >> w) | (m_hi << (64 - w)));
         auto key_at = [&](int pos) -> uint32_t {
             const int bit = 2 * pos, q = bit >> 5, r = bit & 31;
-            const uint32_t x0 = rowh[q], x1 = rowh[q + 1], x2 = rowh[q + 2];
+            const uint32_t x0 = rowh(q), x1 = rowh(q + 1), x2 = rowh(q + 2);
             return order_key0(kmer_hash(funnel(x0, x1, r) & cc.lo_mask, funnel(x1, x2, r) & cc.hi_mask), pos);
         };
         uint32_t cur1 = 0xFFFFFFFFu;
diff --git a/alga_amd/csrc/prefsuf_kernels.h b/alga_amd/csrc/prefsuf_kernels.h
--- a/alga_amd/csrc/prefsuf_kernels.h
+++ b/alga_amd/csrc/prefsuf_kernels.h
@@ -68,9 +68,11 @@
                               unsigned long long *pile_cnt , int no_sample, hipStream_t s);
 constexpr int PILE_CNT_WORDS = 6;
 size_t     pile_own_mask_bytes(uint64_t n);
+size_t     pile_list_bytes(uint64_t n);
 void       launch_pile_build(const NodesDev &nd, const PrefSufCfg &cfg, const ClusterCfg &cc, int uniform_len, const uint32_t *skeys, const uint32_t *sids, const void *dir, void *rec,
                              void *rec2 , void *tab, uint32_t epoch, void *side, const void *runs, int nwin, const unsigned long long *pile_cnt,
-                             uint32_t *own_mask , hipStream_t s);
+                             uint32_t *own_mask ,
+                             void *plist , hipStream_t s);
 void       launch_pile_own_ids(const uint32_t *own_mask, const uint32_t *sids, uint64_t n_entries, int32_t *list, uint32_t cap, unsigned long long *pile_cnt, hipStream_t s);
 void       launch_pile_check(const void *side, uint64_t n_entries, uint32_t n_buckets, const void *tab, const void *rec2, uint32_t epoch, const void *runs, int n_nodes, int nwin,
                              unsigned long long *pile_cnt, hipStream_t s);
@@ -110,6 +112,7 @@
 size_t   scan_scratch_bytes(uint64_t n);
 uint64_t scan_total_index(uint64_t n);
 void launch_exclusive_scan(const uint32_t *in, uint64_t n, uint32_t *out, uint64_t *scratch, hipStream_t s);
+void launch_exclusive_scan_pile_deg(uint32_t *deg, uint64_t n, uint32_t *out, uint64_t *scratch, unsigned long long *first, const unsigned long long *pile_cnt, hipStream_t s);
 constexpr int MAIL_SEGS = 6;
 struct MailSeg { const uint32_t *src; uint32_t words, dst; };
 struct MailArgs {
diff --git a/alga_amd/csrc/prefsuf_kernels.hip b/alga_amd/csrc/prefsuf_kernels.hip
--- a/alga_amd/csrc/prefsuf_kernels.hip
+++ b/alga_amd/csrc/prefsuf_kernels.hip
@@ -3,6 +3,7 @@
 #include "prefsuf_common.h"
 #include "prefsuf_kernels.h"
 #include "prefsuf_device.h"
+#include "prefsuf_cluster_device.h"
 
 namespace alga {
 
@@ -566,6 +567,45 @@
     if (threadIdx.x == 0) tile_sums[blockIdx.x] = tot;
 }
 
+__device__ __forceinline__ uint32_t pile_deg_one(unsigned long long *first, uint64_t i, uint32_t d) {
+    const unsigned long long f = first[i];
+    if (f == LOCAL_FIRST_NONE || d != 0u) return d;
+    if (f & 0x100ull) first[i] = f & ~0x100ull;
+    return 1u + (uint32_t) ((f >> 8) & 1ull);
+}
+__global__ void __launch_bounds__(SCAN_BLOCK) k_scan_tile_sums_pile_deg(uint32_t *__restrict__ deg, uint64_t n, uint64_t *__restrict__ tile_sums, unsigned long long *__restrict__ first,
+                                                                         const unsigned long long *__restrict__ pile_cnt) {
+    __shared__ uint32_t lds[8];
+    const bool move = !pile_cnt_declines(pile_cnt);
+    const uint64_t base = (uint64_t) blockIdx.x * SCAN_TILE;
+    uint32_t s = 0;
+    if (base + SCAN_TILE <= n && (reinterpret_cast<uintptr_t>(deg) & 15u) == 0) {
+        uint4 *d4 = reinterpret_cast<uint4 *>(deg + base);
+#pragma unroll
+        for (int k = 0; k < SCAN_ITEMS / 4; k++) {
+            uint4 v = d4[k * SCAN_BLOCK + threadIdx.x];
+            if (move) {
+                const uint64_t i = base + 4 * ((uint64_t) k * SCAN_BLOCK + threadIdx.x);
+                const uint4 w = make_uint4(pile_deg_one(first, i, v.x), pile_deg_one(first, i + 1, v.y), pile_deg_one(first, i + 2, v.z), pile_deg_one(first, i + 3, v.w));
+                if (w.x != v.x || w.y != v.y || w.z != v.z || w.w != v.w) { d4[k * SCAN_BLOCK + threadIdx.x] = w; v = w; }
+            }
+            s += v.x + v.y + v.z + v.w;
+        }
+    } else {
+        for (int k = 0; k < SCAN_ITEMS; k++) {
+            const uint64_t i = base + (uint64_t) k * SCAN_BLOCK + threadIdx.x;
+            if (i < n) {
+                uint32_t v = deg[i];
+                if (move) { const uint32_t w = pile_deg_one(first, i, v); if (w != v) { deg[i] = w; v = w; } }
+                s += v;
+            }
+        }
+    }
+    uint32_t tot;
+    block_exclusive_scan(s, &tot, lds);
+    if (threadIdx.x == 0) tile_sums[blockIdx.x] = tot;
+}
+
 __global__ void __launch_bounds__(1024) k_scan_spine(uint64_t *tile_sums, uint32_t n_tiles) {
     __shared__ uint64_t lds[1024];
     __shared__ uint64_t carry;
@@ -1170,6 +1210,14 @@
     hipLaunchKernelGGL(k_scan_tiles, dim3(tiles), dim3(SCAN_BLOCK), 0, s, in, n, scratch, out);
 }
 
+void launch_exclusive_scan_pile_deg(uint32_t *deg, uint64_t n, uint32_t *out, uint64_t *scratch, unsigned long long *first, const unsigned long long *pile_cnt, hipStream_t s) {
+    if (n == 0) { launch_exclusive_scan(deg, n, out, scratch, s); return; }
+    const uint32_t tiles = (uint32_t) ((n + SCAN_TILE - 1) / SCAN_TILE);
+    hipLaunchKernelGGL(k_scan_tile_sums_pile_deg, dim3(tiles), dim3(SCAN_BLOCK), 0, s, deg, n, scratch, first, pile_cnt);
+    hipLaunchKernelGGL(k_scan_spine, dim3(1), dim3(1024), 0, s, scratch, tiles);
+    hipLaunchKernelGGL(k_scan_tiles, dim3(tiles), dim3(SCAN_BLOCK), 0, s, (const uint32_t *) deg, n, scratch, out);
+}
+
 uint64_t scan_total_index(uint64_t n) { return (n + SCAN_TILE - 1) / SCAN_TILE; }
 
 __global__ void __launch_bounds__(256) k_mail(MailArgs a, uint32_t *__restrict__ dst) {
diff --git a/alga_amd/csrc/prefsuf_pile.hip b/alga_amd/csrc/prefsuf_pile.hip
--- a/alga_amd/csrc/prefsuf_pile.hip
+++ b/alga_amd/csrc/prefsuf_pile.hip
@@ -13,6 +13,10 @@
 constexpr int PILE_EQ = 3;
 
 __device__ __forceinline__ bool pile_declines(const unsigned long long *pile_cnt) { return pile_cnt_declines(pile_cnt); }
+
+__device__ __forceinline__ uint32_t pile_who(uint32_t group, uint32_t w, uint32_t n_buckets, uint64_t n_entries) {
+    return group == 0u ? min(w, n_buckets) : (uint32_t) min((uint64_t) w, n_entries) | 0x80000000u;
+}
 
 __device__ __forceinline__ void load_row9(const NodesDev &nd, uint32_t id, uint32_t (&row)[9]) {
     const uint32_t *rp = nd.words + (size_t) id * nd.stride;
@@ -29,7 +33,8 @@
 template <bool SAMPLE>
 __global__ void __launch_bounds__(PB_THREADS, 6) k_pile_build(NodesDev nd, const uint32_t *__restrict__ skeys, const uint32_t *__restrict__ sids, uint64_t n_entries, const uint4 *__restrict__ dir, ClusterCfg cc, int U,
                                                            uint4 *__restrict__ rec, uint4 *__restrict__ tab, uint32_t epoch,
-                                                           uint4 *__restrict__ side, unsigned long long *__restrict__ pile_cnt, uint32_t *__restrict__ own_mask) {
+                                                           uint4 *__restrict__ side, unsigned long long *__restrict__ pile_cnt, uint32_t *__restrict__ own_mask,
+                                                           uint32_t *__restrict__ plist, uint32_t *__restrict__ pcount) {
     if (!SAMPLE && pile_declines(pile_cnt)) return;
     const int idx_shift = cc.idx_shift, kk = cc.kk;
     __shared__ uint32_t sRow[PB_THREADS][PILE_SW];
@@ -40,6 +45,7 @@
     __shared__ uint32_t sBad[PB_THREADS];
     __shared__ uint8_t sTag[PB_THREADS];
     __shared__ uint32_t sCount[3];
+    __shared__ uint32_t sPiles;
     const int t = (int) threadIdx.x;
     const uint64_t base = (uint64_t) blockIdx.x * PB_TILE;
     const uint64_t j = base + (uint64_t) t;
@@ -60,6 +66,7 @@
     if (part) load_row9(nd, node_id, row);
     sLead[t] = 0ull; sRm[t] = 0ull; sMin[t] = 0xFFFFFFFFu; sMax[t] = 0u; sBad[t] = 0u;
     if (t < 3) sCount[t] = 0u;
+    if (t == 0) sPiles = 0u;
     __syncthreads();
     const int m = (int) (meta & 63u);
     uint32_t A[PILE_SW];
@@ -152,6 +159,7 @@
                 const bool leftmost = first_group && t == (int) (sMax[L] & 0xFFFFu);
                 side[j] = make_uint4(node_id, succ_id, delta | ((uint32_t) m << 8) | ((uint32_t) k << 16) | (leftmost ? 0x40000000u : 0u) | (first_group ? 0x80000000u : 0u),
                                      k == 0 ? key >> idx_shift : (uint32_t) (e0 + (uint64_t) k));
+                if (leftmost && plist) plist[(size_t) blockIdx.x * PB_THREADS + atomicAdd(&sPiles, 1u)] = pile_who((uint32_t) k, k == 0 ? key >> idx_shift : (uint32_t) (e0 + (uint64_t) k), cc.n_buckets, n_entries);
                 if (!first_group && own_mask) atomicOr(&own_mask[j >> 5], 1u << (j & 31u));
             }
             if (!SAMPLE && L == t && k >= 1 && k < PILE_MAXSUB) {
@@ -193,6 +201,7 @@
     }
     if (SAMPLE && owned) atomicAdd(&sCount[2], 1u);
     __syncthreads();
+    if (!SAMPLE && plist && t == 0) pcount[blockIdx.x] = sPiles;
     if (SAMPLE && t < 3 && sCount[t]) atomicAdd(&pile_cnt[t], (unsigned long long) sCount[t]);
 }
 
@@ -268,6 +277,95 @@
 constexpr int PR_TILE = 3072;
 constexpr int PR_TKW = 21;
 constexpr int PR_RCAP = 14;
+constexpr int PR_SEGS = 32;
+
+template <int RS, int RW>
+__device__ __forceinline__ void pile_consensus_one(uint32_t who, bool in, uint32_t *row, uint32_t (*stk)[TK_ROWS], uint16_t (*rbuf)[TK_ROWS], int t, const uint4 *__restrict__ side,
+                                                   uint64_t n_entries, uint4 *__restrict__ tab, const uint4 *__restrict__ rec, uint4 *__restrict__ rec2, const ClusterCfg &cc, int U,
+                                                   int Lmin, uint32_t *__restrict__ own_mask) {
+    const int fs = cc.idx_shift - CL_MBITS;
+    const int step = max(16, min(64, cc.w) & ~15);
+    const bool further = (who >> 31) != 0u;
+    const uint32_t slot = who & 0x7FFFFFFFu;
+    uint4 *line = tab + (size_t) (further ? 0u : who) * 8;
+    const uint4 *src = further ? rec + (size_t) slot * 4 : (const uint4 *) line;
+    uint32_t S[PILE_SW + 1];
+    unsigned long long rm = 0ull;
+    {
+        const uint4 l0 = src[0], l1 = src[1], l2 = src[2], l3 = src[3];
+        S[0] = l0.x; S[1] = l0.y; S[2] = l0.z; S[3] = l0.w; S[4] = l1.x; S[5] = l1.y; S[6] = l1.z; S[7] = l1.w;
+        S[8] = l2.x; S[9] = l2.y; S[10] = l2.z; S[11] = l2.w; S[12] = l3.x; S[13] = 0u;
+        rm = !in ? 0ull : (further ? (((unsigned long long) l3.w << 32) | l3.z) : (((unsigned long long) l3.z << 32) | l3.y));
+    }
+    const bool act = in && rm != 0ull;
+    const int m_min = act ? __clzll((long long) rm) : 0, m_max = act ? 63 - __builtin_ctzll(rm) : 0;
+    const int len_v = U + m_max - m_min;
+    const int nwin = len_v - Lmin + 1;
+    {
+        const int ob = 2 * (64 - m_max), w0 = ob >> 5, sh = ob & 31;
+        uint32_t m1 = 0u - (uint32_t) (w0 & 1), m2 = 0u - (uint32_t) ((w0 >> 1) & 1), m4 = 0u - (uint32_t) ((w0 >> 2) & 1);
+        asm volatile("" : "+v"(m1), "+v"(m2), "+v"(m4));
+        uint32_t y1[PILE_SW + 1], y2[PILE_SW + 1], y[PILE_SW + 1];
+#pragma unroll
+        for (int k = 0; k <= PILE_SW; k++) y1[k] = ((k + 1 <= PILE_SW ? S[k + 1] : 0u) & m1) | (S[k] & ~m1);
+#pragma unroll
+        for (int k = 0; k <= PILE_SW; k++) y2[k] = ((k + 2 <= PILE_SW ? y1[k + 2] : 0u) & m2) | (y1[k] & ~m2);
+#pragma unroll
+        for (int k = 0; k <= PILE_SW; k++) y[k] = ((k + 4 <= PILE_SW ? y2[k + 4] : 0u) & m4) | (y2[k] & ~m4);
+#pragma unroll
+        for (int k = 0; k < (RW > 0 ? RW : PR_TKW); k++) row[k * RS] = k < PILE_SW ? funnel(y[k], y[k + 1], sh) : 0u;
+    }
+    int nr = 0;
+    bool uncovered = false, stack_ovf = false;
+    uint32_t cur0 = 0u;
+    node_runs_core<true, PR_RCAP, RS, RW>(row, nwin, act, cc, stk, rbuf, t, nr, uncovered, stack_ovf, cur0, step);
+    bool ok = act && nr >= 1 && nr <= PR_RCAP && !uncovered && !stack_ovf;
+    uint32_t key_[PILE_RUNS], kc_[PILE_RUNS];
+#pragma unroll
+    for (int k = 0; k < PILE_RUNS; k++) { key_[k] = 0u; kc_[k] = 0u; }
+    int n = 0;
+    uint32_t last_q = 0xFFFFFFFFu;
+    const int nrs = nr < PR_RCAP ? nr : PR_RCAP;
+    for (int r = PR_RCAP - 1; r >= 0; r--) {
+        if (ok && r < nrs) {
+            const uint32_t d = rbuf[r][t];
+            const int q = (int) (d & 255u), p0 = (int) (d >> 8);
+            if ((uint32_t) q != last_q) {
+                uint32_t h, pk;
+                kmer_key<RS, RW>(row, q < 192 ? q : 0, true, cc, h, pk);
+                const uint32_t kv = cluster_key(h, fs), cv = (uint32_t) (q - m_max + 64) | ((uint32_t) (p0 - m_max + 64) << 8);
+#pragma unroll
+                for (int k = 0; k < PILE_RUNS; k++) if (k == n) { key_[k] = kv; kc_[k] = cv; }
+                n++;
+                last_q = (uint32_t) q;
+            }
+        }
+    }
+    ok = ok && n >= 1 && n <= PILE_RUNS;
+    if (in && further) {
+        uint4 *l2 = rec2 + (size_t) slot * 4 - 4;
+        pile_list_store(l2, 0u, ok, n, key_, kc_, (uint32_t) (nwin - m_max + 64));
+        if (!ok) {
+            const uint64_t jb = slot >= 3u ? (uint64_t) slot - 3u : 0ull;
+            for (uint64_t j2 = jb; j2 < jb + 64u + 3u && j2 < n_entries; j2++) {
+                const uint4 s2 = side[j2];
+                if ((s2.z >> 31) && ((s2.z >> 16) & 3u) != 0u && s2.w == slot) atomicOr(&own_mask[j2 >> 5], 1u << (j2 & 31u));
+            }
+        }
+    } else if (in) {
+        uint32_t *lw = reinterpret_cast<uint32_t *>(line);
+        pile_list_store(line, lw[16], ok, n, key_, kc_, (uint32_t) (nwin - m_max + 64));
+        if (!ok) {
+            lw[16] = lw[16] & 255u;
+            const uint32_t cntb = min(lw[16] & 255u, 64u), e0b = lw[17];
+            for (uint32_t i2 = 0; i2 < cntb; i2++) {
+                const uint64_t j2 = (uint64_t) e0b + i2;
+                if (j2 < n_entries) { const uint4 s2 = side[j2]; if ((s2.z >> 31) && ((s2.z >> 16) & 3u) == 0u) atomicOr(&own_mask[j2 >> 5], 1u << (j2 & 31u)); }
+            }
+        }
+    }
+}
+
 __global__ void __launch_bounds__(TK_ROWS) k_pile_runs_consensus(const uint4 *__restrict__ side, uint64_t n_entries, uint32_t n_buckets, uint4 *__restrict__ tab, const uint4 *__restrict__ rec,
                                                                  uint4 *__restrict__ rec2, ClusterCfg cc, int U, int Lmin,
                                                                  const unsigned long long *__restrict__ pile_cnt, uint32_t *__restrict__ own_mask) {
@@ -286,95 +384,45 @@
         const uint64_t j = base + (uint64_t) q * TK_ROWS + (uint64_t) t;
         if (j < n_entries) {
             const uint4 sd = side[j];
-            if ((sd.z >> 30) & 1u) sList[atomicAdd(&sN, 1u)] = ((sd.z >> 16) & 3u) == 0u ? min(sd.w, n_buckets) : (uint32_t) min((uint64_t) sd.w, n_entries) | 0x80000000u;
+            if ((sd.z >> 30) & 1u) sList[atomicAdd(&sN, 1u)] = pile_who((sd.z >> 16) & 3u, sd.w, n_buckets, n_entries);
         }
     }
     __syncthreads();
     const int np = (int) sN;
-    const int fs = cc.idx_shift - CL_MBITS;
-    const int step = max(16, min(64, cc.w) & ~15);
     for (int c0 = 0; c0 < np; c0 += TK_ROWS) {
         const bool in = c0 + t < np;
-        const uint32_t who = sList[in ? c0 + t : 0];
-        const bool further = (who >> 31) != 0u;
-        const uint32_t slot = who & 0x7FFFFFFFu;
-        uint4 *line = tab + (size_t) (further ? 0u : who) * 8;
-        const uint4 *src = further ? rec + (size_t) slot * 4 : (const uint4 *) line;
-        uint32_t S[PILE_SW + 1];
-        unsigned long long rm = 0ull;
-        {
-            const uint4 l0 = src[0], l1 = src[1], l2 = src[2], l3 = src[3];
-            S[0] = l0.x; S[1] = l0.y; S[2] = l0.z; S[3] = l0.w; S[4] = l1.x; S[5] = l1.y; S[6] = l1.z; S[7] = l1.w;
-            S[8] = l2.x; S[9] = l2.y; S[10] = l2.z; S[11] = l2.w; S[12] = l3.x; S[13] = 0u;
-            rm = !in ? 0ull : (further ? (((unsigned long long) l3.w << 32) | l3.z) : (((unsigned long long) l3.z << 32) | l3.y));
-        }
-        const bool act = in && rm != 0ull;
-        const int m_min = act ? __clzll((long long) rm) : 0, m_max = act ? 63 - __builtin_ctzll(rm) : 0;
-        const int len_v = U + m_max - m_min;
-        const int nwin = len_v - Lmin + 1;
-        {
-            const int ob = 2 * (64 - m_max), w0 = ob >> 5, sh = ob & 31;
-            uint32_t m1 = 0u - (uint32_t) (w0 & 1), m2 = 0u - (uint32_t) ((w0 >> 1) & 1), m4 = 0u - (uint32_t) ((w0 >> 2) & 1);
-            asm volatile("" : "+v"(m1), "+v"(m2), "+v"(m4));
-            uint32_t y1[PILE_SW + 1], y2[PILE_SW + 1], y[PILE_SW + 1];
-#pragma unroll
-            for (int k = 0; k <= PILE_SW; k++) y1[k] = ((k + 1 <= PILE_SW ? S[k + 1] : 0u) & m1) | (S[k] & ~m1);
-#pragma unroll
-            for (int k = 0; k <= PILE_SW; k++) y2[k] = ((k + 2 <= PILE_SW ? y1[k + 2] : 0u) & m2) | (y1[k] & ~m2);
-#pragma unroll
-            for (int k = 0; k <= PILE_SW; k++) y[k] = ((k + 4 <= PILE_SW ? y2[k + 4] : 0u) & m4) | (y2[k] & ~m4);
-#pragma unroll
-            for (int k = 0; k < PR_TKW; k++) s[t][k] = k < PILE_SW ? funnel(y[k], y[k + 1], sh) : 0u;
-        }
-        int nr = 0;
-        bool uncovered = false, stack_ovf = false;
-        uint32_t cur0 = 0u;
-        node_runs_core<true, PR_RCAP>(s[t], nwin, act, cc, stk, rbuf, t, nr, uncovered, stack_ovf, cur0, step);
-        bool ok = act && nr >= 1 && nr <= PR_RCAP && !uncovered && !stack_ovf;
-        uint32_t key_[PILE_RUNS], kc_[PILE_RUNS];
-#pragma unroll
-        for (int k = 0; k < PILE_RUNS; k++) { key_[k] = 0u; kc_[k] = 0u; }
-        int n = 0;
-        uint32_t last_q = 0xFFFFFFFFu;
-        const int nrs = nr < PR_RCAP ? nr : PR_RCAP;
-        for (int r = PR_RCAP - 1; r >= 0; r--) {
-            if (ok && r < nrs) {
-                const uint32_t d = rbuf[r][t];
-                const int q = (int) (d & 255u), p0 = (int) (d >> 8);
-                if ((uint32_t) q != last_q) {
-                    uint32_t h, pk;
-                    kmer_key(s[t], q < 192 ? q : 0, true, cc, h, pk);
-                    const uint32_t kv = cluster_key(h, fs), cv = (uint32_t) (q - m_max + 64) | ((uint32_t) (p0 - m_max + 64) << 8);
-#pragma unroll
-                    for (int k = 0; k < PILE_RUNS; k++) if (k == n) { key_[k] = kv; kc_[k] = cv; }
-                    n++;
-                    last_q = (uint32_t) q;
-                }
-            }
-        }
-        ok = ok && n >= 1 && n <= PILE_RUNS;
-        if (in && further) {
-            uint4 *l2 = rec2 + (size_t) slot * 4 - 4;
-            pile_list_store(l2, 0u, ok, n, key_, kc_, (uint32_t) (nwin - m_max + 64));
-            if (!ok) {
-                const uint64_t jb = slot >= 3u ? (uint64_t) slot - 3u : 0ull;
-                for (uint64_t j2 = jb; j2 < jb + 64u + 3u && j2 < n_entries; j2++) {
-                    const uint4 s2 = side[j2];
-                    if ((s2.z >> 31) && ((s2.z >> 16) & 3u) != 0u && s2.w == slot) atomicOr(&own_mask[j2 >> 5], 1u << (j2 & 31u));
-                }
-            }
-        } else if (in) {
-            uint32_t *lw = reinterpret_cast<uint32_t *>(line);
-            pile_list_store(line, lw[16], ok, n, key_, kc_, (uint32_t) (nwin - m_max + 64));
-            if (!ok) {
-                lw[16] = lw[16] & 255u;
-                const uint32_t cntb = min(lw[16] & 255u, 64u), e0b = lw[17];
-                for (uint32_t i2 = 0; i2 < cntb; i2++) {
-                    const uint64_t j2 = (uint64_t) e0b + i2;
-                    if (j2 < n_entries) { const uint4 s2 = side[j2]; if ((s2.z >> 31) && ((s2.z >> 16) & 3u) == 0u) atomicOr(&own_mask[j2 >> 5], 1u << (j2 & 31u)); }
-                }
-            }
-        }
+        pile_consensus_one<1, 0>(sList[in ? c0 + t : 0], in, s[t], stk, rbuf, t, side, n_entries, tab, rec, rec2, cc, U, Lmin, own_mask);
+    }
+}
+
+__global__ void __launch_bounds__(TK_ROWS) k_pile_runs_consensus_list(const uint32_t *__restrict__ plist, const uint32_t *__restrict__ pcount, uint32_t n_segs, const uint4 *__restrict__ side,
+                                                                      uint64_t n_entries, uint4 *__restrict__ tab, const uint4 *__restrict__ rec, uint4 *__restrict__ rec2, ClusterCfg cc,
+                                                                      int U, int Lmin, const unsigned long long *__restrict__ pile_cnt, uint32_t *__restrict__ own_mask) {
+    if (pile_declines(pile_cnt)) return;
+    __shared__ uint32_t s[PILE_SW][TK_ROWS];
+    __shared__ uint32_t stk[2 * (NR_STACK + 1)][TK_ROWS];
+    __shared__ uint16_t rbuf[PR_RCAP + 1][TK_ROWS];
+    __shared__ uint32_t sOff[PR_SEGS + 1];
+    const int t = (int) threadIdx.x;
+    const uint32_t seg0 = blockIdx.x * PR_SEGS;
+    if (t < 64) {
+        const uint32_t g = seg0 + (uint32_t) t;
+        uint32_t c = (t < PR_SEGS && g < n_segs) ? min(pcount[g], (uint32_t) PB_THREADS) : 0u;
+#pragma unroll
+        for (int d = 1; d < PR_SEGS; d <<= 1) { const uint32_t o = __shfl_up(c, d); if (t >= d) c += o; }
+        if (t < PR_SEGS) sOff[t + 1] = c;
+        if (t == 0) sOff[0] = 0u;
+    }
+    __syncthreads();
+    const int np = (int) sOff[PR_SEGS];
+    for (int c0 = 0; c0 < np; c0 += TK_ROWS) {
+        const int i = c0 + t;
+        const bool in = i < np;
+        int g = 0;
+#pragma unroll
+        for (int b = PR_SEGS / 2; b >= 1; b >>= 1) g += (g + b <= PR_SEGS - 1 && (int) sOff[g + b] <= i) ? b : 0;
+        const uint32_t who = in ? plist[(size_t) (seg0 + (uint32_t) g) * PB_THREADS + (uint32_t) (i - (int) sOff[g])] : 0u;
+        pile_consensus_one<TK_ROWS, PILE_SW>(who, in, &s[0][t], stk, rbuf, t, side, n_entries, tab, rec, rec2, cc, U, Lmin, own_mask);
     }
 }
 
@@ -849,19 +897,24 @@
     const uint64_t tiles = (n_entries + PB_TILE - 1) / PB_TILE;
     const dim3 sample((unsigned) std::max<uint64_t>(1, std::min<uint64_t>(tiles, std::max<uint64_t>(64, tiles / 32)))), block(PB_THREADS);
     hipLaunchKernelGGL((k_pile_build<true>), sample, block, 0, s, nd, skeys, sids, n_entries, (const uint4 *) dir, cc, uniform_len, (uint4 *) nullptr, (uint4 *) nullptr, 0u, (uint4 *) nullptr, pile_cnt,
-                       (uint32_t *) nullptr);
+                       (uint32_t *) nullptr, (uint32_t *) nullptr, (uint32_t *) nullptr);
     hipLaunchKernelGGL(k_pile_sample_close, dim3(1), dim3(1), 0, s, pile_cnt);
 }
 
 void launch_pile_build(const NodesDev &nd, const PrefSufCfg &cfg, const ClusterCfg &cc, int uniform_len, const uint32_t *skeys, const uint32_t *sids, const void *dir, void *rec, void *rec2,
-                       void *tab, uint32_t epoch, void *side, const void *runs, int nwin, const unsigned long long *pile_cnt, uint32_t *own_mask, hipStream_t s) {
+                       void *tab, uint32_t epoch, void *side, const void *runs, int nwin, const unsigned long long *pile_cnt, uint32_t *own_mask, void *plist, hipStream_t s) {
     const uint64_t n_entries = nd.n > 0 ? (uint64_t) nd.n : 0;
     if (n_entries == 0) return;
     const uint64_t tiles = (n_entries + PB_TILE - 1) / PB_TILE;
+    if (!own_mask) plist = nullptr;
+    uint32_t *pl = (uint32_t *) plist, *pc = pl ? pl + tiles * PB_THREADS : nullptr;
     if (own_mask) (void) hipMemsetAsync(own_mask, 0, pile_own_mask_bytes(n_entries), s);
     hipLaunchKernelGGL((k_pile_build<false>), dim3((unsigned) tiles), dim3(PB_THREADS), 0, s, nd, skeys, sids, n_entries, (const uint4 *) dir, cc, uniform_len, (uint4 *) rec, (uint4 *) tab, epoch,
-                       (uint4 *) side, const_cast<unsigned long long *>(pile_cnt), own_mask);
-    if (own_mask)
+                       (uint4 *) side, const_cast<unsigned long long *>(pile_cnt), own_mask, pl, pc);
+    if (pl)
+        hipLaunchKernelGGL(k_pile_runs_consensus_list, dim3((unsigned) ((tiles + PR_SEGS - 1) / PR_SEGS)), dim3(TK_ROWS), 0, s, (const uint32_t *) pl, (const uint32_t *) pc, (uint32_t) tiles,
+                           (const uint4 *) side, n_entries, (uint4 *) tab, (const uint4 *) rec, (uint4 *) rec2, cc, uniform_len, cfg.Lmin, pile_cnt, own_mask);
+    else if (own_mask)
         hipLaunchKernelGGL(k_pile_runs_consensus, dim3((unsigned) ((n_entries + PR_TILE - 1) / PR_TILE)), dim3(TK_ROWS), 0, s, (const uint4 *) side, n_entries, cc.n_buckets, (uint4 *) tab,
                            (const uint4 *) rec, (uint4 *) rec2, cc, uniform_len, cfg.Lmin, pile_cnt, own_mask);
     else
@@ -869,6 +922,8 @@
 }
 
 size_t pile_own_mask_bytes(uint64_t n) { return (size_t) ((n + 31) / 32 + 1024) * 4; }
+
+size_t pile_list_bytes(uint64_t n) { const uint64_t tiles = (n + PB_TILE - 1) / PB_TILE; return (size_t) (tiles * (PB_THREADS + 1) + 64) * 4; }
 
 void launch_pile_own_ids(const uint32_t *own_mask, const uint32_t *sids, uint64_t n_entries, int32_t *list, uint32_t cap, unsigned long long *pile_cnt, hipStream_t s) {
     if (n_entries == 0) return;
```

Measured after the change: 4.895 billion edges/s (median of 6 runs). +3.8%, better.
